# ErikNatanael/knaster

Hardware: AMD Instinct MI355X
Metric: UGen-samples/sec (voices x block_size x UGens / s) (higher is better)
Workload: dtype f32

## Files before the change

bindings/rust/knaster_hip/src/ffi.rs:

```rust
#![allow(non_camel_case_types)]
use core::ffi::{c_char, c_void};

#[repr(C)]
pub struct knh_bank {
    _private: [u8; 0],
}
#[repr(C)]
pub struct knh_comm {
    _private: [u8; 0],
}
pub const KNH_COMM_ID_BYTES: usize = 128;
pub type knh_reduce_fn = Option<unsafe extern "C" fn(user: *mut c_void, device_buf: *mut c_void, count: usize, sample_type: u32, root: u32, hip_stream: *mut c_void) -> i32>;

#[repr(C)]
#[derive(Clone, Copy, Debug, Default, PartialEq, Eq)]
pub struct knh_stage_desc {
    pub kind: u16,
    pub flags: u16,
    pub delayed_changes_per_block: u16,
    pub ar_param: u16,
    pub input: u16,
    pub input2: u16,
}

#[repr(C)]
pub struct knh_bank_desc {
    pub abi_version: u32,
    pub n_voices: u32,
    pub sample_type: u32,
    pub n_stages: u32,
    pub stages: *const knh_stage_desc,
    pub out_channels: u32,
    pub mix_mode: u32,
    pub device: i32,
    pub allow_fma: u32,
    pub in_channels: u32,
}

pub const KNH_ABI_VERSION: u32 = 4;

pub const KNH_OK: i32 = 0;
pub const KNH_ERR_INVALID_ARGUMENT: i32 = 1;
pub const KNH_ERR_OUT_OF_RANGE: i32 = 2;
pub const KNH_ERR_UNSUPPORTED_CHAIN: i32 = 3;
pub const KNH_ERR_DEVICE: i32 = 4;
pub const KNH_ERR_NOT_INITIALISED: i32 = 5;
pub const KNH_ERR_NO_DEVICE: i32 = 6;
pub const KNH_ERR_WRONG_VALUE_KIND: i32 = 7;
pub const KNH_ERR_OUT_OF_MEMORY: i32 = 8;
pub const KNH_ERR_INTERNAL: i32 = 9;

pub const KNH_F32: u32 = 0;
pub const KNH_F64: u32 = 1;

pub const KNH_VALUE_FLOAT: u32 = 0;
pub const KNH_VALUE_TRIGGER: u32 = 1;
pub const KNH_VALUE_INTEGER: u32 = 2;
pub const KNH_VALUE_BOOL: u32 = 3;
pub const KNH_VALUE_SMOOTHING: u32 = 4;

pub const KNH_STAGE_SIN_WT: u16 = 0;
pub const KNH_STAGE_SIN_NUMERIC: u16 = 1;
pub const KNH_STAGE_SVF: u16 = 2;
pub const KNH_STAGE_ONEPOLE_LPF: u16 = 3;
pub const KNH_STAGE_ONEPOLE_HPF: u16 = 4;
pub const KNH_STAGE_MUL_ENV_ASR: u16 = 5;
pub const KNH_STAGE_MUL_ENV_AR: u16 = 6;
pub const KNH_STAGE_MUL_CONST: u16 = 7;
pub const KNH_STAGE_ADD_CONST: u16 = 8;
pub const KNH_STAGE_SUB_CONST: u16 = 9;
pub const KNH_STAGE_DIV_CONST: u16 = 10;
pub const KNH_STAGE_WR_MUL: u16 = 11;
pub const KNH_STAGE_WR_ADD: u16 = 12;
pub const KNH_STAGE_WR_SUB: u16 = 13;
pub const KNH_STAGE_MUL_ENVELOPE: u16 = 14;
pub const KNH_STAGE_WR_VSUB: u16 = 15;
pub const KNH_STAGE_WR_DIV: u16 = 16;
pub const KNH_STAGE_WR_VDIV: u16 = 17;
pub const KNH_STAGE_WR_POWF: u16 = 18;
pub const KNH_STAGE_WR_POWI: u16 = 19;
pub const KNH_STAGE_POW_CONST: u16 = 20;
pub const KNH_STAGE_SAMPLE_DELAY: u16 = 21;
pub const KNH_STAGE_PHASOR: u16 = 22;
pub const KNH_STAGE_SAFETY_LIMITER: u16 = 23;
pub const KNH_STAGE_POLYBLEP: u16 = 24;
pub const KNH_STAGE_ALLPASS_DELAY: u16 = 25;
pub const KNH_STAGE_ALLPASS_FB_DELAY: u16 = 26;
pub const KNH_STAGE_BUFFER_READER: u16 = 27;
pub const KNH_STAGE_WHITE_NOISE: u16 = 28;
pub const KNH_STAGE_PINK_NOISE: u16 = 29;
pub const KNH_STAGE_BROWN_NOISE: u16 = 30;
pub const KNH_STAGE_RANDOM_LIN: u16 = 31;
pub const KNH_STAGE_PAN2: u16 = 32;
pub const KNH_STAGE_MATH_ADD: u16 = 33;
pub const KNH_STAGE_MATH_SUB: u16 = 34;
pub const KNH_STAGE_MATH_MUL: u16 = 35;
pub const KNH_STAGE_MATH_DIV: u16 = 36;
pub const KNH_STAGE_MATH_POW: u16 = 37;
pub const KNH_STAGE_INPUT: u16 = 38;
pub const KNH_STAGE_GALACTIC: u16 = 39;
pub const KNH_STAGE_KIND_COUNT: u16 = 40;

pub const KNH_SVF_LOW: u32 = 0;
pub const KNH_SVF_HIGH: u32 = 1;
pub const KNH_SVF_BAND: u32 = 2;
pub const KNH_SVF_NOTCH: u32 = 3;
pub const KNH_SVF_PEAK: u32 = 4;
pub const KNH_SVF_ALL: u32 = 5;
pub const KNH_SVF_BELL: u32 = 6;
pub const KNH_SVF_LOW_SHELF: u32 = 7;
pub const KNH_SVF_HIGH_SHELF: u32 = 8;

pub const KNH_STAGE_FLAG_AR_FREQ: u16 = 1 << 0;
pub const KNH_STAGE_FLAG_SMOOTH_PARAMS: u16 = 1 << 1;

pub const KNH_MIX_TREE: u32 = 0;
pub const KNH_MIX_LEFT_FOLD: u32 = 1;

pub const KNH_FLAG_ANY_DONE: u32 = 1 << 0;
pub const KNH_FLAG_ALL_DONE: u32 = 1 << 1;

#[link(name = "knaster_hip")]
unsafe extern "C" {
    pub fn knh_abi_version() -> u32;
    pub fn knh_device_count() -> i32;
    pub fn knh_status_string(status: i32) -> *const c_char;
    pub fn knh_last_error(bank: *const knh_bank) -> *const c_char;
    pub fn knh_chain_ugen_count(stages: *const knh_stage_desc, n_stages: u32) -> i32;
    pub fn knh_bank_create(desc: *const knh_bank_desc, out_bank: *mut *mut knh_bank) -> i32;
    pub fn knh_bank_create_sharded(desc: *const knh_bank_desc, host_threads: u32, out_bank: *mut *mut knh_bank) -> i32;
    pub fn knh_bank_set_ctor_args(bank: *mut knh_bank, stage: u32, first_voice: u32, count: u32, args: *const f64, n_args: u32) -> i32;
    pub fn knh_bank_set_buffer(bank: *mut knh_bank, stage: u32, samples: *const c_void, n_frames: usize, buffer_sample_rate: f64) -> i32;
    pub fn knh_bank_init(bank: *mut knh_bank, sample_rate: u32, block_size: usize) -> i32;
    pub fn knh_bank_destroy(bank: *mut knh_bank);
    pub fn knh_bank_inputs(bank: *const knh_bank) -> u16;
    pub fn knh_bank_outputs(bank: *const knh_bank) -> u16;
    pub fn knh_bank_stage_parameters(bank: *const knh_bank, stage: u32) -> u16;
    pub fn knh_bank_stage_param_description(bank: *const knh_bank, stage: u32, param: u32) -> *const c_char;
    pub fn knh_bank_param_apply(bank: *mut knh_bank, voice: u32, stage: u32, param: u32, kind: u32, fvalue: f64, ivalue: i64) -> i32;
    pub fn knh_bank_set_delay_within_block_for_param(bank: *mut knh_bank, voice: u32, stage: u32, param: u32, delay: u16) -> i32;
    pub fn knh_bank_param_apply_range(bank: *mut knh_bank, voice_begin: u32, voice_end: u32, stage: u32, param: u32, kind: u32, fvalue: f64, ivalue: i64) -> i32;
    pub fn knh_bank_param_apply_many(bank: *mut knh_bank, count: usize, voices: *const u32, stages: *const u32, params: *const u32, kinds: *const u32, fvalues: *const f64, ivalues: *const i64, delays: *const u16) -> i32;
    pub fn knh_bank_process_block(bank: *mut knh_bank, frames_to_process: usize, block_start_offset: usize, frame_clock: u64, out: *mut c_void, out_flags: *mut u32) -> i32;
    pub fn knh_jit_stats(memory_hits: *mut u64, disk_hits: *mut u64, helper_compiles: *mut u64, in_process_compiles: *mut u64);
    pub fn knh_bank_resident_stats(bank: *mut knh_bank, calls: *mut u64, launches: *mut u64) -> i32;
    pub fn knh_bank_resident_trace(bank: *mut knh_bank, ticks5: *mut u64) -> i32;
    pub fn knh_bank_process_block_channels(bank: *mut knh_bank, frames_to_process: usize, block_start_offset: usize, frame_clock: u64, out_channels: *const *mut c_void, out_flags: *mut u32) -> i32;
    pub fn knh_bank_process_block_device(bank: *mut knh_bank, frames_to_process: usize, block_start_offset: usize, frame_clock: u64, out_device: *mut c_void, hip_stream: *mut c_void) -> i32;
    pub fn knh_bank_process_block_voices(bank: *mut knh_bank, frames_to_process: usize, block_start_offset: usize, frame_clock: u64, out: *mut c_void, voices_out: *mut c_void, out_flags: *mut u32) -> i32;
    pub fn knh_bank_process_blocks(bank: *mut knh_bank, n_blocks: u32, frame_clock: u64, out: *mut c_void, out_flags: *mut u32) -> i32;
    pub fn knh_bank_process_blocks_device(bank: *mut knh_bank, n_blocks: u32, frame_clock: u64, out_device: *mut c_void, hip_stream: *mut c_void) -> i32;
    pub fn knh_bank_process_blocks_device_add(bank: *mut knh_bank, n_blocks: u32, frame_clock: u64, out_device: *mut c_void, hip_stream: *mut c_void) -> i32;
    pub fn knh_device_malloc(bytes: usize, device: i32) -> *mut c_void;
    pub fn knh_device_free(device_ptr: *mut c_void);
    pub fn knh_device_read(dst_host: *mut c_void, src_device: *const c_void, bytes: usize, hip_stream: *mut c_void) -> i32;
    pub fn knh_bank_param_apply_many_at(bank: *mut knh_bank, block_offset: u32, count: usize, voices: *const u32, stages: *const u32, params: *const u32, kinds: *const u32, fvalues: *const f64, ivalues: *const i64, delays: *const u16) -> i32;
    pub fn knh_bank_read_done_frames(bank: *mut knh_bank, done_frames: *mut u32) -> i32;
    pub fn knh_bank_debug_words(bank: *mut knh_bank, out16: *mut u32) -> i32;
    pub fn knh_bank_debug_signature(bank: *const knh_bank) -> *const core::ffi::c_char;
    pub fn knh_bank_synchronize(bank: *mut knh_bank) -> i32;
    pub fn knh_bank_timing_reset(bank: *mut knh_bank, enable: i32) -> i32;
    pub fn knh_bank_timing_read(bank: *mut knh_bank, kernel_ms: *mut f64, launches: *mut u64) -> i32;
    pub fn knh_bank_collective_timing_read(bank: *mut knh_bank, reduce_ms: *mut f64, reduces: *mut u64) -> i32;
    pub fn knh_bank_algorithmic_bytes_per_voice_block(bank: *const knh_bank, read_bytes: *mut u32, write_bytes: *mut u32) -> i32;
    pub fn knh_bank_process_blocks_begin(bank: *mut knh_bank, n_blocks: u32, frame_clock: u64) -> i32;
    pub fn knh_bank_process_blocks_end(bank: *mut knh_bank, out: *mut c_void) -> i32;
    pub fn knh_bank_set_input(bank: *mut knh_bank, n_blocks: u32, input: *const c_void) -> i32;
    pub fn knh_bank_set_input_device(bank: *mut knh_bank, n_blocks: u32, in_device: *const c_void) -> i32;
    pub fn knh_bank_create_multi_device(desc: *const knh_bank_desc, devices: *const i32, n_devices: u32, out_bank: *mut *mut knh_bank) -> i32;
    pub fn knh_comm_unique_id(id: *mut u8) -> i32;
    pub fn knh_bank_create_rank(desc: *const knh_bank_desc, rank: u32, world: u32, comm_id: *const u8, out_bank: *mut *mut knh_bank) -> i32;
    pub fn knh_bank_create_rank_custom(desc: *const knh_bank_desc, rank: u32, world: u32, reduce: knh_reduce_fn, user: *mut c_void, out_bank: *mut *mut knh_bank) -> i32;
    pub fn knh_shard_voice_range(n_voices: u32, rank: u32, world: u32, first: *mut u32, count: *mut u32) -> i32;
    pub fn knh_bank_ranks(bank: *const knh_bank) -> u32;
    pub fn knh_comm_create(rank: u32, world: u32, id: *const u8, device: i32, out_comm: *mut *mut knh_comm) -> i32;
    pub fn knh_comm_destroy(comm: *mut knh_comm);
    pub fn knh_comm_last_error(comm: *const knh_comm) -> *const c_char;
    pub fn knh_comm_world(comm: *const knh_comm) -> u32;
    pub fn knh_comm_rccl_version() -> i32;
    pub fn knh_comm_reduce_sum(comm: *mut knh_comm, buf: *mut c_void, count: usize, sample_type: u32, root: u32, after_stream: *mut c_void) -> i32;
    pub fn knh_comm_wait_buffer(comm: *mut knh_comm, buf: *const c_void, stream: *mut c_void) -> i32;
    pub fn knh_comm_wait(comm: *mut knh_comm, stream: *mut c_void) -> i32;
    pub fn knh_comm_synchronize(comm: *mut knh_comm) -> i32;
    pub fn knh_comm_timing_reset(comm: *mut knh_comm, enable: i32) -> i32;
    pub fn knh_comm_timing_read(comm: *mut knh_comm, reduce_ms: *mut f64, reduces: *mut u64) -> i32;
}
```

include/knaster_hip.h:

```cpp
#ifndef KNASTER_HIP_H
#define KNASTER_HIP_H

#include <stddef.h>
#include <stdint.h>

#ifdef __cplusplus
extern "C" {
#endif

#define KNH_ABI_VERSION 4

typedef enum knh_status {
  KNH_OK = 0,
  KNH_ERR_INVALID_ARGUMENT = 1,
  KNH_ERR_OUT_OF_RANGE = 2,
  KNH_ERR_UNSUPPORTED_CHAIN = 3,
  KNH_ERR_DEVICE = 4,
  KNH_ERR_NOT_INITIALISED = 5,
  KNH_ERR_NO_DEVICE = 6,
  KNH_ERR_WRONG_VALUE_KIND = 7,
  KNH_ERR_OUT_OF_MEMORY = 8,
  KNH_ERR_INTERNAL = 9
} knh_status;

typedef enum knh_sample_type { KNH_F32 = 0, KNH_F64 = 1 } knh_sample_type;

typedef enum knh_value_kind {
  KNH_VALUE_FLOAT = 0,
  KNH_VALUE_TRIGGER = 1,
  KNH_VALUE_INTEGER = 2,
  KNH_VALUE_BOOL = 3,
  KNH_VALUE_SMOOTHING = 4
} knh_value_kind;

typedef enum knh_stage_kind {
  KNH_STAGE_SIN_WT = 0,
  KNH_STAGE_SIN_NUMERIC = 1,
  KNH_STAGE_SVF = 2,
  KNH_STAGE_ONEPOLE_LPF = 3,
  KNH_STAGE_ONEPOLE_HPF = 4,
  KNH_STAGE_MUL_ENV_ASR = 5,
  KNH_STAGE_MUL_ENV_AR = 6,
  KNH_STAGE_MUL_CONST = 7,
  KNH_STAGE_ADD_CONST = 8,
  KNH_STAGE_SUB_CONST = 9,
  KNH_STAGE_DIV_CONST = 10,
  KNH_STAGE_WR_MUL = 11,
  KNH_STAGE_WR_ADD = 12,
  KNH_STAGE_WR_SUB = 13,
  KNH_STAGE_MUL_ENVELOPE = 14,
  KNH_STAGE_WR_VSUB = 15,
  KNH_STAGE_WR_DIV = 16,
  KNH_STAGE_WR_VDIV = 17,
  KNH_STAGE_WR_POWF = 18,
  KNH_STAGE_WR_POWI = 19,
  KNH_STAGE_POW_CONST = 20,
  KNH_STAGE_SAMPLE_DELAY = 21,
  KNH_STAGE_PHASOR = 22,
  KNH_STAGE_SAFETY_LIMITER = 23,
  KNH_STAGE_POLYBLEP = 24,
  KNH_STAGE_ALLPASS_DELAY = 25,
  KNH_STAGE_ALLPASS_FB_DELAY = 26,
  KNH_STAGE_BUFFER_READER = 27,
  KNH_STAGE_WHITE_NOISE = 28,
  KNH_STAGE_PINK_NOISE = 29,
  KNH_STAGE_BROWN_NOISE = 30,
  KNH_STAGE_RANDOM_LIN = 31,
  KNH_STAGE_PAN2 = 32,
  KNH_STAGE_MATH_ADD = 33,
  KNH_STAGE_MATH_SUB = 34,
  KNH_STAGE_MATH_MUL = 35,
  KNH_STAGE_MATH_DIV = 36,
  KNH_STAGE_MATH_POW = 37,
  KNH_STAGE_INPUT = 38,
  KNH_STAGE_GALACTIC = 39,
  KNH_STAGE_KIND_COUNT = 40
} knh_stage_kind;

typedef enum knh_svf_type {
  KNH_SVF_LOW = 0, KNH_SVF_HIGH = 1, KNH_SVF_BAND = 2, KNH_SVF_NOTCH = 3, KNH_SVF_PEAK = 4,
  KNH_SVF_ALL = 5, KNH_SVF_BELL = 6, KNH_SVF_LOW_SHELF = 7, KNH_SVF_HIGH_SHELF = 8
} knh_svf_type;

enum {
  KNH_STAGE_FLAG_AR_FREQ = 1u << 0,
  KNH_STAGE_FLAG_SMOOTH_PARAMS = 1u << 1
};

typedef struct knh_stage_desc {
  uint16_t kind;
  uint16_t flags;
  uint16_t delayed_changes_per_block;
  uint16_t ar_param;
  uint16_t input;
  uint16_t input2;
} knh_stage_desc;

typedef enum knh_mix_mode {
  KNH_MIX_TREE = 0,
  KNH_MIX_LEFT_FOLD = 1
} knh_mix_mode;

typedef struct knh_bank_desc {
  uint32_t abi_version;
  uint32_t n_voices;
  uint32_t sample_type;
  uint32_t n_stages;
  const knh_stage_desc* stages;
  uint32_t out_channels;
  uint32_t mix_mode;
  int32_t device;
  uint32_t allow_fma;
  uint32_t in_channels;
} knh_bank_desc;

typedef struct knh_bank knh_bank;

enum {
  KNH_FLAG_ANY_DONE = 1u << 0,
  KNH_FLAG_ALL_DONE = 1u << 1
};

uint32_t knh_abi_version(void);
int32_t knh_device_count(void);
const char* knh_status_string(int32_t status);
const char* knh_last_error(const knh_bank* bank);

int32_t knh_chain_ugen_count(const knh_stage_desc* stages, uint32_t n_stages);

int32_t knh_bank_create(const knh_bank_desc* desc, knh_bank** out_bank);
int32_t knh_bank_create_sharded(const knh_bank_desc* desc, uint32_t host_threads, knh_bank** out_bank);
int32_t knh_bank_set_ctor_args(knh_bank* bank, uint32_t stage, uint32_t first_voice, uint32_t count,
                               const double* args, uint32_t n_args);
int32_t knh_bank_set_buffer(knh_bank* bank, uint32_t stage, const void* samples, size_t n_frames, double buffer_sample_rate);
int32_t knh_bank_init(knh_bank* bank, uint32_t sample_rate, size_t block_size);
void knh_bank_destroy(knh_bank* bank);

uint16_t knh_bank_inputs(const knh_bank* bank);
uint16_t knh_bank_outputs(const knh_bank* bank);
uint16_t knh_bank_stage_parameters(const knh_bank* bank, uint32_t stage);
const char* knh_bank_stage_param_description(const knh_bank* bank, uint32_t stage, uint32_t param);

int32_t knh_bank_param_apply(knh_bank* bank, uint32_t voice, uint32_t stage, uint32_t param,
                             uint32_t kind, double fvalue, int64_t ivalue);
int32_t knh_bank_set_delay_within_block_for_param(knh_bank* bank, uint32_t voice, uint32_t stage,
                                                  uint32_t param, uint16_t delay);
int32_t knh_bank_param_apply_many(knh_bank* bank, size_t count, const uint32_t* voices,
                                  const uint32_t* stages, const uint32_t* params,
                                  const uint32_t* kinds, const double* fvalues,
                                  const int64_t* ivalues, const uint16_t* delays);
int32_t knh_bank_param_apply_range(knh_bank* bank, uint32_t voice_begin, uint32_t voice_end, uint32_t stage,
                                   uint32_t param, uint32_t kind, double fvalue, int64_t ivalue);

int32_t knh_bank_process_block(knh_bank* bank, size_t frames_to_process, size_t block_start_offset,
                               uint64_t frame_clock, void* out, uint32_t* out_flags);
int32_t knh_bank_process_block_channels(knh_bank* bank, size_t frames_to_process, size_t block_start_offset,
                                        uint64_t frame_clock, void* const* out_channels, uint32_t* out_flags);
int32_t knh_bank_resident_stats(knh_bank* bank, uint64_t* calls, uint64_t* launches);
int32_t knh_bank_resident_trace(knh_bank* bank, uint64_t* ticks5);
int32_t knh_bank_process_block_device(knh_bank* bank, size_t frames_to_process,
                                      size_t block_start_offset, uint64_t frame_clock,
                                      void* out_device, void* hip_stream);
int32_t knh_bank_set_input(knh_bank* bank, uint32_t n_blocks, const void* in);
int32_t knh_bank_set_input_device(knh_bank* bank, uint32_t n_blocks, const void* in_device);
int32_t knh_bank_process_block_voices(knh_bank* bank, size_t frames_to_process,
                                      size_t block_start_offset, uint64_t frame_clock, void* out,
                                      void* voices_out, uint32_t* out_flags);
int32_t knh_bank_process_blocks(knh_bank* bank, uint32_t n_blocks, uint64_t frame_clock, void* out,
                                uint32_t* out_flags);
int32_t knh_bank_process_blocks_device(knh_bank* bank, uint32_t n_blocks, uint64_t frame_clock,
                                       void* out_device, void* hip_stream);
int32_t knh_bank_process_blocks_device_add(knh_bank* bank, uint32_t n_blocks, uint64_t frame_clock,
                                           void* out_device, void* hip_stream);
int32_t knh_bank_process_blocks_begin(knh_bank* bank, uint32_t n_blocks, uint64_t frame_clock);
int32_t knh_bank_process_blocks_end(knh_bank* bank, void* out);
void* knh_device_malloc(size_t bytes, int32_t device);
void knh_device_free(void* device_ptr);
int32_t knh_device_read(void* dst_host, const void* src_device, size_t bytes, void* hip_stream);
int32_t knh_bank_param_apply_many_at(knh_bank* bank, uint32_t block_offset, size_t count,
                                     const uint32_t* voices, const uint32_t* stages,
                                     const uint32_t* params, const uint32_t* kinds,
                                     const double* fvalues, const int64_t* ivalues,
                                     const uint16_t* delays);
int32_t knh_bank_read_done_frames(knh_bank* bank, uint32_t* done_frames);
int32_t knh_bank_debug_words(knh_bank* bank, uint32_t* out16);
const char* knh_bank_debug_signature(const knh_bank* bank);
void knh_jit_stats(uint64_t* memory_hits, uint64_t* disk_hits, uint64_t* helper_compiles, uint64_t* in_process_compiles);
int32_t knh_bank_synchronize(knh_bank* bank);

int32_t knh_bank_timing_reset(knh_bank* bank, int32_t enable);
int32_t knh_bank_timing_read(knh_bank* bank, double* kernel_ms, uint64_t* launches);
int32_t knh_bank_collective_timing_read(knh_bank* bank, double* reduce_ms, uint64_t* reduces);
int32_t knh_bank_algorithmic_bytes_per_voice_block(const knh_bank* bank, uint32_t* read_bytes,
                                                   uint32_t* write_bytes);


int32_t knh_bank_create_multi_device(const knh_bank_desc* desc, const int32_t* devices, uint32_t n_devices, knh_bank** out_bank);

#define KNH_COMM_ID_BYTES 128
int32_t knh_comm_unique_id(uint8_t* id);
int32_t knh_bank_create_rank(const knh_bank_desc* desc, uint32_t rank, uint32_t world, const uint8_t* comm_id, knh_bank** out_bank);
typedef int32_t (*knh_reduce_fn)(void* user, void* device_buf, size_t count, uint32_t sample_type, uint32_t root, void* hip_stream);
int32_t knh_bank_create_rank_custom(const knh_bank_desc* desc, uint32_t rank, uint32_t world, knh_reduce_fn reduce, void* user,
                                    knh_bank** out_bank);
int32_t knh_shard_voice_range(uint32_t n_voices, uint32_t rank, uint32_t world, uint32_t* first, uint32_t* count);
uint32_t knh_bank_ranks(const knh_bank* bank);

typedef struct knh_comm knh_comm;
int32_t knh_comm_create(uint32_t rank, uint32_t world, const uint8_t* id, int32_t device, knh_comm** out_comm);
void knh_comm_destroy(knh_comm* comm);
const char* knh_comm_last_error(const knh_comm* comm);
uint32_t knh_comm_world(const knh_comm* comm);
int32_t knh_comm_rccl_version(void);
int32_t knh_comm_reduce_sum(knh_comm* comm, void* buf, size_t count, uint32_t sample_type, uint32_t root, void* after_stream);
int32_t knh_comm_wait_buffer(knh_comm* comm, const void* buf, void* stream);
int32_t knh_comm_wait(knh_comm* comm, void* stream);
int32_t knh_comm_synchronize(knh_comm* comm);
int32_t knh_comm_timing_reset(knh_comm* comm, int32_t enable);
int32_t knh_comm_timing_read(knh_comm* comm, double* reduce_ms, uint64_t* reduces);

#ifdef __cplusplus
}
#endif
#endif
```

knaster_amd/_lib.py:

```python
from __future__ import annotations

import ctypes as C
import os

_HERE = os.path.dirname(os.path.abspath(__file__))
LIB_PATH = os.environ.get("KNH_LIB") or os.path.join(_HERE, "csrc", "libknaster_hip.so")

KNH_ABI_VERSION = 4

OK, ERR_INVALID_ARGUMENT, ERR_OUT_OF_RANGE, ERR_UNSUPPORTED_CHAIN, ERR_DEVICE = 0, 1, 2, 3, 4
ERR_NOT_INITIALISED, ERR_NO_DEVICE, ERR_WRONG_VALUE_KIND, ERR_OUT_OF_MEMORY, ERR_INTERNAL = 5, 6, 7, 8, 9
F32, F64 = 0, 1
VALUE_FLOAT, VALUE_TRIGGER, VALUE_INTEGER, VALUE_BOOL, VALUE_SMOOTHING = 0, 1, 2, 3, 4
(STAGE_SIN_WT, STAGE_SIN_NUMERIC, STAGE_SVF, STAGE_ONEPOLE_LPF, STAGE_ONEPOLE_HPF, STAGE_MUL_ENV_ASR,
 STAGE_MUL_ENV_AR, STAGE_MUL_CONST, STAGE_ADD_CONST, STAGE_SUB_CONST, STAGE_DIV_CONST, STAGE_WR_MUL,
 STAGE_WR_ADD, STAGE_WR_SUB, STAGE_MUL_ENVELOPE, STAGE_WR_VSUB, STAGE_WR_DIV, STAGE_WR_VDIV, STAGE_WR_POWF,
 STAGE_WR_POWI, STAGE_POW_CONST, STAGE_SAMPLE_DELAY, STAGE_PHASOR, STAGE_SAFETY_LIMITER, STAGE_POLYBLEP, STAGE_ALLPASS_DELAY, STAGE_ALLPASS_FB_DELAY, STAGE_BUFFER_READER,
 STAGE_WHITE_NOISE, STAGE_PINK_NOISE, STAGE_BROWN_NOISE, STAGE_RANDOM_LIN, STAGE_PAN2,
 STAGE_MATH_ADD, STAGE_MATH_SUB, STAGE_MATH_MUL, STAGE_MATH_DIV, STAGE_MATH_POW, STAGE_INPUT, STAGE_GALACTIC) = range(40)
STAGE_FLAG_AR_FREQ = 1
STAGE_FLAG_SMOOTH_PARAMS = 2
SVF_LOW, SVF_HIGH, SVF_BAND, SVF_NOTCH, SVF_PEAK, SVF_ALL, SVF_BELL, SVF_LOW_SHELF, SVF_HIGH_SHELF = range(9)
MIX_TREE, MIX_LEFT_FOLD = 0, 1
FLAG_ANY_DONE, FLAG_ALL_DONE = 1, 2

STAGE_CTOR_ARGS = {
    STAGE_SIN_WT: 1, STAGE_SIN_NUMERIC: 1, STAGE_SVF: 4, STAGE_ONEPOLE_LPF: 1, STAGE_ONEPOLE_HPF: 0,
    STAGE_MUL_ENV_ASR: 2, STAGE_MUL_ENV_AR: 2, STAGE_MUL_CONST: 1, STAGE_ADD_CONST: 1, STAGE_SUB_CONST: 1,
    STAGE_DIV_CONST: 1, STAGE_WR_MUL: 1, STAGE_WR_ADD: 1, STAGE_WR_SUB: 1,
    STAGE_WR_VSUB: 1, STAGE_WR_DIV: 1, STAGE_WR_VDIV: 1, STAGE_WR_POWF: 1, STAGE_WR_POWI: 1, STAGE_POW_CONST: 1, STAGE_SAMPLE_DELAY: 1, STAGE_PHASOR: 1, STAGE_SAFETY_LIMITER: 0, STAGE_POLYBLEP: 2, STAGE_ALLPASS_DELAY: 1, STAGE_ALLPASS_FB_DELAY: 1, STAGE_BUFFER_READER: 3,
    STAGE_WHITE_NOISE: 1, STAGE_PINK_NOISE: 1, STAGE_BROWN_NOISE: 1, STAGE_RANDOM_LIN: 2, STAGE_PAN2: 1,
    STAGE_MATH_ADD: 0, STAGE_MATH_SUB: 0, STAGE_MATH_MUL: 0, STAGE_MATH_DIV: 0, STAGE_MATH_POW: 0, STAGE_INPUT: 1,
    STAGE_GALACTIC: 7,
}


class StageDesc(C.Structure):
    _fields_ = [("kind", C.c_uint16), ("flags", C.c_uint16), ("delayed_changes_per_block", C.c_uint16),
                ("ar_param", C.c_uint16), ("input", C.c_uint16), ("input2", C.c_uint16)]


class BankDesc(C.Structure):
    _fields_ = [("abi_version", C.c_uint32), ("n_voices", C.c_uint32), ("sample_type", C.c_uint32),
                ("n_stages", C.c_uint32), ("stages", C.POINTER(StageDesc)), ("out_channels", C.c_uint32),
                ("mix_mode", C.c_uint32), ("device", C.c_int32), ("allow_fma", C.c_uint32), ("in_channels", C.c_uint32)]


PROTOTYPES = {
    "knh_abi_version": (C.c_uint32, []),
    "knh_device_count": (C.c_int32, []),
    "knh_status_string": (C.c_char_p, [C.c_int32]),
    "knh_last_error": (C.c_char_p, [C.c_void_p]),
    "knh_chain_ugen_count": (C.c_int32, [C.POINTER(StageDesc), C.c_uint32]),
    "knh_bank_create": (C.c_int32, [C.POINTER(BankDesc), C.POINTER(C.c_void_p)]),
    "knh_bank_create_sharded": (C.c_int32, [C.POINTER(BankDesc), C.c_uint32, C.POINTER(C.c_void_p)]),
    "knh_bank_set_ctor_args": (C.c_int32, [C.c_void_p, C.c_uint32, C.c_uint32, C.c_uint32, C.c_void_p, C.c_uint32]),
    "knh_bank_set_buffer": (C.c_int32, [C.c_void_p, C.c_uint32, C.c_void_p, C.c_size_t, C.c_double]),
    "knh_bank_init": (C.c_int32, [C.c_void_p, C.c_uint32, C.c_size_t]),
    "knh_bank_destroy": (None, [C.c_void_p]),
    "knh_bank_inputs": (C.c_uint16, [C.c_void_p]),
    "knh_bank_outputs": (C.c_uint16, [C.c_void_p]),
    "knh_bank_stage_parameters": (C.c_uint16, [C.c_void_p, C.c_uint32]),
    "knh_bank_stage_param_description": (C.c_char_p, [C.c_void_p, C.c_uint32, C.c_uint32]),
    "knh_bank_param_apply": (C.c_int32, [C.c_void_p, C.c_uint32, C.c_uint32, C.c_uint32, C.c_uint32, C.c_double, C.c_int64]),
    "knh_bank_set_delay_within_block_for_param": (C.c_int32, [C.c_void_p, C.c_uint32, C.c_uint32, C.c_uint32, C.c_uint16]),
    "knh_bank_param_apply_many": (C.c_int32, [C.c_void_p, C.c_size_t, C.c_void_p, C.c_void_p, C.c_void_p, C.c_void_p,
                                             C.c_void_p, C.c_void_p, C.c_void_p]),
    "knh_bank_param_apply_range": (C.c_int32, [C.c_void_p, C.c_uint32, C.c_uint32, C.c_uint32, C.c_uint32, C.c_uint32, C.c_double, C.c_int64]),
    "knh_bank_process_block": (C.c_int32, [C.c_void_p, C.c_size_t, C.c_size_t, C.c_uint64, C.c_void_p, C.POINTER(C.c_uint32)]),
    "knh_jit_stats": (None, [C.POINTER(C.c_uint64), C.POINTER(C.c_uint64), C.POINTER(C.c_uint64), C.POINTER(C.c_uint64)]),
    "knh_bank_resident_stats": (C.c_int32, [C.c_void_p, C.POINTER(C.c_uint64), C.POINTER(C.c_uint64)]),
    "knh_bank_resident_trace": (C.c_int32, [C.c_void_p, C.POINTER(C.c_uint64)]),
    "knh_bank_process_block_channels": (C.c_int32, [C.c_void_p, C.c_size_t, C.c_size_t, C.c_uint64, C.POINTER(C.c_void_p), C.POINTER(C.c_uint32)]),
    "knh_bank_process_block_device": (C.c_int32, [C.c_void_p, C.c_size_t, C.c_size_t, C.c_uint64, C.c_void_p, C.c_void_p]),
    "knh_bank_process_block_voices": (C.c_int32, [C.c_void_p, C.c_size_t, C.c_size_t, C.c_uint64, C.c_void_p, C.c_void_p,
                                                 C.POINTER(C.c_uint32)]),
    "knh_bank_process_blocks": (C.c_int32, [C.c_void_p, C.c_uint32, C.c_uint64, C.c_void_p, C.POINTER(C.c_uint32)]),
    "knh_bank_process_blocks_device": (C.c_int32, [C.c_void_p, C.c_uint32, C.c_uint64, C.c_void_p, C.c_void_p]),
    "knh_bank_process_blocks_device_add": (C.c_int32, [C.c_void_p, C.c_uint32, C.c_uint64, C.c_void_p, C.c_void_p]),
    "knh_device_malloc": (C.c_void_p, [C.c_size_t, C.c_int32]),
    "knh_device_free": (None, [C.c_void_p]),
    "knh_device_read": (C.c_int32, [C.c_void_p, C.c_void_p, C.c_size_t, C.c_void_p]),
    "knh_bank_param_apply_many_at": (C.c_int32, [C.c_void_p, C.c_uint32, C.c_size_t, C.c_void_p, C.c_void_p, C.c_void_p,
                                                C.c_void_p, C.c_void_p, C.c_void_p, C.c_void_p]),
    "knh_bank_read_done_frames": (C.c_int32, [C.c_void_p, C.c_void_p]),
    "knh_bank_debug_words": (C.c_int32, [C.c_void_p, C.c_void_p]),
    "knh_bank_debug_signature": (C.c_char_p, [C.c_void_p]),
    "knh_bank_synchronize": (C.c_int32, [C.c_void_p]),
    "knh_bank_timing_reset": (C.c_int32, [C.c_void_p, C.c_int32]),
    "knh_bank_timing_read": (C.c_int32, [C.c_void_p, C.POINTER(C.c_double), C.POINTER(C.c_uint64)]),
    "knh_bank_collective_timing_read": (C.c_int32, [C.c_void_p, C.POINTER(C.c_double), C.POINTER(C.c_uint64)]),
    "knh_bank_algorithmic_bytes_per_voice_block": (C.c_int32, [C.c_void_p, C.POINTER(C.c_uint32), C.POINTER(C.c_uint32)]),
}

COMM_ID_BYTES = 128
REDUCE_FN = C.CFUNCTYPE(C.c_int32, C.c_void_p, C.c_void_p, C.c_size_t, C.c_uint32, C.c_uint32, C.c_void_p)
PROTOTYPES.update({
    "knh_bank_process_blocks_begin": (C.c_int32, [C.c_void_p, C.c_uint32, C.c_uint64]),
    "knh_bank_process_blocks_end": (C.c_int32, [C.c_void_p, C.c_void_p]),
    "knh_bank_set_input": (C.c_int32, [C.c_void_p, C.c_uint32, C.c_void_p]),
    "knh_bank_set_input_device": (C.c_int32, [C.c_void_p, C.c_uint32, C.c_void_p]),
    "knh_bank_create_multi_device": (C.c_int32, [C.POINTER(BankDesc), C.POINTER(C.c_int32), C.c_uint32, C.POINTER(C.c_void_p)]),
    "knh_comm_unique_id": (C.c_int32, [C.c_void_p]),
    "knh_bank_create_rank": (C.c_int32, [C.POINTER(BankDesc), C.c_uint32, C.c_uint32, C.c_void_p, C.POINTER(C.c_void_p)]),
    "knh_bank_create_rank_custom": (C.c_int32, [C.POINTER(BankDesc), C.c_uint32, C.c_uint32, REDUCE_FN, C.c_void_p, C.POINTER(C.c_void_p)]),
    "knh_shard_voice_range": (C.c_int32, [C.c_uint32, C.c_uint32, C.c_uint32, C.POINTER(C.c_uint32), C.POINTER(C.c_uint32)]),
    "knh_bank_ranks": (C.c_uint32, [C.c_void_p]),
    "knh_comm_create": (C.c_int32, [C.c_uint32, C.c_uint32, C.c_void_p, C.c_int32, C.POINTER(C.c_void_p)]),
    "knh_comm_destroy": (None, [C.c_void_p]),
    "knh_comm_last_error": (C.c_char_p, [C.c_void_p]),
    "knh_comm_world": (C.c_uint32, [C.c_void_p]),
    "knh_comm_rccl_version": (C.c_int32, []),
    "knh_comm_reduce_sum": (C.c_int32, [C.c_void_p, C.c_void_p, C.c_size_t, C.c_uint32, C.c_uint32, C.c_void_p]),
    "knh_comm_wait_buffer": (C.c_int32, [C.c_void_p, C.c_void_p, C.c_void_p]),
    "knh_comm_wait": (C.c_int32, [C.c_void_p, C.c_void_p]),
    "knh_comm_synchronize": (C.c_int32, [C.c_void_p]),
    "knh_comm_timing_reset": (C.c_int32, [C.c_void_p, C.c_int32]),
    "knh_comm_timing_read": (C.c_int32, [C.c_void_p, C.POINTER(C.c_double), C.POINTER(C.c_uint64)]),
})

_lib = None


class KnasterHipError(RuntimeError):
    def __init__(self, status: int, message: str):
        super().__init__(f"knaster_hip status {status}: {message}")
        self.status = status


def load() -> C.CDLL:
    global _lib
    if _lib is not None:
        return _lib
    if not os.path.exists(LIB_PATH):
        raise ImportError(
            f"{LIB_PATH} is missing: build it with `python -m knaster_amd.build` "
            "(hipcc --offload-arch=gfx950).  knaster_amd has no CPU fallback.")
    lib = C.CDLL(LIB_PATH)
    for name, (res, args) in PROTOTYPES.items():
        fn = getattr(lib, name)
        fn.restype = res
        fn.argtypes = args
    if lib.knh_abi_version() != KNH_ABI_VERSION:
        raise ImportError("libknaster_hip.so ABI version mismatch; rebuild it")
    _lib = lib
    return lib
```

knaster_amd/bank.py:

```python
from __future__ import annotations

import ctypes as C
from dataclasses import dataclass
from typing import Optional, Sequence

import numpy as np

from . import _lib as L

TRIGGER = object()


@dataclass(frozen=True)
class Stage:
    kind: int
    flags: int = 0
    delayed_changes_per_block: int = 0
    input: int = 0
    input2: int = 0
    ar_param: int = 0


def _stage_array(stages: Sequence[Stage]):
    arr = (L.StageDesc * len(stages))()
# ... 84 lines not shown
    def _check(self, rc: int):
        if rc != L.OK:
            raise L.KnasterHipError(rc, (self._lib.knh_last_error(self._h) or b"").decode())

    def set_ctor_args(self, stage: int, args, first_voice: int = 0):
        a = np.ascontiguousarray(np.asarray(args, dtype=np.float64))
        if a.ndim == 1:
            a = a.reshape(-1, 1)
        self._check(self._lib.knh_bank_set_ctor_args(self._h, stage, first_voice, a.shape[0],
                                                     a.ctypes.data_as(C.c_void_p), a.shape[1]))

    def set_buffer(self, stage: int, samples, buffer_sample_rate: float):
        a = np.ascontiguousarray(np.asarray(samples, dtype=self.dtype))
        self._check(self._lib.knh_bank_set_buffer(self._h, stage, a.ctypes.data_as(C.c_void_p), a.shape[0], float(buffer_sample_rate)))

    def init(self, sample_rate: int, block_size: int):
        self._check(self._lib.knh_bank_init(self._h, sample_rate, block_size))
        self.sample_rate, self.block_size = sample_rate, block_size

    def inputs(self) -> int:
        return int(self._lib.knh_bank_inputs(self._h))

    def outputs(self) -> int:
        return int(self._lib.knh_bank_outputs(self._h))

    def stage_parameters(self, stage: int) -> int:
        return int(self._lib.knh_bank_stage_parameters(self._h, stage))

    def stage_param_descriptions(self, stage: int):
        out = []
        for p in range(self.stage_parameters(stage)):
            d = self._lib.knh_bank_stage_param_description(self._h, stage, p)
            out.append(d.decode() if d else None)
        return out

    @staticmethod
    def _value(value):
        if value is TRIGGER:
            return L.VALUE_TRIGGER, 0.0, 0
        if isinstance(value, (bool, np.bool_)):
            return L.VALUE_BOOL, 0.0, int(value)
        if isinstance(value, (int, np.integer)):
            return L.VALUE_INTEGER, 0.0, int(value)
        return L.VALUE_FLOAT, float(value), 0

    def param_apply(self, voice: int, stage: int, param: int, value):
        kind, f, i = self._value(value)
        self._check(self._lib.knh_bank_param_apply(self._h, voice, stage, param, kind, f, i))

    def param(self, voice: int, stage: int, param, value):
        if isinstance(param, str):
            descs = self.stage_param_descriptions(stage)
            if param not in descs:
                raise KeyError(f"DescriptionNotFound({param!r})")
            param = descs.index(param)
        self.param_apply(voice, stage, param, value)

    def set_delay_within_block_for_param(self, voice: int, stage: int, param: int, delay: int):
        self._check(self._lib.knh_bank_set_delay_within_block_for_param(self._h, voice, stage, param, delay))

    def param_apply_many(self, voices, stages, params, kinds, fvalues=None, ivalues=None, delays=None, block_offset=0):
        self.param_apply_prepared(self.prepare_many(voices, stages, params, kinds, fvalues, ivalues, delays), block_offset)

    def param_apply_range(self, voice_begin, voice_end, stage, param, kind, fvalue=0.0, ivalue=0):
        self._check(self._lib.knh_bank_param_apply_range(self._h, voice_begin, voice_end, stage, param, kind, float(fvalue), int(ivalue)))

    @staticmethod
    def prepare_many(voices, stages, params, kinds, fvalues=None, ivalues=None, delays=None):
        v = np.ascontiguousarray(voices, dtype=np.uint32)
        n = v.shape[0]
        s = np.ascontiguousarray(np.broadcast_to(np.asarray(stages, dtype=np.uint32), (n,)))
        p = np.ascontiguousarray(np.broadcast_to(np.asarray(params, dtype=np.uint32), (n,)))
        k = np.ascontiguousarray(np.broadcast_to(np.asarray(kinds, dtype=np.uint32), (n,)))
        f = None if fvalues is None else np.ascontiguousarray(np.broadcast_to(np.asarray(fvalues, dtype=np.float64), (n,)))
        i = None if ivalues is None else np.ascontiguousarray(np.broadcast_to(np.asarray(ivalues, dtype=np.int64), (n,)))
        d = None if delays is None else np.ascontiguousarray(np.broadcast_to(np.asarray(delays, dtype=np.uint16), (n,)))
        arrays = (v, s, p, k, f, i, d)
        return n, arrays, tuple(None if a is None else a.ctypes.data_as(C.c_void_p) for a in arrays)

    def param_apply_prepared(self, batch, block_offset=0):
        n, _arrays, ptrs = batch
        if block_offset:
            self._check(self._lib.knh_bank_param_apply_many_at(self._h, block_offset, n, *ptrs))
        else:
            self._check(self._lib.knh_bank_param_apply_many(self._h, n, *ptrs))

    def set_input(self, blocks):
        a = np.ascontiguousarray(np.asarray(blocks, dtype=self.dtype))
        if a.ndim == 2:
            a = a.reshape(1, *a.shape)
        assert a.shape[1:] == (self.in_channels, self.block_size), a.shape
        self._check(self._lib.knh_bank_set_input(self._h, a.shape[0], a.ctypes.data_as(C.c_void_p)))

    def process_block(self, frames_to_process: Optional[int] = None, block_start_offset: int = 0, frame_clock: int = 0,
                      out: Optional[np.ndarray] = None):
        ftp = self.block_size if frames_to_process is None else frames_to_process
        if out is None:
            out = np.zeros((self.out_channels, self.block_size), dtype=self.dtype)
        flags = C.c_uint32(0)
        self._check(self._lib.knh_bank_process_block(self._h, ftp, block_start_offset, frame_clock,
                                                     out.ctypes.data_as(C.c_void_p), C.byref(flags)))
        return out, int(flags.value)

    def process_block_voices(self, frames_to_process: Optional[int] = None, block_start_offset: int = 0, frame_clock: int = 0):
        ftp = self.block_size if frames_to_process is None else frames_to_process
        out = np.zeros((self.out_channels, self.block_size), dtype=self.dtype)
        pan = bool(self.stages) and self.stages[-1].kind in (L.STAGE_PAN2, L.STAGE_GALACTIC)
        voices = np.zeros((2, self.n_voices, self.block_size) if pan else (self.n_voices, self.block_size), dtype=self.dtype)
        flags = C.c_uint32(0)
        self._check(self._lib.knh_bank_process_block_voices(self._h, ftp, block_start_offset, frame_clock,
                                                            out.ctypes.data_as(C.c_void_p),
                                                            voices.ctypes.data_as(C.c_void_p), C.byref(flags)))
        return out, voices, int(flags.value)

    def process_block_device(self, out_device_ptr: int = 0, hip_stream: int = 0, frames_to_process: Optional[int] = None,
                             block_start_offset: int = 0, frame_clock: int = 0):
        ftp = self.block_size if frames_to_process is None else frames_to_process
        self._check(self._lib.knh_bank_process_block_device(self._h, ftp, block_start_offset, frame_clock,
                                                            C.c_void_p(out_device_ptr or None), C.c_void_p(hip_stream or None)))

    def process_blocks(self, n_blocks: int, frame_clock: int = 0):
        out = np.zeros((n_blocks, self.out_channels, self.block_size), dtype=self.dtype)
        flags = C.c_uint32(0)
        self._check(self._lib.knh_bank_process_blocks(self._h, n_blocks, frame_clock, out.ctypes.data_as(C.c_void_p), C.byref(flags)))
        return out, int(flags.value)

    def process_blocks_begin(self, n_blocks: int, frame_clock: int = 0):
        self._check(self._lib.knh_bank_process_blocks_begin(self._h, n_blocks, frame_clock))
        self._begun = getattr(self, "_begun", []) + [n_blocks]

    def process_blocks_end(self):
        n_blocks = self._begun.pop(0)
        out = np.zeros((n_blocks, self.out_channels, self.block_size), dtype=self.dtype)
        self._check(self._lib.knh_bank_process_blocks_end(self._h, out.ctypes.data_as(C.c_void_p)))
        return out

    def process_blocks_device(self, n_blocks: int, out_device_ptr: int = 0, hip_stream: int = 0, frame_clock: int = 0):
        self._check(self._lib.knh_bank_process_blocks_device(self._h, n_blocks, frame_clock, C.c_void_p(out_device_ptr or None),
                                                             C.c_void_p(hip_stream or None)))

    def read_done_frames(self) -> np.ndarray:
        d = np.zeros(self.n_voices, dtype=np.uint32)
        self._check(self._lib.knh_bank_read_done_frames(self._h, d.ctypes.data_as(C.c_void_p)))
        return d

    def debug_signature(self) -> str:
        return self._lib.knh_bank_debug_signature(self._h).decode()

    def resident_stats(self):
        c, n = C.c_uint64(0), C.c_uint64(0)
        self._check(self._lib.knh_bank_resident_stats(self._h, C.byref(c), C.byref(n)))
        return int(c.value), int(n.value)

    def debug_words(self) -> np.ndarray:
        d = np.zeros(16, dtype=np.uint32)
        self._check(self._lib.knh_bank_debug_words(self._h, d.ctypes.data_as(C.c_void_p)))
        return d

    def synchronize(self):
        self._check(self._lib.knh_bank_synchronize(self._h))

    def ranks(self) -> int:
        return int(self._lib.knh_bank_ranks(self._h))

    def timing_reset(self, enable: bool = True):
        self._check(self._lib.knh_bank_timing_reset(self._h, 1 if enable else 0))

    def timing_read(self):
        ms, n = C.c_double(0), C.c_uint64(0)
        self._check(self._lib.knh_bank_timing_read(self._h, C.byref(ms), C.byref(n)))
        return float(ms.value), int(n.value)

    def collective_timing_read(self):
        ms, n = C.c_double(0), C.c_uint64(0)
        self._check(self._lib.knh_bank_collective_timing_read(self._h, C.byref(ms), C.byref(n)))
        return float(ms.value), int(n.value)

    def algorithmic_bytes_per_voice_block(self):
        r, w = C.c_uint32(0), C.c_uint32(0)
        self._check(self._lib.knh_bank_algorithmic_bytes_per_voice_block(self._h, C.byref(r), C.byref(w)))
        return int(r.value), int(w.value)
```

knaster_amd/build.py:

```python
from __future__ import annotations

import os
import shutil
import subprocess
import sys

HERE = os.path.dirname(os.path.abspath(__file__))
CSRC = os.path.join(HERE, "csrc")
LIB = os.path.join(CSRC, "libknaster_hip.so")
SOURCES = ["kernels_pipe.hip", "kernels_single.hip", "kernels_wide.hip", "kernels_fold.hip", "kernels_interp.hip", "kernels_events.hip", "kernels_galactic.hip", "bank.hip", "jit.hip", "comm.hip"]
UNITS = [("kernels_pipe.hip", "kernels_pipe_mixer.o", ["-DKNH_PIPE_PART=0"]), ("kernels_pipe.hip", "kernels_pipe_fold.o", ["-DKNH_PIPE_PART=1"]),
         ("kernels_pipe.hip", "kernels_pipe_inplace.o", ["-DKNH_PIPE_PART=2"])] + [(s, s.replace(".hip", ".o"), []) for s in SOURCES[1:]]
HELPER = os.path.join(CSRC, "knh_jit_helper")
HEADERS = ["jit_cache.hpp", "stage_table.hpp", "bank_base.hpp", "voice_bank.hpp", "resident_call.hpp", "event_resolver.hpp", "chain_signature.hpp", "voice_stages.hpp", "voice_chain.hpp", "voice_pipe.hpp", "voice_frame.hpp", "kernel_registry.hpp", "jit.hpp", "host_shards.hpp", "shard_workers.hpp", "rank_bank.hpp", "galactic_bank.hpp", "voice_galactic.hpp", os.path.join("..", "..", "include", "knaster_hip.h"),
           os.path.join("..", "build.py")]
FLAGS = [
    "--offload-arch=gfx950",
    "-O3",
    "-std=c++17",
    "-ffp-contract=off",
    "-fPIC",
    "-Wall",
    "-Wno-unused-value",
]
LINK_FLAGS = ["--offload-arch=gfx950", "-shared", "-fPIC", "-lhiprtc", "-lpthread", "-ldl"]


def _hipcc() -> str:
    for cand in (os.environ.get("HIPCC"), shutil.which("hipcc"), "/opt/rocm/bin/hipcc"):
        if cand and os.path.exists(cand):
            return cand
    raise RuntimeError("hipcc not found (looked at $HIPCC, PATH, /opt/rocm/bin/hipcc)")


def needs_build() -> bool:
    if not os.path.exists(LIB) or not os.path.exists(HELPER):
        return True
    t = min(os.path.getmtime(LIB), os.path.getmtime(HELPER))
    deps = [os.path.join(CSRC, f) for f in SOURCES + HEADERS + ["jit_helper.cpp"]]
    return any(os.path.getmtime(d) > t for d in deps)


def build_helper(verbose: bool = True) -> str:
    src = os.path.join(CSRC, "jit_helper.cpp")
    if os.path.exists(HELPER) and os.path.getmtime(HELPER) >= max(os.path.getmtime(src), os.path.getmtime(os.path.join(CSRC, "jit_cache.hpp"))):
        return HELPER
    rocm = os.environ.get("ROCM_PATH", "/opt/rocm")
    cmd = [os.environ.get("CXX", "g++"), "-std=c++17", "-O2", "-Wall", "-D__HIP_PLATFORM_AMD__", "-I" + os.path.join(rocm, "include"), src, "-o", HELPER + ".tmp",
           "-L" + os.path.join(rocm, "lib"), "-Wl,-rpath," + os.path.join(rocm, "lib"), "-lhiprtc", "-lpthread"]
    if verbose:
        print("[knaster_amd.build]", " ".join(cmd), flush=True)
    res = subprocess.run(cmd, cwd=CSRC, capture_output=True, text=True)
    if res.returncode != 0:
        sys.stderr.write(res.stdout + res.stderr)
        raise RuntimeError("building knh_jit_helper failed")
    os.replace(HELPER + ".tmp", HELPER)
    return HELPER


def write_jit_source() -> None:
    text = open(os.path.join(CSRC, "voice_stages.hpp")).read()
    chain = open(os.path.join(CSRC, "voice_chain.hpp")).read()
    text += "\n" + chain.replace("#pragma once", "").replace('#include "voice_stages.hpp"', "")
    pipe = open(os.path.join(CSRC, "voice_pipe.hpp")).read()
    text += "\n" + pipe.replace("#pragma once", "").replace('#include "voice_chain.hpp"', "")
    frame = open(os.path.join(CSRC, "voice_frame.hpp")).read()
    text += "\n" + frame.replace("#pragma once", "").replace('#include "voice_chain.hpp"', "")
    chunks = [text[i:i + 8000] for i in range(0, len(text), 8000)]
    body = "\n".join('R"KNHJIT(' + c + ')KNHJIT"' for c in chunks) + "\n"
    path = os.path.join(CSRC, "jit_source.inc")
    if not os.path.exists(path) or open(path).read() != body:
        with open(path, "w") as f:
            f.write(body)


def build(force: bool = False, verbose: bool = True, variant: str = "") -> str:
    variant = variant or os.environ.get("KNH_BUILD_VARIANT", "")
    lib = LIB if not variant else LIB.replace(".so", "_" + variant + ".so")
    if not force and not variant and not needs_build():
        return LIB
    build_helper(verbose)
    write_jit_source()
    extra = ["-DKNH_DAG_STAMPS"] if os.environ.get("KNH_BUILD_STAMPS") == "1" or variant == "stamps" else []
    extra += os.environ.get("KNH_EXTRA_FLAGS", "").split()
    objdir = os.path.join(CSRC, "build" + ("_" + variant if variant else ""))
    os.makedirs(objdir, exist_ok=True)
    hipcc = _hipcc()
    procs = []
    objs = []
    header_time = max(os.path.getmtime(os.path.join(CSRC, h)) for h in HEADERS if os.path.exists(os.path.join(CSRC, h)))
    header_time = max(header_time, os.path.getmtime(os.path.join(CSRC, "jit_source.inc")))
    for src, objname, unit_flags in UNITS:
        obj = os.path.join(objdir, objname)
        objs.append(obj)
        cmd = [hipcc, *FLAGS, *extra, *unit_flags, "-c", src, "-o", obj]
        stamp = obj + ".flags"
        fresh = (not force and os.path.exists(obj) and os.path.exists(stamp) and open(stamp).read() == " ".join(cmd)
                 and os.path.getmtime(obj) >= max(os.path.getmtime(os.path.join(CSRC, src)), header_time))
        if fresh:
            continue
        if os.path.exists(stamp):
            os.remove(stamp)
        if verbose:
            print("[knaster_amd.build]", " ".join(cmd), flush=True)
        procs.append((src, obj, subprocess.Popen(cmd, cwd=CSRC, stdout=subprocess.PIPE, stderr=subprocess.STDOUT, text=True), " ".join(cmd)))
    failed = False
    for src, obj, p, cmdline in procs:
        out, _ = p.communicate()
        if p.returncode == 0:
            with open(obj + ".flags", "w") as f:
                f.write(cmdline)
        if p.returncode != 0:
            sys.stderr.write(out)
            failed = True
        elif out.strip() and verbose:
            sys.stderr.write(out)
    if failed:
        raise RuntimeError("hipcc failed building libknaster_hip.so")
    cmd = [hipcc, *LINK_FLAGS, "-o", lib + ".tmp", *objs]
    if verbose:
        print("[knaster_amd.build]", " ".join(cmd), flush=True)
    res = subprocess.run(cmd, cwd=CSRC, capture_output=True, text=True)
    if res.returncode != 0:
        sys.stderr.write(res.stdout + res.stderr)
        raise RuntimeError("hipcc failed linking libknaster_hip.so")
    os.replace(lib + ".tmp", lib)
    return lib


if __name__ == "__main__":
    print(build(force="--force" in sys.argv, variant=next((a.split("=", 1)[1] for a in sys.argv if a.startswith("--variant=")), "")))
```

knaster_amd/csrc/bank.hip:

```cpp
#include <hip/hip_runtime.h>

#include <algorithm>
#include <atomic>
#include <chrono>
#include <cmath>
#include <cstddef>
#include <cstdio>
#include <cstdlib>
#include <cstring>
#include <functional>
#include <memory>
#include <mutex>
#include <new>
#include <stdexcept>
#include <string>
#include <thread>
#include <vector>

#include "../../include/knaster_hip.h"
#include "jit.hpp"
#include "kernel_registry.hpp"

using knh_dev::Event;
using knh_dev::VoiceKernelArgs;

#include "stage_table.hpp"
#include "bank_base.hpp"
#include "chain_signature.hpp"
#include "event_resolver.hpp"
#include "resident_call.hpp"
#include "voice_bank.hpp"

namespace {

template <typename F>
knh_bank* make_bank(const knh_bank_desc& d, const knh::KernelEntry* entry, const std::string& sig) {
  std::unique_ptr<Bank<F>> b(new Bank<F>());
  b->desc = d;
  b->entry = entry;
  b->signature = sig;
  {
    const char* jit_env = std::getenv("KNH_JIT");
    if (jit_env && jit_env[0] == '1') b->entry = nullptr;
    const char* env = std::getenv("KNH_PIPELINE");
    const int level = env && env[0] >= '0' && env[0] <= '2' ? env[0] - '0' : 1;
    b->pipeline_level = level;
    const char* big_env = std::getenv("KNH_PIPE_BIG");
    const unsigned forms = big_env && big_env[0] == '0' ? 1u : (big_env && big_env[0] == '1' ? 3u : 7u);
    if (b->entry && level >= 1) b->pipe = knh::find_pipe(sig.c_str(), forms);
    {
      const unsigned groups = (d.n_voices + 63u) / 64u;
      const char* penv = std::getenv("KNH_PAIR");
      const knh::PipeEntry* pair = b->entry && level >= 1 ? knh::find_pipe(sig.c_str(), 1u << 2 , 2) : nullptr;
      const bool want = penv ? penv[0] == '1' : (groups > 256u && groups <= 512u && d.sample_type != KNH_F64);
      if (pair && want && !(penv && penv[0] == '0')) { b->pipe = pair; b->pipe_pair = true; }
    }
    b->wide = b->entry && !b->pipe_pair ? knh::find_wide(sig.c_str()) : nullptr;
    if (b->wide) {
      const unsigned groups = (d.n_voices + 63u) / 64u;
      const unsigned pipe_max = d.sample_type == KNH_F64 ? 256u : 512u;
      int ww = groups <= pipe_max && b->pipe ? 0 : (groups <= 1024 ? 4 : 8);
      if (!b->pipe && groups <= 256) ww = 0;
      if (b->pipe && sig.find_first_of("DYZ") != std::string::npos) ww = groups <= 256 ? 0 : (groups <= 1024 ? 4 : 8);
      const char* wenv = std::getenv("KNH_WIDE");
      if (wenv) ww = std::atoi(wenv);
      if (ww == 4 || ww == 8 || ww == 16) b->wide_waves = ww;
    }
  }
  b->nv = d.n_voices;
  int slot = 0, pbase = 0;
  for (uint32_t i = 0; i < d.n_stages; ++i) {
    const KindInfo& k = kKinds[d.stages[i].kind];
    StageInfo s{d.stages[i].kind, d.stages[i].flags, d.stages[i].delayed_changes_per_block, slot, k.n_slots, k.n_params, k.n_ctor, pbase,
                d.stages[i].input, d.stages[i].input2, d.stages[i].ar_param};
    if (s.kind == KNH_STAGE_SVF && s.ar_param != 0) s.n_slots = 12;
    b->stages.push_back(s);
    b->ctor.emplace_back(static_cast<size_t>(d.n_voices) * (k.n_ctor > 0 ? k.n_ctor : 0), 0.0);
    slot += s.n_slots;
    pbase += k.n_params;
  }
  b->n_slots = slot;
  b->n_params_total = pbase;
  b->desc.stages = nullptr;
  return b.release();
}

}

#include "host_shards.hpp"
#include "rank_bank.hpp"
#include "galactic_bank.hpp"

namespace {
template <typename F>
knh_bank* make_sharded(const knh_bank_desc& d, const knh::KernelEntry* entry, const std::string& sig, uint32_t host_threads,
                       const int32_t* devices = nullptr) {
  const uint32_t groups = (d.n_voices + 63u) / 64u;
  const uint32_t k = std::min(host_threads, groups);
  const uint32_t per = ((groups + k - 1) / k) * 64u;
  std::unique_ptr<ShardedBank<F>> b(new ShardedBank<F>());
  b->desc = d;
  b->nv = d.n_voices;
  b->per_shard = per;
  for (uint32_t v = 0; v < d.n_voices; v += per) {
    knh_bank_desc dk = d;
    dk.n_voices = std::min(per, d.n_voices - v);
    if (devices) {
      dk.device = devices[b->shard.size()];
      b->shard_device.push_back(dk.device);
    }
    b->base.push_back(v);
    b->shard.emplace_back(make_bank<F>(dk, entry, sig));
  }
  b->base.push_back(d.n_voices);
  b->stages = b->shard[0]->stages;
  b->n_slots = b->shard[0]->n_slots;
  b->n_params_total = b->shard[0]->n_params_total;
  b->desc.stages = nullptr;
  return b.release();
}
}

namespace {
template <typename F>
knh_bank* make_rank_bank(const knh_bank_desc& d, const knh::KernelEntry* entry, const std::string& sig, uint32_t rank, uint32_t world,
                                const uint8_t* comm_id, knh_reduce_fn reduce, void* user) {
  std::unique_ptr<RankBank<F>> b(new RankBank<F>());
  b->desc = d;
  b->total = d.n_voices;
  b->rank = rank;
  b->world = world;
  uint32_t first = 0, count = 0;
  shard_voice_range(d.n_voices, rank, world, &first, &count);
  b->lo = first;
  b->hi = first + count;
  if (comm_id) std::memcpy(b->comm_id, comm_id, KNH_COMM_ID_BYTES);
  b->custom = reduce;
  b->custom_user = user;
  knh_bank_desc dl = d;
  dl.n_voices = count ? count : 1;
  const char* env = std::getenv("KNH_HOST_THREADS");
  const long k = env ? std::strtol(env, nullptr, 10) : 0;
  std::unique_ptr<knh_bank> proto(k >= 2 && k <= 64 && dl.n_voices > 64 ? make_sharded<F>(dl, entry, sig, static_cast<uint32_t>(k)) : make_bank<F>(dl, entry, sig));
  b->stages = proto->stages;
  b->n_slots = proto->n_slots;
  b->n_params_total = proto->n_params_total;
  if (count) b->local = std::move(proto);
  b->desc.stages = nullptr;
  return b.release();
}
}

namespace {
inline bool ends_in_galactic(const knh_bank_desc& d) { return d.n_stages > 0 && d.stages[d.n_stages - 1].kind == KNH_STAGE_GALACTIC; }
template <typename F>
knh_bank* make_galactic(const knh_bank_desc& d, const std::string& inner_sig) {
  std::unique_ptr<GalacticBank<F>> b(new GalacticBank<F>());
  knh_bank_desc di = d;
  di.n_stages = d.n_stages - 1;
  di.out_channels = 1;
  di.mix_mode = KNH_MIX_TREE;
  b->inner.reset(static_cast<Bank<F>*>(make_bank<F>(di, knh::find_kernel(inner_sig.c_str()), inner_sig)));
  b->desc = d;
  b->nv = d.n_voices;
  b->gstage = d.n_stages - 1;
  b->stages = b->inner->stages;
  const KindInfo& k = kKinds[KNH_STAGE_GALACTIC];
  b->stages.push_back(StageInfo{KNH_STAGE_GALACTIC, 0, 0, b->inner->n_slots, k.n_slots, k.n_params, k.n_ctor, b->inner->n_params_total, 0, 0, 0});
  b->n_slots = b->inner->n_slots;
  b->n_params_total = b->inner->n_params_total + k.n_params;
  b->gctor.assign(static_cast<size_t>(d.n_voices) * 7, 0.0);
  b->par.assign(static_cast<size_t>(d.n_voices) * 5, F(0));
  b->drifted.assign(d.n_voices, 0);
  b->h_params.resize(d.n_voices);
  b->desc.stages = nullptr;
  return b.release();
}
}

namespace {
template <typename Fn>
int32_t guarded(knh_bank* bank, Fn&& fn) noexcept {
  const char* what = nullptr;
// ... 141 lines not shown
  return guarded(nullptr, [&]() -> int32_t {
    if (world > 1 && !reduce) { g_create_error = "null reduce function"; if (out_bank) *out_bank = nullptr; return KNH_ERR_INVALID_ARGUMENT; }
    return create_rank_bank(desc, rank, world, nullptr, reduce, user, out_bank);
  });
}
uint32_t knh_bank_ranks(const knh_bank* bank) { return bank ? bank->ranks() : 0; }

static int32_t create_bank(const knh_bank_desc* desc, uint32_t host_threads, knh_bank** out_bank) {
  return guarded(nullptr, [&]() -> int32_t {
    std::string sig;
    int rc = check_desc(desc, out_bank, &sig);
    if (rc != KNH_OK) return rc;
    if (host_threads > 64) { g_create_error = "host_threads must be at most 64"; return KNH_ERR_INVALID_ARGUMENT; }
    if (ends_in_galactic(*desc)) {
      *out_bank = desc->sample_type == KNH_F64 ? make_galactic<double>(*desc, sig) : make_galactic<float>(*desc, sig);
      return KNH_OK;
    }
    const knh::KernelEntry* entry = knh::find_kernel(sig.c_str());
    if (host_threads >= 2 && desc->mix_mode == KNH_MIX_TREE && desc->n_voices > 64)
      *out_bank = desc->sample_type == KNH_F64 ? make_sharded<double>(*desc, entry, sig, host_threads) : make_sharded<float>(*desc, entry, sig, host_threads);
    else
      *out_bank = desc->sample_type == KNH_F64 ? make_bank<double>(*desc, entry, sig) : make_bank<float>(*desc, entry, sig);
    return KNH_OK;
  });
}

int32_t knh_bank_create(const knh_bank_desc* desc, knh_bank** out_bank) {
  return guarded(nullptr, [&]() -> int32_t {
    const char* env = std::getenv("KNH_HOST_THREADS");
    const long k = env ? std::strtol(env, nullptr, 10) : 0;
    return create_bank(desc, k >= 2 && k <= 64 ? static_cast<uint32_t>(k) : 0u, out_bank);
  });
}

int32_t knh_bank_create_sharded(const knh_bank_desc* desc, uint32_t host_threads, knh_bank** out_bank) {
  return guarded(nullptr, [&]() -> int32_t {
    return create_bank(desc, host_threads, out_bank);
  });
}

void knh_bank_destroy(knh_bank* bank) {
  try {
    if (bank && bank->pipe_stream) {
      (void)hipSetDevice(bank->device);
      (void)hipStreamSynchronize(bank->pipe_stream);
    }
    delete bank;
  } catch (...) {
  }
}

int32_t knh_bank_set_ctor_args(knh_bank* bank, uint32_t stage, uint32_t first_voice, uint32_t count, const double* args, uint32_t n_args) {
  return guarded(bank, [&]() -> int32_t {
    if (!bank) return KNH_ERR_INVALID_ARGUMENT;
    return bank->set_ctor(stage, first_voice, count, args, n_args);
  });
}
int32_t knh_bank_set_buffer(knh_bank* bank, uint32_t stage, const void* samples, size_t n_frames, double buffer_sample_rate) {
  return guarded(bank, [&]() -> int32_t {
    if (!bank) return KNH_ERR_INVALID_ARGUMENT;
    return bank->set_buffer(stage, samples, n_frames, buffer_sample_rate);
  });
}
int32_t knh_bank_init(knh_bank* bank, uint32_t sample_rate, size_t block_size) {
  return guarded(bank, [&]() -> int32_t {
    if (!bank) return KNH_ERR_INVALID_ARGUMENT;
    const int rc = bank->init(sample_rate, block_size);
    if (rc == KNH_OK) bank->channel_block.assign(static_cast<size_t>(bank->desc.out_channels) * block_size * (bank->desc.sample_type == KNH_F64 ? 8 : 4), 0);
    return rc;
  });
}
uint16_t knh_bank_inputs(const knh_bank* bank) { return bank ? static_cast<uint16_t>(bank->desc.in_channels) : 0; }
int32_t knh_bank_set_input(knh_bank* bank, uint32_t n_blocks, const void* in) {
  return guarded(bank, [&]() -> int32_t {
    if (!bank) return KNH_ERR_INVALID_ARGUMENT;
    if (!in) return bank->fail(KNH_ERR_INVALID_ARGUMENT, "null input");
    return bank->set_input(n_blocks, in, nullptr);
  });
}
int32_t knh_bank_set_input_device(knh_bank* bank, uint32_t n_blocks, const void* in_device) {
  return guarded(bank, [&]() -> int32_t {
    if (!bank) return KNH_ERR_INVALID_ARGUMENT;
    if (!in_device) return bank->fail(KNH_ERR_INVALID_ARGUMENT, "null input");
    return bank->set_input(n_blocks, nullptr, in_device);
  });
}
uint16_t knh_bank_outputs(const knh_bank* bank) { return bank ? static_cast<uint16_t>(bank->desc.out_channels) : 0; }
uint16_t knh_bank_stage_parameters(const knh_bank* bank, uint32_t stage) {
  if (!bank || stage >= bank->stages.size()) return 0;
  return static_cast<uint16_t>(bank->stages[stage].n_params);
}
const char* knh_bank_stage_param_description(const knh_bank* bank, uint32_t stage, uint32_t param) {
  if (!bank || stage >= bank->stages.size() || param >= static_cast<uint32_t>(bank->stages[stage].n_params)) return nullptr;
  return kKinds[bank->stages[stage].kind].params[param];
}
int32_t knh_bank_param_apply(knh_bank* bank, uint32_t voice, uint32_t stage, uint32_t param, uint32_t kind, double fvalue, int64_t ivalue) {
  return guarded(bank, [&]() -> int32_t {
    if (!bank) return KNH_ERR_INVALID_ARGUMENT;
    return bank->param_apply(voice, stage, param, kind, fvalue, ivalue);
  });
}
int32_t knh_bank_set_delay_within_block_for_param(knh_bank* bank, uint32_t voice, uint32_t stage, uint32_t param, uint16_t delay) {
  return guarded(bank, [&]() -> int32_t {
    if (!bank) return KNH_ERR_INVALID_ARGUMENT;
    return bank->set_delay(voice, stage, param, delay);
  });
}
int32_t knh_bank_param_apply_many(knh_bank* bank, size_t count, const uint32_t* voices, const uint32_t* stages, const uint32_t* params,
                                  const uint32_t* kinds, const double* fvalues, const int64_t* ivalues, const uint16_t* delays) {
  return guarded(bank, [&]() -> int32_t {
    if (!bank) return KNH_ERR_INVALID_ARGUMENT;
    if (count && (!voices || !stages || !params || !kinds)) return bank->fail(KNH_ERR_INVALID_ARGUMENT, "null array");
    return bank->apply_many(0, count, voices, stages, params, kinds, fvalues, ivalues, delays);
  });
}
int32_t knh_bank_param_apply_range(knh_bank* bank, uint32_t voice_begin, uint32_t voice_end, uint32_t stage, uint32_t param, uint32_t kind,
                                   double fvalue, int64_t ivalue) {
  return guarded(bank, [&]() -> int32_t {
    if (!bank) return KNH_ERR_INVALID_ARGUMENT;
    if (voice_end < voice_begin) return bank->fail(KNH_ERR_INVALID_ARGUMENT, "voice_end < voice_begin");
    return bank->apply_range(voice_begin, voice_end, stage, param, kind, fvalue, ivalue);
  });
}
int32_t knh_bank_process_block(knh_bank* bank, size_t frames_to_process, size_t block_start_offset, uint64_t frame_clock, void* out, uint32_t* out_flags) {
  return guarded(bank, [&]() -> int32_t {
    if (!bank) return KNH_ERR_INVALID_ARGUMENT;
    if (!out) return bank->fail(KNH_ERR_INVALID_ARGUMENT, "null output block");
    return bank->process(1, frames_to_process, block_start_offset, frame_clock, out, nullptr, nullptr, out_flags, nullptr, true);
  });
}
int32_t knh_bank_process_block_channels(knh_bank* bank, size_t frames_to_process, size_t block_start_offset, uint64_t frame_clock, void* const* out_channels, uint32_t* out_flags) {
  return guarded(bank, [&]() -> int32_t {
    if (!bank) return KNH_ERR_INVALID_ARGUMENT;
    if (!out_channels) return bank->fail(KNH_ERR_INVALID_ARGUMENT, "null output channels");
    for (uint32_t c = 0; c < bank->desc.out_channels; ++c)
      if (!out_channels[c]) return bank->fail(KNH_ERR_INVALID_ARGUMENT, "null output channel");
    if (!bank->initialised) return bank->fail(KNH_ERR_NOT_INITIALISED, "bank not initialised");
    unsigned char* blk = bank->channel_block.data();
    const int rc = bank->process(1, frames_to_process, block_start_offset, frame_clock, blk, nullptr, nullptr, out_flags, nullptr, true);
    if (rc != KNH_OK) return rc;
    const size_t word = bank->desc.sample_type == KNH_F64 ? 8 : 4;
    for (uint32_t c = 0; c < bank->desc.out_channels; ++c)
      std::memcpy(out_channels[c], blk + (static_cast<size_t>(c) * bank->block_size + block_start_offset) * word, frames_to_process * word);
    return KNH_OK;
  });
}
int32_t knh_bank_resident_stats(knh_bank* bank, uint64_t* calls, uint64_t* launches) {
  return guarded(bank, [&]() -> int32_t {
    if (!bank) return KNH_ERR_INVALID_ARGUMENT;
    bank->resident_stats(calls, launches);
    return KNH_OK;
  });
}
int32_t knh_bank_resident_trace(knh_bank* bank, uint64_t* ticks5) {
  return guarded(bank, [&]() -> int32_t {
    if (!bank || !ticks5) return KNH_ERR_INVALID_ARGUMENT;
    bank->resident_trace(ticks5);
    return KNH_OK;
  });
}
int32_t knh_bank_process_block_device(knh_bank* bank, size_t frames_to_process, size_t block_start_offset, uint64_t frame_clock, void* out_device, void* hip_stream) {
  return guarded(bank, [&]() -> int32_t {
    if (!bank) return KNH_ERR_INVALID_ARGUMENT;
    return bank->process(1, frames_to_process, block_start_offset, frame_clock, nullptr, out_device, nullptr, nullptr, hip_stream, false);
  });
}
int32_t knh_bank_process_block_voices(knh_bank* bank, size_t frames_to_process, size_t block_start_offset, uint64_t frame_clock, void* out, void* voices_out, uint32_t* out_flags) {
  return guarded(bank, [&]() -> int32_t {
    if (!bank) return KNH_ERR_INVALID_ARGUMENT;
    if (!voices_out) return bank->fail(KNH_ERR_INVALID_ARGUMENT, "null voices_out");
    return bank->process(1, frames_to_process, block_start_offset, frame_clock, out, nullptr, voices_out, out_flags, nullptr, true);
  });
}
int32_t knh_bank_process_blocks(knh_bank* bank, uint32_t n_blocks, uint64_t frame_clock, void* out, uint32_t* out_flags) {
  return guarded(bank, [&]() -> int32_t {
    if (!bank) return KNH_ERR_INVALID_ARGUMENT;
    if (!out) return bank->fail(KNH_ERR_INVALID_ARGUMENT, "null output");
    return bank->process(n_blocks, bank->block_size, 0, frame_clock, out, nullptr, nullptr, out_flags, nullptr, true);
  });
}
int32_t knh_bank_process_blocks_device(knh_bank* bank, uint32_t n_blocks, uint64_t frame_clock, void* out_device, void* hip_stream) {
  return guarded(bank, [&]() -> int32_t {
    if (!bank) return KNH_ERR_INVALID_ARGUMENT;
    return bank->process(n_blocks, bank->block_size, 0, frame_clock, nullptr, out_device, nullptr, nullptr, hip_stream, false);
  });
}
int32_t knh_bank_process_blocks_device_add(knh_bank* bank, uint32_t n_blocks, uint64_t frame_clock, void* out_device, void* hip_stream) {
  return guarded(bank, [&]() -> int32_t {
    if (!bank) return KNH_ERR_INVALID_ARGUMENT;
    return bank->process(n_blocks, bank->block_size, 0, frame_clock, nullptr, out_device, nullptr, nullptr, hip_stream, false, true);
  });
}
int32_t knh_bank_process_blocks_begin(knh_bank* bank, uint32_t n_blocks, uint64_t frame_clock) {
  return guarded(bank, [&]() -> int32_t {
    if (!bank) return KNH_ERR_INVALID_ARGUMENT;
    if (!bank->initialised) return bank->fail(KNH_ERR_NOT_INITIALISED, "bank not initialised");
    if (bank->pipe_count == 2) return bank->fail(KNH_ERR_INVALID_ARGUMENT, "two launches are outstanding: fetch one with knh_bank_process_blocks_end first");
    if (n_blocks == 0 || n_blocks > 4096) return bank->fail(KNH_ERR_INVALID_ARGUMENT, "n_blocks must be in 1..4096");
    auto hip = [&](hipError_t e, const char* what) { return e == hipSuccess ? KNH_OK : bank->fail(KNH_ERR_DEVICE, std::string(what) + ": " + hipGetErrorString(e)); };
    int rc = hip(hipSetDevice(bank->device), "hipSetDevice");
    if (rc != KNH_OK) return rc;
    if (!bank->pipe_stream && (rc = hip(hipStreamCreateWithFlags(&bank->pipe_stream, hipStreamNonBlocking), "hipStreamCreate")) != KNH_OK) return rc;
    knh_bank::PipeSlot& p = bank->pipe[(bank->pipe_head + bank->pipe_count) % 2];
    const size_t bytes = static_cast<size_t>(n_blocks) * bank->desc.out_channels * bank->block_size * (bank->desc.sample_type == KNH_F64 ? 8 : 4);
    if (bytes > p.cap) {
      if (p.dev) (void)hipFree(p.dev);
      if (p.host) (void)hipHostFree(p.host);
      p.dev = p.host = nullptr;
      p.cap = 0;
      if ((rc = hip(hipMalloc(&p.dev, bytes), "hipMalloc")) != KNH_OK) return rc;
      if ((rc = hip(hipMemset(p.dev, 0, bytes), "hipMemset")) != KNH_OK) return rc;
      if ((rc = hip(hipHostMalloc(&p.host, bytes), "hipHostMalloc")) != KNH_OK) return rc;
      p.cap = bytes;
    }
    if (!p.done && (rc = hip(hipEventCreateWithFlags(&p.done, hipEventDisableTiming), "hipEventCreate")) != KNH_OK) return rc;
    p.bytes = bytes;
    rc = bank->process(n_blocks, bank->block_size, 0, frame_clock, nullptr, p.dev, nullptr, nullptr, bank->pipe_stream, false);
    if (rc != KNH_OK) return rc;
    if ((rc = bank->order_after_collective(bank->pipe_stream)) != KNH_OK) return rc;
    if ((rc = hip(hipSetDevice(bank->device), "hipSetDevice")) != KNH_OK) return rc;
    if ((rc = hip(hipMemcpyAsync(p.host, p.dev, bytes, hipMemcpyDeviceToHost, bank->pipe_stream), "hipMemcpyAsync")) != KNH_OK) return rc;
    if ((rc = hip(hipEventRecord(p.done, bank->pipe_stream), "hipEventRecord")) != KNH_OK) return rc;
    bank->pipe_count += 1;
    return KNH_OK;
  });
}
int32_t knh_bank_process_blocks_end(knh_bank* bank, void* out) {
  return guarded(bank, [&]() -> int32_t {
    if (!bank) return KNH_ERR_INVALID_ARGUMENT;
    if (!out) return bank->fail(KNH_ERR_INVALID_ARGUMENT, "null output");
    if (bank->pipe_count == 0) return bank->fail(KNH_ERR_INVALID_ARGUMENT, "no launch is outstanding (knh_bank_process_blocks_begin)");
    knh_bank::PipeSlot& p = bank->pipe[bank->pipe_head];
    if (hipSetDevice(bank->device) != hipSuccess || hipEventSynchronize(p.done) != hipSuccess) return bank->fail(KNH_ERR_DEVICE, "waiting for the launch failed");
    std::memcpy(out, p.host, p.bytes);
    bank->pipe_head = (bank->pipe_head + 1) % 2;
    bank->pipe_count -= 1;
    return KNH_OK;
  });
}
void* knh_device_malloc(size_t bytes, int32_t device) {
  if (device >= 0 && hipSetDevice(device) != hipSuccess) return nullptr;
  void* p = nullptr;
  if (hipMalloc(&p, bytes) != hipSuccess) return nullptr;
  if (hipMemset(p, 0, bytes) != hipSuccess) { (void)hipFree(p); return nullptr; }
  return p;
}
void knh_device_free(void* p) {
  if (p) (void)hipFree(p);
}
int32_t knh_device_read(void* dst_host, const void* src_device, size_t bytes, void* hip_stream) {
  return guarded(nullptr, [&]() -> int32_t {
    if (hipDeviceSynchronize() != hipSuccess) return KNH_ERR_DEVICE;
    (void)hip_stream;
    return hipMemcpy(dst_host, src_device, bytes, hipMemcpyDeviceToHost) == hipSuccess ? KNH_OK : KNH_ERR_DEVICE;
  });
}
int32_t knh_bank_param_apply_many_at(knh_bank* bank, uint32_t block_offset, size_t count, const uint32_t* voices, const uint32_t* stages,
                                     const uint32_t* params, const uint32_t* kinds, const double* fvalues, const int64_t* ivalues,
                                     const uint16_t* delays) {
  return guarded(bank, [&]() -> int32_t {
    if (!bank) return KNH_ERR_INVALID_ARGUMENT;
    if (count && (!voices || !stages || !params || !kinds)) return bank->fail(KNH_ERR_INVALID_ARGUMENT, "null array");
    return bank->apply_many(block_offset, count, voices, stages, params, kinds, fvalues, ivalues, delays);
  });
}
int32_t knh_bank_read_done_frames(knh_bank* bank, uint32_t* done_frames) {
  return guarded(bank, [&]() -> int32_t {
    if (!bank) return KNH_ERR_INVALID_ARGUMENT;
    return bank->read_done_frames(done_frames);
  });
}
void knh_jit_stats(uint64_t* memory_hits, uint64_t* disk_hits, uint64_t* helper_compiles, uint64_t* in_process_compiles) {
  const knh::JitStats st = knh::jit_stats();
  if (memory_hits) *memory_hits = st.memory_hits;
  if (disk_hits) *disk_hits = st.disk_hits;
  if (helper_compiles) *helper_compiles = st.helper_runs;
  if (in_process_compiles) *in_process_compiles = st.in_process;
}
const char* knh_bank_debug_signature(const knh_bank* bank) { return bank ? bank->debug_signature() : ""; }
int32_t knh_bank_debug_words(knh_bank* bank, uint32_t* out16) {
  return guarded(bank, [&]() -> int32_t {
    if (!bank || !out16) return KNH_ERR_INVALID_ARGUMENT;
    return bank->debug_read(out16);
  });
}
int32_t knh_bank_synchronize(knh_bank* bank) {
  return guarded(bank, [&]() -> int32_t {
    if (!bank) return KNH_ERR_INVALID_ARGUMENT;
    return bank->synchronize();
  });
}
int32_t knh_bank_timing_reset(knh_bank* bank, int32_t enable) {
  return guarded(bank, [&]() -> int32_t {
    if (!bank) return KNH_ERR_INVALID_ARGUMENT;
    return bank->timing_reset(enable);
  });
}
int32_t knh_bank_timing_read(knh_bank* bank, double* kernel_ms, uint64_t* launches) {
  return guarded(bank, [&]() -> int32_t {
    if (!bank) return KNH_ERR_INVALID_ARGUMENT;
    return bank->timing_read(kernel_ms, launches);
  });
}
int32_t knh_bank_collective_timing_read(knh_bank* bank, double* reduce_ms, uint64_t* reduces) {
  return guarded(bank, [&]() -> int32_t {
    if (!bank) return KNH_ERR_INVALID_ARGUMENT;
// ... 37 lines not shown
```

knaster_amd/csrc/bank_base.hpp:

```cpp
#pragma once

struct knh_bank {
  virtual ~knh_bank() {
    if (pipe_stream || pipe[0].dev || pipe[1].dev) (void)hipSetDevice(device);
    for (PipeSlot& p : pipe) {
      if (p.done) (void)hipEventDestroy(p.done);
      if (p.dev) (void)hipFree(p.dev);
      if (p.host) (void)hipHostFree(p.host);
    }
    if (pipe_stream) (void)hipStreamDestroy(pipe_stream);
  }
  struct PipeSlot { void* dev = nullptr; void* host = nullptr; hipEvent_t done = nullptr; size_t cap = 0, bytes = 0; };
  PipeSlot pipe[2];
  hipStream_t pipe_stream = nullptr;
  unsigned pipe_head = 0, pipe_count = 0;
  virtual int order_after_collective(void* ) { return KNH_OK; }
  std::vector<unsigned char> channel_block;
  std::string err;
  std::vector<std::string> warnings;
  knh_bank_desc desc{};
  std::vector<StageInfo> stages;
  int n_slots = 0, n_params_total = 0;
  bool initialised = false;
  uint32_t sample_rate = 0;
  size_t block_size = 0;
  int device = 0;

  virtual int set_ctor(uint32_t stage, uint32_t first, uint32_t count, const double* args, uint32_t n_args) = 0;
  virtual int set_buffer(uint32_t stage, const void* samples, size_t n_frames, double buffer_sample_rate) = 0;
  virtual int init(uint32_t sr, size_t bs) = 0;
  virtual int param_apply(uint32_t voice, uint32_t stage, uint32_t param, uint32_t kind, double f, int64_t i) = 0;
  virtual int set_delay(uint32_t voice, uint32_t stage, uint32_t param, uint16_t delay) = 0;
  virtual int call_at(uint32_t block_offset, bool is_delay, uint32_t voice, uint32_t stage, uint32_t param, uint32_t kind, double f,
                      int64_t i, uint16_t delay) = 0;
  virtual int check_call(uint32_t , uint32_t , uint32_t , uint32_t ) { return KNH_OK; }
  virtual int process(uint32_t n_blocks, size_t ftp, size_t offset, uint64_t clock, void* out_host, void* out_device,
                      void* voices_host, uint32_t* out_flags, void* stream, bool sync, bool accumulate = false) = 0;
  std::vector<uint32_t> range_scratch[4];
  std::vector<double> range_f;
  std::vector<int64_t> range_i;
  virtual int apply_range(uint32_t v0, uint32_t v1, uint32_t stage, uint32_t param, uint32_t kind, double f, int64_t iv) {
    const size_t n = v1 - v0;
    if (n == 0) return KNH_OK;
    range_scratch[0].resize(n);
    for (size_t k = 0; k < n; ++k) range_scratch[0][k] = v0 + static_cast<uint32_t>(k);
    range_scratch[1].assign(n, stage);
    range_scratch[2].assign(n, param);
    range_scratch[3].assign(n, kind);
    range_f.assign(n, f);
    range_i.assign(n, iv);
    return apply_many(0, n, range_scratch[0].data(), range_scratch[1].data(), range_scratch[2].data(), range_scratch[3].data(), range_f.data(), range_i.data(), nullptr);
  }
  virtual int apply_many(uint32_t block_offset, size_t count, const uint32_t* voices, const uint32_t* stgs, const uint32_t* params,
                         const uint32_t* kinds, const double* fvalues, const int64_t* ivalues, const uint16_t* delays) {
    int rc = KNH_OK;
    for (size_t k = 0; k < count; ++k) {
      if (delays && delays[k] > 0) {
        int r = check_call(voices[k], stgs[k], params[k], kinds[k]);
        if (r == KNH_OK) r = call_at(block_offset, true, voices[k], stgs[k], params[k], 0, 0.0, 0, delays[k]);
        if (r != KNH_OK) { rc = r; continue; }
      }
      int r = call_at(block_offset, false, voices[k], stgs[k], params[k], kinds[k], fvalues ? fvalues[k] : 0.0, ivalues ? ivalues[k] : 0, 0);
      if (r != KNH_OK) rc = r;
    }
    return rc;
  }
  virtual int set_input(uint32_t n_blocks, const void* host, const void* dev) = 0;
  virtual int read_done_frames(uint32_t* out) = 0;
  virtual int synchronize() = 0;
  virtual int debug_read(uint32_t* out16) = 0;
  virtual const char* debug_signature() const { return ""; }
  virtual int timing_reset(int enable) = 0;
  virtual int timing_read(double* ms, uint64_t* launches) = 0;
  virtual int collective_timing_read(double* ms, uint64_t* reduces) {
    if (ms) *ms = 0.0;
    if (reduces) *reduces = 0;
    return KNH_OK;
  }
  virtual uint32_t ranks() const { return 1; }
  virtual void resident_stats(uint64_t* calls, uint64_t* launches) { if (calls) *calls = 0; if (launches) *launches = 0; }
  virtual void resident_trace(uint64_t* five) { for (int k = 0; k < 5; ++k) five[k] = 0; }

  int fail(int code, const std::string& msg) {
    err = msg;
    return code;
  }
  void warn(const std::string& msg) {
    if (warnings.size() < 32) warnings.push_back(msg);
  }
};

#define KNH_HIP(expr)                                                                                      \
  do {                                                                                                     \
    hipError_t e_ = (expr);                                                                                \
    if (e_ != hipSuccess)                                                                                  \
      return fail(KNH_ERR_DEVICE, std::string(#expr) + ": " + hipGetErrorString(e_));                      \
  } while (0)
```

knaster_amd/csrc/voice_bank.hpp:

```cpp
#pragma once

namespace {

template <typename F>
struct Bank final : knh_bank {
  typedef typename knh_dev::WordOf<F>::type W;
  const knh::KernelEntry* entry = nullptr;
  const knh::PipeEntry* pipe = nullptr;
  bool pipe_pair = false;
  const knh::WideEntry* wide = nullptr;
  int wide_waves = 0;
  bool interp = false;
  std::vector<knh_dev::InterpOp> h_prog;
  knh_dev::InterpOp* d_prog = nullptr;
  unsigned interp_sigs = 0, interp_out = 0;
  const knh::JitKernel* frame_jit = nullptr;
  uint32_t* d_sin_slots = nullptr;
  unsigned frame_vpw = 1, n_sin = 0;
  uint64_t env_ranks = 0;
  const knh::JitKernel* jit = nullptr;
  int pipeline_level = 1;
  std::string signature;
  const char* debug_signature() const override { return signature.c_str(); }
  uint32_t nv = 0;
// ... 7 lines not shown
  std::vector<Shadow> shadow;
  double f2pi = 0.0;
  std::vector<uint16_t> next_delay;
  std::vector<std::pair<uint64_t, QueuedChange>> queued;
  struct SmoothState {
    bool linear = false;
    double current_value = 0, start_value = 0, end_value = 0;
    size_t duration_frames = 0, frames_elapsed = 0;
    uint8_t audio_rate = 0;
    bool done = true;
    double interpolated() const {
      double mix = static_cast<double>(frames_elapsed) / static_cast<double>(duration_frames);
      return (end_value - start_value) * mix + start_value;
    }
  };
  std::vector<std::vector<SmoothState>> smooth;
  std::vector<uint64_t> smooth_active;
  std::vector<std::vector<uint32_t>> smooth_mark;
  uint32_t smooth_epoch = 0;
  std::vector<HostEvent> pending;
  bool pending_needs_sort = false;
  struct RangeEvent { uint32_t v0, v1, frame, op, slot; uint64_t bits; size_t at; };
  std::vector<RangeEvent> pending_ranges, sent_ranges;
  uint32_t res_n_ranges = 0;
  void expand_ranges() {
    if (pending_ranges.empty()) return;
    size_t extra = 0;
    for (const RangeEvent& r : pending_ranges) extra += r.v1 - r.v0;
    std::vector<HostEvent> out;
    out.reserve(pending.size() + extra);
    size_t k = 0;
    auto emit = [&](const RangeEvent& r) { for (uint32_t v = r.v0; v < r.v1; ++v) out.push_back(HostEvent{v, r.frame, r.op, r.slot, r.bits}); };
    for (size_t i = 0; i < pending.size(); ++i) {
      while (k < pending_ranges.size() && pending_ranges[k].at <= i) emit(pending_ranges[k++]);
      out.push_back(pending[i]);
    }
    while (k < pending_ranges.size()) emit(pending_ranges[k++]);
    pending.swap(out);
    pending_ranges.clear();
  }
  bool res_ranges_ok() const { return jit ? jit_pipe : pipe != nullptr; }
  uint32_t frame_base = 0;
  struct Call { uint8_t is_delay; uint16_t delay; uint32_t voice, stage, param, kind; double f; int64_t i; };
  std::vector<std::vector<Call>> future;
  std::vector<std::vector<QRec>> qfuture;
  struct NodeQ { uint32_t epoch; uint16_t at; uint16_t taken : 15, blocked : 1; };
  std::vector<NodeQ> node_q;
  std::vector<int> wrapped_index;
  uint32_t n_wrapped = 0, q_epoch = 0;
  bool fastq(const StageInfo& S) const { return S.dcpb > 0 && !(S.flags & KNH_STAGE_FLAG_SMOOTH_PARAMS); }
  std::vector<QRec>& qblock(uint32_t block_offset) {
    if (qfuture.size() <= block_offset) qfuture.resize(block_offset + 1);
    return qfuture[block_offset];
  }
  std::vector<uint8_t> stage_dev;
  std::vector<uint8_t> dev_class;
  DevEventResolver resolver;
  static bool dev_resolvable_kind(uint16_t kind) {
    switch (kind) {
      case KNH_STAGE_SIN_WT: case KNH_STAGE_SIN_NUMERIC: case KNH_STAGE_MUL_ENV_ASR: case KNH_STAGE_MUL_ENV_AR:
      case KNH_STAGE_MUL_CONST: case KNH_STAGE_ADD_CONST: case KNH_STAGE_SUB_CONST: case KNH_STAGE_DIV_CONST: case KNH_STAGE_POW_CONST:
      case KNH_STAGE_WR_MUL: return true;
      default: return false;
    }
  }
  int push_rec(uint32_t block_offset, const QRec& r) {
    if (stage_dev[r.stage]) return resolver.push(block_offset, r);
    qblock(block_offset).push_back(r);
    return KNH_OK;
  }

  hipStream_t own_stream = nullptr;
  W* d_state = nullptr;
  float* d_sine = nullptr;
  double* d_seg_table = nullptr;
  uint32_t seg_max = 0;
  F* d_buffer = nullptr;
  std::vector<F> h_buffer;
  double buffer_sr = 0.0;
  std::vector<double> buf_start, buf_dur, buf_rate;
  double buf_base_rate = 0.0;
  void* d_delay = nullptr;
  uint32_t delay_stride = 0;
  std::vector<uint32_t> delay_len;
  std::vector<double> env_start;
  std::vector<uint32_t> env_nseg;
  F* d_partials = nullptr;
  F* d_out = nullptr;
  F* d_voices = nullptr;
  uint32_t* d_done = nullptr;
  uint32_t* d_flags = nullptr;
  uint32_t flags_parity = 0;
  uint32_t* flags_last = nullptr;
  hipStream_t flags_stream = nullptr;
  bool flags_stream_set = false;
  uint32_t* h_ev_start2[2] = {nullptr, nullptr};
  Event* h_events2[2] = {nullptr, nullptr};
  size_t h_events_cap2[2] = {0, 0};
  hipEvent_t list_done[2] = {nullptr, nullptr};
  bool list_busy[2] = {false, false};
  unsigned list_parity = 0;
  int list_in_use = -1;
  uint32_t* h_ev_start = nullptr;
  Event* h_events = nullptr;
  F* h_out = nullptr;
  uint32_t* h_done = nullptr;
  uint32_t* d_fold_count = nullptr;
  uint32_t done_epoch = 0;
  ResidentCall<F> resident;
  void resident_stats(uint64_t* calls, uint64_t* launches) override { resident.stats(calls, launches); }
  void resident_trace(uint64_t* five) override { resident.trace(five); }
  bool jit_pipe = false;
  bool res_possible() const {
    if (interp || uses_input || desc.mix_mode != KNH_MIX_TREE) return false;
    if ((nv + 63u) / 64u > 256u || block_size > 4096) return false;
    if (wide_waves != 0) return false;
    if (jit) return true;
    if (pipe) return !pipe_pair && pipe->form != 1  && pipe->gpw == 1;
    return entry != nullptr;
  }
  uint32_t res_tile_frames() const {
    if (jit && jit_pipe) return sizeof(F) == 8 ? 16u : 32u;
    if (jit || !pipe) return 64u;
    const bool big = pipe->long_tiles != 0;
    return sizeof(F) == 8 ? (big ? 32u : 16u) : (big ? 64u : 32u);
  }
  void fill_launch_args(VoiceKernelArgs<F>& a, uint32_t n_blocks, uint32_t fb, uint32_t fe) {
    a.state = d_state;
    a.stride = stride;
    a.n_voices = nv;
    a.env_ranks = env_ranks;
    a.block_size = static_cast<uint32_t>(block_size);
    a.n_blocks = n_blocks;
    a.frame_begin = fb;
    a.frame_end = fe;
    a.sine_table = d_sine;
    a.f2pi = f2pi;
    a.sample_rate = sample_rate;
    a.seg_table = d_seg_table;
    a.seg_max = seg_max;
    a.delay_ring = d_delay;
    a.delay_stride = delay_stride;
    a.buffer = d_buffer;
    a.buffer_frames = static_cast<uint32_t>(h_buffer.size());
    a.input = nullptr;
    a.in_channels = desc.in_channels;
    a.ev_start = nullptr;
    a.events = nullptr;
    a.partials = d_partials;
    a.voices_out = nullptr;
    a.done_frames = d_done;
    a.flags = d_flags;
    a.res = knh_dev::Resident{};
  }
  bool timing = false;
  std::vector<std::pair<hipEvent_t, hipEvent_t>> timing_pool;
  size_t timing_used = 0;
  double timing_ms = 0.0;
  uint64_t timing_launches = 0;

  ~Bank() override {
    if (device >= 0) (void)hipSetDevice(device);
    (void)resident.leave();
    if (own_stream) (void)hipStreamSynchronize(own_stream);
    resolver.quiesce();
    if (flags_stream_set && flags_stream != own_stream) (void)hipStreamSynchronize(flags_stream);
    void* dev_ptrs[] = {d_state, d_sine, d_seg_table, d_delay, d_buffer, d_partials, d_out, d_voices, d_done, d_flags, d_input, d_prog, d_sin_slots, d_fold_count};
    for (void* p : dev_ptrs)
      if (p) (void)hipFree(p);
    void* host_ptrs[] = {h_ev_start2[0], h_ev_start2[1], h_events2[0], h_events2[1], h_out, h_input, h_done};
    for (void* p : host_ptrs)
      if (p) (void)hipHostFree(p);
    for (hipEvent_t e : list_done)
      if (e) (void)hipEventDestroy(e);
    if (in_copied) (void)hipEventDestroy(in_copied);
    for (auto& p : timing_pool) {
      (void)hipEventDestroy(p.first);
      (void)hipEventDestroy(p.second);
    }
    if (own_stream) (void)hipStreamDestroy(own_stream);
  }

  int set_ctor(uint32_t stage, uint32_t first, uint32_t count, const double* args, uint32_t n_args) override {
    if (initialised) return fail(KNH_ERR_INVALID_ARGUMENT, "constructor arguments must be set before init");
    if (stage >= stages.size()) return fail(KNH_ERR_OUT_OF_RANGE, "stage out of range");
    if (static_cast<uint64_t>(first) + count > nv) return fail(KNH_ERR_OUT_OF_RANGE, "voice range out of range");
    if (stages[stage].kind == KNH_STAGE_MUL_ENVELOPE && stages[stage].n_ctor < 0) {
      if (n_args < 6 || (n_args - 4) % 2 != 0) return fail(KNH_ERR_INVALID_ARGUMENT, "Envelope takes 4 + 2 * n_max constructor arguments");
      stages[stage].n_ctor = static_cast<int>(n_args);
      ctor[stage].assign(static_cast<size_t>(nv) * n_args, 0.0);
    }
    if (static_cast<int>(n_args) != stages[stage].n_ctor) return fail(KNH_ERR_INVALID_ARGUMENT, "wrong number of constructor arguments");
    if (n_args && !args) return fail(KNH_ERR_INVALID_ARGUMENT, "null args");
    std::copy(args, args + static_cast<size_t>(count) * n_args, ctor[stage].begin() + static_cast<size_t>(first) * n_args);
    return KNH_OK;
  }

  int set_buffer(uint32_t stage, const void* samples, size_t n_frames, double sr) override {
    if (initialised) return fail(KNH_ERR_INVALID_ARGUMENT, "knh_bank_set_buffer comes before knh_bank_init");
    if (stage >= stages.size() || stages[stage].kind != KNH_STAGE_BUFFER_READER) return fail(KNH_ERR_INVALID_ARGUMENT, "not a BufferReader stage");
    if (!samples || n_frames == 0 || n_frames >= (1ull << 31) || !(sr > 0.0)) return fail(KNH_ERR_INVALID_ARGUMENT, "empty buffer or bad sample rate");
    h_buffer.assign(static_cast<const F*>(samples), static_cast<const F*>(samples) + n_frames);
    buffer_sr = sr;
    return KNH_OK;
  }

  F* d_input = nullptr;
  F* h_input = nullptr;
  uint32_t in_blocks_cap = 0, in_blocks_set = 0;
  const void* in_device = nullptr;
  bool in_host_pending = false;
  hipEvent_t in_copied = nullptr;
  bool in_copy_pending = false;
  bool uses_input = false;
  int set_input(uint32_t n_blocks, const void* host, const void* dev) override {
    if (!initialised) return fail(KNH_ERR_NOT_INITIALISED, "bank not initialised");
    if (desc.in_channels == 0) return fail(KNH_ERR_INVALID_ARGUMENT, "the bank has no input channels (knh_bank_desc.in_channels)");
    if (n_blocks == 0 || n_blocks > 4096 || (!host && !dev)) return fail(KNH_ERR_INVALID_ARGUMENT, "knh_bank_set_input: n_blocks in 1..4096 and a buffer");
    KNH_HIP(hipSetDevice(device));
    in_blocks_set = n_blocks;
    in_device = dev;
    in_host_pending = false;
    if (dev) return KNH_OK;
    const size_t elems = static_cast<size_t>(n_blocks) * desc.in_channels * block_size;
    if (n_blocks > in_blocks_cap) {
      KNH_HIP(hipDeviceSynchronize());
      if (d_input) KNH_HIP(hipFree(d_input));
      if (h_input) KNH_HIP(hipHostFree(h_input));
      d_input = nullptr; h_input = nullptr;
      KNH_HIP(hipMalloc(&d_input, elems * sizeof(F)));
      KNH_HIP(hipHostMalloc(&h_input, elems * sizeof(F)));
      in_blocks_cap = n_blocks;
    } else if (in_copy_pending) {
      KNH_HIP(hipEventSynchronize(in_copied));
      in_copy_pending = false;
    }
    std::memcpy(h_input, host, elems * sizeof(F));
    in_host_pending = true;
    return KNH_OK;
  }

  int init(uint32_t sr, size_t bs) override {
    if (initialised) return fail(KNH_ERR_INVALID_ARGUMENT, "already initialised");
    if (sr == 0 || bs == 0 || bs > 65535) return fail(KNH_ERR_INVALID_ARGUMENT, "sample_rate/block_size out of range (block_size <= 65535)");
    int ndev = knh_device_count();
    if (ndev <= 0) return fail(KNH_ERR_NO_DEVICE, "no gfx950 device visible; this engine has no CPU path");
    if (desc.device >= 0) device = desc.device;
    else KNH_HIP(hipGetDevice(&device));
    KNH_HIP(hipSetDevice(device));
    if (pipe && !pipe_pair && pipe->form != 0 && bs % (sizeof(F) == 4 ? 64u : 32u) != 0) pipe = knh::find_pipe(signature.c_str(), 1u);
    const unsigned n_groups = (nv + 63u) / 64u;
    {
      const char* ie = std::getenv("KNH_INTERP");
      bool can = !entry && bs <= 1024 && stages.size() <= 4096;
      for (const StageInfo& S : stages) can = can && S.flags == 0 && S.dcpb == 0 && S.ar_param == 0 && std::strchr("Wmasdvq*+-/", kKinds[S.kind].sig) != nullptr;
      if (can && !(ie && ie[0] == '0')) {
        if (!parse_frame_program(signature, stages, &h_prog, &interp_sigs, &interp_out)) return fail(KNH_ERR_UNSUPPORTED_CHAIN, "interpreter: malformed graph signature");
        if (knh::interp_lds_bytes(static_cast<unsigned>(h_prog.size()), static_cast<unsigned>(n_slots), interp_sigs, static_cast<unsigned>(bs), sizeof(F) == 8) <= 158u * 1024u)
          interp = true;
        const char* fj = std::getenv("KNH_FRAME_JIT");
        if (interp && !(fj && fj[0] == '0')) {
          const unsigned tpv = ((static_cast<unsigned>(bs) + 63u) / 64u) * 64u;
          const size_t nwp = (static_cast<size_t>(n_slots) + 3u) & ~size_t(3);
          unsigned vpw = std::max(1u, nv / 256u);
          vpw = std::min(vpw, 1024u / tpv);
          while (vpw > 1u && 65536u + vpw * nwp * sizeof(W) > 156u * 1024u) --vpw;
          if (65536u + vpw * nwp * sizeof(W) <= 156u * 1024u) {
            std::vector<knh::FrameOp> fops(h_prog.size());
            for (size_t k = 0; k < h_prog.size(); ++k) fops[k] = knh::FrameOp{h_prog[k].kind, h_prog[k].a, h_prog[k].b, h_prog[k].o, h_prog[k].slot};
            std::string why;
            frame_jit = knh::jit_frame_kernel(fops.data(), static_cast<unsigned>(fops.size()), interp_sigs, interp_out, static_cast<unsigned>(n_slots), vpw, tpv,
                                              sizeof(F) == 8, &why);
            if (frame_jit) frame_vpw = vpw;
            else warnings.push_back("frame-parallel kernel not built (" + why.substr(0, 300) + "): the interpreter runs the voice");
          }
        }
      }
    }
    env_ranks = envelope_task_ranks(signature, stages);
    const char* jp = std::getenv("KNH_JIT_PIPE");
    const unsigned jit_pipe_max = !entry && (sizeof(F) == 8 || signature.find_first_of("DYZ") != std::string::npos) ? 256u : 512u;
    const bool pipe_jit = !interp && !pipe && wide_waves == 0 && pipeline_level >= 1 && n_groups <= jit_pipe_max && !(jp && jp[0] == '0') &&
                          !(entry && n_groups == 1) && !signature_is_dag(signature);
    if (pipe_jit) {
      std::string why;
      unsigned cuts[2];
      const unsigned n_cuts = partition_chain(signature, cuts);
      jit = knh::jit_pipe_kernel(signature.c_str(), cuts, n_cuts, sizeof(F) == 8, desc.allow_fma != 0, &why);
      jit_pipe = jit != nullptr;
      if (!jit) return fail(why.rfind("JIT_CRASH: ", 0) == 0 ? KNH_ERR_INTERNAL : KNH_ERR_UNSUPPORTED_CHAIN, "run-time fusion of chain '" + signature + "' (pipelined) failed: " + why);
    } else if (!entry && !interp) {
      std::string why;
      unsigned jw = !signature_is_dag(signature) && n_groups > jit_pipe_max ? (n_groups <= 1024 ? 4u : 8u) : 1u;
      if (const char* e = std::getenv("KNH_JIT_WAVES")) { const int v = std::atoi(e); if ((v == 1 || v == 4 || v == 8 || v == 16) && !signature_is_dag(signature)) jw = static_cast<unsigned>(v); }
      if (sizeof(F) == 8 && jw == 16) jw = 8;
      jit = knh::jit_voice_kernel(signature.c_str(), sizeof(F) == 8, desc.allow_fma != 0, &why, jw);
      if (!jit) return fail(why.rfind("JIT_CRASH: ", 0) == 0 ? KNH_ERR_INTERNAL : KNH_ERR_UNSUPPORTED_CHAIN, "run-time fusion of chain '" + signature + "' failed: " + why);
    }
    sample_rate = sr;
    block_size = bs;
    stride = (static_cast<long>(nv) + 63) / 64 * 64;
    f2pi = 16384.0 * 65536.0 * (1.0 / static_cast<double>(sr));
    const F sr_as_f32 = static_cast<F>(static_cast<float>(sr));

    std::vector<W> st(static_cast<size_t>(n_slots) * stride, W(0));
    std::vector<double> seg_rows;
    auto slot = [&](int s, uint32_t v) -> W& { return st[static_cast<size_t>(s) * stride + v]; };
    auto fw = [](F x) { return static_cast<W>(to_bits(x)); };
    shadow.assign(stages.size(), Shadow{});
    for (size_t si = 0; si < stages.size(); ++si) {
      const StageInfo& S = stages[si];
      const double* ca = ctor[si].data();
      Shadow& sh = shadow[si];
      for (uint32_t v = 0; v < nv; ++v) {
        const double* a = ca + static_cast<size_t>(v) * S.n_ctor;
        switch (S.kind) {
          case KNH_STAGE_SIN_WT: {
            if (v == 0) sh.a.resize(nv);
            F freq = static_cast<F>(a[0]);
            sh.a[v] = freq;
// ... 103 lines not shown
            const double step = a[0] * (1.0 / static_cast<double>(sr));
            const uint64_t sb = to_bits(step);
            slot(S.slot_base + 0, v) = 0;
            slot(S.slot_base + 1, v) = 0;
            slot(S.slot_base + 2, v) = static_cast<W>(static_cast<uint32_t>(sb));
            slot(S.slot_base + 3, v) = static_cast<W>(static_cast<uint32_t>(sb >> 32));
          } break;
          case KNH_STAGE_SAFETY_LIMITER: break;
          case KNH_STAGE_INPUT: {
            uses_input = true;
            if (!(a[0] >= 0.0) || a[0] >= static_cast<double>(desc.in_channels)) return fail(KNH_ERR_INVALID_ARGUMENT, "KNH_STAGE_INPUT: channel is not below knh_bank_desc.in_channels");
            slot(S.slot_base, v) = static_cast<W>(static_cast<uint32_t>(a[0]));
          } break;
          case KNH_STAGE_MATH_ADD: case KNH_STAGE_MATH_SUB: case KNH_STAGE_MATH_MUL: case KNH_STAGE_MATH_DIV: case KNH_STAGE_MATH_POW: break;
          case KNH_STAGE_WHITE_NOISE: case KNH_STAGE_PINK_NOISE: case KNH_STAGE_BROWN_NOISE: {
            const uint64_t seed = a[0] >= 0.0 ? static_cast<uint64_t>(a[0]) : 0u;
            slot(S.slot_base + 0, v) = static_cast<W>(static_cast<uint32_t>(seed));
            slot(S.slot_base + 1, v) = static_cast<W>(static_cast<uint32_t>(seed >> 32));
            if (S.kind == KNH_STAGE_BROWN_NOISE) slot(S.slot_base + 2, v) = to_bits(F(0));
            if (S.kind == KNH_STAGE_PINK_NOISE) {
              slot(S.slot_base + 2, v) = 1u;
              for (int k = 3; k < 14; ++k) slot(S.slot_base + k, v) = to_bits(F(0));
            }
          } break;
          case KNH_STAGE_RANDOM_LIN: {
            uint64_t rng = (a[0] >= 0.0 ? static_cast<uint64_t>(a[0]) : 0u) * 94u + 53u;
            auto draw = [&rng]() {
              rng += 0x2d358dccaa6c78a5ull;
              const unsigned __int128 t = static_cast<unsigned __int128>(rng) * static_cast<unsigned __int128>(rng ^ 0x8bb84b93962eacc9ull);
              const uint32_t r = static_cast<uint32_t>(static_cast<uint64_t>(t) ^ static_cast<uint64_t>(t >> 64));
              const uint32_t bits = 0x3F800000u + (r >> 9);
              float f;
              std::memcpy(&f, &bits, 4);
              return f - 1.0f;
            };
            const F first = static_cast<F>(draw());
            const F inc = F(1) / static_cast<F>(sr);
            const F step = static_cast<F>(a[1]) * inc;
            const F old_target = first + F(0);
            const F second = static_cast<F>(draw());
            slot(S.slot_base + 0, v) = static_cast<W>(static_cast<uint32_t>(rng));
            slot(S.slot_base + 1, v) = static_cast<W>(static_cast<uint32_t>(rng >> 32));
            slot(S.slot_base + 2, v) = to_bits(old_target);
            slot(S.slot_base + 3, v) = to_bits(static_cast<F>(second - old_target));
            slot(S.slot_base + 4, v) = to_bits(F(0));
            slot(S.slot_base + 5, v) = to_bits(step);
          } break;
          case KNH_STAGE_POLYBLEP: {
            const F srf = static_cast<F>(sr);
            const F freq = static_cast<F>(a[1]);
            const F dt = freq != F(0) ? freq / srf : F(0);
            const uint64_t wf = a[0] >= 0.0 && a[0] < 14.0 ? static_cast<uint64_t>(a[0]) : 0u;
            slot(S.slot_base + 0, v) = fw(F(0));
            slot(S.slot_base + 1, v) = fw(dt);
            slot(S.slot_base + 2, v) = fw(F(0.5));
            slot(S.slot_base + 3, v) = static_cast<W>(wf);
            slot(S.slot_base + 4, v) = (dt * srf >= srf / F(4)) ? 1u : 0u;
          } break;
          case KNH_STAGE_ALLPASS_FB_DELAY:
          case KNH_STAGE_ALLPASS_DELAY: {
            if (v == 0) delay_len.assign(nv, 0u);
            const double secs_in = a[0];
            if (!(secs_in >= 0.0) || secs_in >= 4294967296.0) return fail(KNH_ERR_INVALID_ARGUMENT, "AllpassDelay: max delay out of range");
            const uint64_t whole = static_cast<uint64_t>(std::floor(secs_in));
            const uint64_t tes = sat_u32((secs_in - std::floor(secs_in)) * 282240000.0);
            const uint64_t nsamp = whole * sr + tes * static_cast<uint64_t>(sr) / 282240000ull;
            if (nsamp == 0) return fail(KNH_ERR_INVALID_ARGUMENT, "AllpassDelay: the ring would be empty (the reference takes a remainder by zero)");
            if (nsamp >= (1ull << 30)) return fail(KNH_ERR_INVALID_ARGUMENT, "AllpassDelay: max delay too long");
            delay_len[v] = static_cast<uint32_t>(nsamp);
            slot(S.slot_base + 0, v) = 0;
            slot(S.slot_base + 1, v) = 0;
            slot(S.slot_base + 2, v) = static_cast<W>(nsamp);
            slot(S.slot_base + 3, v) = v;
            slot(S.slot_base + 4, v) = fw(F(1));
            slot(S.slot_base + 5, v) = fw(F(1));
            slot(S.slot_base + 6, v) = fw(F(1));
            if (S.kind == KNH_STAGE_ALLPASS_FB_DELAY) slot(S.slot_base + 7, v) = fw(F(0));
          } break;
          case KNH_STAGE_SAMPLE_DELAY: {
            if (v == 0) delay_len.assign(nv, 0u);
            const double secs_in = a[0];
            if (!(secs_in >= 0.0) || secs_in >= 4294967296.0) return fail(KNH_ERR_INVALID_ARGUMENT, "SampleDelay: max delay out of range");
            const uint32_t whole = static_cast<uint32_t>(std::floor(secs_in));
            const uint32_t tes = sat_u32((secs_in - std::floor(secs_in)) * 282240000.0);
            const double secs = static_cast<double>(whole) + static_cast<double>(tes) / 282240000.0;
            const double nf = secs * static_cast<double>(sr);
            if (!(nf >= 1.0)) return fail(KNH_ERR_INVALID_ARGUMENT, "SampleDelay: the ring would be empty (the reference divides by zero)");
            if (nf >= 1073741824.0) return fail(KNH_ERR_INVALID_ARGUMENT, "SampleDelay: max delay too long");
            const uint32_t len = static_cast<uint32_t>(nf);
            delay_len[v] = len;
            slot(S.slot_base + 0, v) = 0;
            slot(S.slot_base + 1, v) = len;
            slot(S.slot_base + 2, v) = len;
            slot(S.slot_base + 3, v) = v;
          } break;
          case KNH_STAGE_WR_POWI:
            slot(S.slot_base, v) = static_cast<W>(static_cast<uint32_t>(static_cast<int32_t>(a[0])));
            break;
          case KNH_STAGE_PAN2: {
            float gl, gr;
            pan2_gains(static_cast<float>(a[0]), &gl, &gr);
            slot(S.slot_base + 0, v) = fw(static_cast<F>(gl));
            slot(S.slot_base + 1, v) = fw(static_cast<F>(gr));
          } break;
          default:
            slot(S.slot_base, v) = fw(static_cast<F>(a[0]));
            break;
        }
      }
    }
    KNH_HIP(hipStreamCreateWithFlags(&own_stream, hipStreamNonBlocking));
    KNH_HIP(hipMalloc(&d_state, st.size() * sizeof(W)));
    KNH_HIP(hipMemcpy(d_state, st.data(), st.size() * sizeof(W), hipMemcpyHostToDevice));
    {
      std::vector<float> table(16384);
      const double PI = 3.14159265358979323846;
      for (int i = 0; i < 16384; ++i) table[i] = static_cast<float>(std::sin((static_cast<double>(i) / 16384.0) * PI * 2.0));
      KNH_HIP(hipMalloc(&d_sine, 16384 * sizeof(float)));
      KNH_HIP(hipMemcpy(d_sine, table.data(), 16384 * sizeof(float), hipMemcpyHostToDevice));
    }
    if (!h_buffer.empty()) {
      KNH_HIP(hipMalloc(&d_buffer, h_buffer.size() * sizeof(F)));
      KNH_HIP(hipMemcpy(d_buffer, h_buffer.data(), h_buffer.size() * sizeof(F), hipMemcpyHostToDevice));
    }
    if (!delay_len.empty()) {
      uint32_t mx = 0;
      for (uint32_t l : delay_len) mx = std::max(mx, l);
      delay_stride = (mx + 3u) & ~3u;
      const size_t bytes = (static_cast<size_t>(nv) + 1) * delay_stride * sizeof(F) + 4096;
      size_t free_b = 0, total_b = 0;
      KNH_HIP(hipMemGetInfo(&free_b, &total_b));
      if (bytes > free_b) return fail(KNH_ERR_DEVICE, "SampleDelay: the delay rings do not fit in device memory");
      KNH_HIP(hipMalloc(&d_delay, bytes));
      KNH_HIP(hipMemset(d_delay, 0, bytes));
    }
    if (!seg_rows.empty()) {
      KNH_HIP(hipMalloc(&d_seg_table, seg_rows.size() * sizeof(double)));
      KNH_HIP(hipMemcpy(d_seg_table, seg_rows.data(), seg_rows.size() * sizeof(double), hipMemcpyHostToDevice));
    }
    const size_t n_waves = interp ? nv : (nv + 63) / 64;
    if (interp) {
      KNH_HIP(hipMalloc(&d_prog, h_prog.size() * sizeof(knh_dev::InterpOp)));
      KNH_HIP(hipMemcpy(d_prog, h_prog.data(), h_prog.size() * sizeof(knh_dev::InterpOp), hipMemcpyHostToDevice));
      std::vector<uint32_t> sins;
      for (const knh_dev::InterpOp& op : h_prog)
        if (op.kind == knh_dev::INTERP_SIN_WT) sins.push_back(op.slot);
      n_sin = static_cast<unsigned>(sins.size());
      KNH_HIP(hipMalloc(&d_sin_slots, std::max<size_t>(1, sins.size()) * sizeof(uint32_t)));
      if (!sins.empty()) KNH_HIP(hipMemcpy(d_sin_slots, sins.data(), sins.size() * sizeof(uint32_t), hipMemcpyHostToDevice));
    }
    pan = !signature.empty() && stages.back().kind == KNH_STAGE_PAN2;
    fold_planes = pan ? 2u : 1u;
    KNH_HIP(hipMalloc(&d_partials, fold_planes * n_waves * bs * sizeof(F)));
    KNH_HIP(hipMalloc(&d_out, desc.out_channels * bs * sizeof(F)));
    KNH_HIP(hipMemset(d_out, 0, desc.out_channels * bs * sizeof(F)));
    KNH_HIP(hipMalloc(&d_done, static_cast<size_t>(nv) * sizeof(uint32_t)));
    KNH_HIP(hipMemset(d_done, 0xFF, static_cast<size_t>(nv) * sizeof(uint32_t)));
    KNH_HIP(hipMalloc(&d_flags, 48 * sizeof(uint32_t)));
    KNH_HIP(hipMemset(d_flags, 0, 48 * sizeof(uint32_t)));
    for (int b = 0; b < 2; ++b) {
      KNH_HIP(hipHostMalloc(&h_ev_start2[b], (static_cast<size_t>(nv) + 2) * sizeof(uint32_t)));
      h_events_cap2[b] = std::max<size_t>(2048, 2 * static_cast<size_t>(nv));
      KNH_HIP(hipHostMalloc(&h_events2[b], h_events_cap2[b] * sizeof(Event)));
      KNH_HIP(hipEventCreateWithFlags(&list_done[b], hipEventDisableTiming));
    }
    KNH_HIP(hipHostMalloc(&h_out, desc.out_channels * bs * sizeof(F) + 2 * sizeof(uint32_t), hipHostMallocMapped | hipHostMallocCoherent));
    KNH_HIP(hipHostMalloc(&h_done, 64, hipHostMallocMapped | hipHostMallocCoherent));
    std::memset(h_done, 0, 64);
    KNH_HIP(hipMalloc(&d_fold_count, sizeof(uint32_t)));
    KNH_HIP(hipMemset(d_fold_count, 0, sizeof(uint32_t)));
    if (desc.mix_mode == KNH_MIX_LEFT_FOLD) KNH_HIP(ensure_voices());
    bool any_wrapped = false;
    for (auto& S : stages) any_wrapped = any_wrapped || S.dcpb > 0;
    if (any_wrapped) next_delay.assign(static_cast<size_t>(n_params_total) * nv, 0);
    wrapped_index.assign(stages.size(), -1);
    n_wrapped = 0;
    for (size_t si = 0; si < stages.size(); ++si)
      if (fastq(stages[si])) wrapped_index[si] = static_cast<int>(n_wrapped++);
    node_q.assign(static_cast<size_t>(nv) * n_wrapped, NodeQ{0u, 0, 0, 0});
    {
      const char* de = std::getenv("KNH_DEV_EVENTS");
      stage_dev.assign(stages.size(), 0);
      std::vector<knh_dev::DevStage> ds(stages.size());
      int n_dev = 0;
      for (size_t si = 0; si < stages.size(); ++si) {
        const StageInfo& S = stages[si];
        const bool on = fastq(S) && dev_resolvable_kind(S.kind) && n_dev < 8 && !(de && de[0] == '0') && S.slot_base < 65536 && n_params_total < 65536;
        ds[si] = knh_dev::DevStage{S.kind, S.dcpb, static_cast<unsigned short>(S.slot_base), static_cast<unsigned short>(S.param_base), S.flags, S.ar_param,
                                   static_cast<short>(on ? n_dev : -1), 0};
        if (on) { stage_dev[si] = 1; ++n_dev; }
      }
      dev_class.assign(stages.size() * 8u, 0);
      for (size_t si = 0; si < stages.size(); ++si)
        if (stage_dev[si])
          for (int pp = 0; pp < stages[si].n_params && pp < 8; ++pp) dev_class[si * 8u + pp] = static_cast<uint8_t>(1 + expected_value_kind(stages[si].kind, pp));
      if (n_dev > 0) {
        const int rc = resolver.init(DevEventResolver::Setup{this, nv, static_cast<uint32_t>(n_params_total), static_cast<uint32_t>(bs), sr, sizeof(F) == 8, f2pi}, ds);
        if (rc != KNH_OK) return rc;
      }
    }
    smooth.assign(stages.size(), {});
    smooth_mark.assign(stages.size(), {});
    for (size_t si = 0; si < stages.size(); ++si)
      if (stages[si].flags & KNH_STAGE_FLAG_SMOOTH_PARAMS) {
        smooth[si].assign(static_cast<size_t>(nv) * stages[si].n_params, SmoothState{});
        smooth_mark[si].assign(nv, 0u);
      }
    can_finish = chain_can_finish(stages);
    {
      typename ResidentCall<F>::Setup rs{};
      rs.bank = this;
      rs.own_stream = own_stream;
      rs.n_rows = (nv + 63u) / 64u;
      rs.fold_planes = fold_planes;
      rs.out_channels = desc.out_channels;
      rs.block_size = static_cast<uint32_t>(bs);
      rs.tile_frames = res_tile_frames();
      rs.can_finish = can_finish;
      rs.ev_start = h_ev_start2;
      rs.events = h_events2;
      rs.launch_voice = [this](const knh_dev::Resident& r) {
        VoiceKernelArgs<F> a;
        fill_launch_args(a, 1, 0, static_cast<uint32_t>(block_size));
        a.flags = d_flags + 32;
        a.res = r;
        return launch_voice(a, (nv + 63) / 64, own_stream);
      };
      resident.setup(rs);
    }
    initialised = true;
    return KNH_OK;
  }
  bool can_finish = false;
  bool pan = false;
  F* stage_out = nullptr;
  unsigned fold_planes = 1;
  hipError_t ensure_voices() {
    if (d_voices) return hipSuccess;
    return hipMalloc(&d_voices, static_cast<size_t>(fold_planes) * nv * block_size * sizeof(F));
  }

  int check_target(uint32_t voice, uint32_t stage, uint32_t param) {
    if (!initialised) return fail(KNH_ERR_NOT_INITIALISED, "bank not initialised");
    if (voice >= nv) return fail(KNH_ERR_OUT_OF_RANGE, "voice out of range");
    if (stage >= stages.size()) return fail(KNH_ERR_OUT_OF_RANGE, "stage out of range");
    if (param >= static_cast<uint32_t>(stages[stage].n_params)) return fail(KNH_ERR_OUT_OF_RANGE, "parameter index out of range");
    return KNH_OK;
  }
  int set_delay(uint32_t voice, uint32_t stage, uint32_t param, uint16_t delay) override {
    int rc = check_target(voice, stage, param);
    if (rc != KNH_OK) return rc;
    const StageInfo& S = stages[stage];
    if (S.dcpb == 0) {
      warn("Parameter delay set, but the stage is not wrapped in WrPreciseTiming; no effect");
      return KNH_OK;
    }
    if (fastq(S)) {
      QRec r{};
      r.voice = voice; r.delay = delay; r.stage = static_cast<uint16_t>(stage); r.param = static_cast<uint8_t>(param); r.kb = 0x10u;
      return push_rec(0, r);
    }
    next_delay[static_cast<size_t>(S.param_base + param) * nv + voice] = delay;
    return KNH_OK;
  }
  int param_apply(uint32_t voice, uint32_t stage, uint32_t param, uint32_t kind, double f, int64_t i) override {
    int rc = check_target(voice, stage, param);
    if (rc != KNH_OK) return rc;
    const StageInfo& S = stages[stage];
    if (!kind_ok(S, param, kind)) return fail(KNH_ERR_WRONG_VALUE_KIND, "parameter value kind does not match the parameter type");
    if (fastq(S) && frame_base == 0) {
      return push_rec(0, make_qrec(voice, stage, param, kind, f, i, 0, false));
    }
    if (S.dcpb > 0) {
      uint16_t d = next_delay[static_cast<size_t>(S.param_base + param) * nv + voice];
      if (d != 0) {
        queued.emplace_back(static_cast<uint64_t>(voice) * stages.size() + stage, QueuedChange{d, param, kind, f, i});
        return KNH_OK;
      }
    }
    deliver(voice, stage, param, kind, f, i, frame_base);
    return KNH_OK;
  }
  static QRec make_qrec(uint32_t voice, uint32_t stage, uint32_t param, uint32_t kind, double f, int64_t i, uint16_t delay, bool arm) {
    QRec r{};
    r.voice = voice; r.delay = delay; r.stage = static_cast<uint16_t>(stage); r.param = static_cast<uint8_t>(param);
    r.kb = static_cast<uint8_t>((kind & 15u) | (arm ? 0x10u : 0u) | 0x20u);
    if (kind == KNH_VALUE_FLOAT) r.v.f = f; else r.v.i = i;
    return r;
  }
  static bool kind_ok(const StageInfo& S, uint32_t param, uint32_t kind) {
    const int want = expected_value_kind(S.kind, param);
    if (static_cast<int>(kind) == want) return true;
    return kind == KNH_VALUE_SMOOTHING && (S.flags & KNH_STAGE_FLAG_SMOOTH_PARAMS) && want == KNH_VALUE_FLOAT;
  }
  void deliver(uint32_t voice, uint32_t stage, uint32_t param, uint32_t kind, double f, int64_t iv, uint32_t frame) {
    const StageInfo& S = stages[stage];
    if (!(S.flags & KNH_STAGE_FLAG_SMOOTH_PARAMS) || (kind != KNH_VALUE_FLOAT && kind != KNH_VALUE_SMOOTHING)) {
      apply_now(voice, stage, param, f, iv, frame, pending);
      return;
    }
    SmoothState& st = smooth[stage][static_cast<size_t>(voice) * S.n_params + param];
    if (kind == KNH_VALUE_SMOOTHING) {
      if (iv == 0) {
        if (st.linear) {
          double cv = st.interpolated();
          st = SmoothState{};
// ... 572 lines not shown
      KNH_HIP(hipEventSynchronize(list_done[lb]));
      list_busy[lb] = false;
    }
    if (total > h_events_cap2[lb]) {
      { int rl = resident.leave(); if (rl != KNH_OK) return rl; }
      size_t cap = std::max<size_t>(total, 1024) * 2;
      if (h_events2[lb]) KNH_HIP(hipHostFree(h_events2[lb]));
      h_events2[lb] = nullptr;
      KNH_HIP(hipHostMalloc(&h_events2[lb], cap * sizeof(Event)));
      h_events_cap2[lb] = cap;
    }
    h_ev_start = h_ev_start2[lb];
    h_events = h_events2[lb];
    list_in_use = static_cast<int>(lb);
    if (!pending_ranges.empty()) {
      for (size_t j = 0; j < pending_ranges.size(); ++j) {
        const RangeEvent& r = pending_ranges[j];
        Event& d = h_events[2 * j];
        d.frame = r.frame;
        d.slot_op = (r.slot & 0xFFFFFFu) | (r.op << 24);
        d.bits = r.bits;
        Event& w = h_events[2 * j + 1];
        w.frame = r.v0;
        w.slot_op = r.v1;
        w.bits = 0;
      }
      res_n_ranges = static_cast<uint32_t>(pending_ranges.size());
      sent_ranges.swap(pending_ranges);
      pending_ranges.clear();
      finish();
      *have_events = true;
      return KNH_OK;
    }
    uint32_t* start = h_ev_start;
    bool in_voice_order = true;
    {
      uint32_t prev = 0;
      for (const HostEvent& e : pending) { if (e.voice < prev) { in_voice_order = false; break; } prev = e.voice; }
    }
    if (in_voice_order) {
      uint32_t v_next = 0, i = 0;
      for (const HostEvent& e : pending) {
        while (v_next <= e.voice) start[v_next++] = i;
        Event& d = h_events[i++];
        d.frame = e.frame;
        d.slot_op = (e.slot & 0xFFFFFFu) | (e.op << 24);
        d.bits = e.bits;
      }
      while (v_next <= nv) start[v_next++] = i;
    } else {
    std::fill(start, start + nv + 2, 0u);
    for (const HostEvent& e : pending) start[e.voice + 2]++;
    for (uint32_t v = 0; v < nv; ++v) start[v + 2] += start[v + 1];
    for (const HostEvent& e : pending) {
      Event& d = h_events[start[e.voice + 1]++];
      d.frame = e.frame;
      d.slot_op = (e.slot & 0xFFFFFFu) | (e.op << 24);
      d.bits = e.bits;
    }
    }
    if (pending_needs_sort) {
      for (uint32_t v = 0; v < nv; ++v) {
        Event* b = h_events + h_ev_start[v];
        Event* e = h_events + h_ev_start[v + 1];
        auto by_frame = [](const Event& x, const Event& y) { return x.frame < y.frame; };
        if (e - b > 1 && !std::is_sorted(b, e, by_frame)) std::stable_sort(b, e, by_frame);
      }
    }
    (void)s;
    finish();
    *have_events = true;
    return KNH_OK;
  }

  int process(uint32_t n_blocks, size_t ftp, size_t offset, uint64_t , void* out_host, void* out_device, void* voices_host,
              uint32_t* out_flags, void* stream, bool sync, bool accumulate) override {
    if (accumulate && !out_device) return fail(KNH_ERR_INVALID_ARGUMENT, "accumulation needs a device output buffer");
    if (!initialised) return fail(KNH_ERR_NOT_INITIALISED, "bank not initialised");
    if (offset + ftp > block_size) return fail(KNH_ERR_INVALID_ARGUMENT, "block_start_offset + frames_to_process exceeds block_size");
    if (n_blocks == 0 || n_blocks > 4096) return fail(KNH_ERR_INVALID_ARGUMENT, "n_blocks must be in 1..4096");
    if (n_blocks > 1 && (offset != 0 || ftp != block_size)) return fail(KNH_ERR_INVALID_ARGUMENT, "multi-block launches process whole blocks");
    if (n_blocks > 1 && voices_host) return fail(KNH_ERR_INVALID_ARGUMENT, "per-voice output is only available for single blocks");
    KNH_HIP(hipSetDevice(device));
    hipStream_t s = stream ? static_cast<hipStream_t>(stream) : own_stream;
    if (resolver.take_overflow()) warn("Not enough space for scheduled changes in WrPreciseTiming, change ignored");
    const uint32_t fb = static_cast<uint32_t>(offset), fe = static_cast<uint32_t>(offset + ftp);
    for (uint32_t b = 0; b < n_blocks; ++b) {
      frame_base = b * static_cast<uint32_t>(block_size);
      if (b > 0 && b < future.size()) {
        for (const Call& c : future[b]) {
          if (c.is_delay) set_delay(c.voice, c.stage, c.param, c.delay);
          else param_apply(c.voice, c.stage, c.param, c.kind, c.f, c.i);
        }
      }
      if (b < qfuture.size()) resolve_qrecs(qfuture[b], fb, fe);
      resolve_queues(fb, fe);
    }
    frame_base = 0;
    if (!qfuture.empty()) {
      if (qfuture.size() <= n_blocks) {
        for (auto& q : qfuture) q.clear();
      } else {
        std::rotate(qfuture.begin(), qfuture.begin() + n_blocks, qfuture.end());
        for (size_t k = qfuture.size() - n_blocks; k < qfuture.size(); ++k) qfuture[k].clear();
      }
    }
    const bool res_now = sync && out_host && !out_device && !voices_host && !stream && n_blocks == 1 && fe > fb && !accumulate && !timing &&
                         !resolver.pending() && res_possible() && resident.enabled() && resident.ready();
    bool have_events = false;
    int rc = upload_events(s, &have_events, n_blocks, res_now && res_ranges_ok());
    if (rc != KNH_OK) return rc;
    if (!future.empty()) {
      if (future.size() <= n_blocks) future.clear();
      else future.erase(future.begin(), future.begin() + n_blocks);
      if (!future.empty()) {
        std::vector<Call> due;
        due.swap(future[0]);
        for (const Call& c : due) {
          if (c.is_delay) set_delay(c.voice, c.stage, c.param, c.delay);
          else param_apply(c.voice, c.stage, c.param, c.kind, c.f, c.i);
        }
      }
    }
    {
      if (res_now) {
        const int held_list = list_in_use, call_list = have_events ? list_in_use : -1;
        if (call_list >= 0) { list_busy[call_list] = false; list_in_use = -1; }
        rc = resident.call(fb, fe, call_list, res_n_ranges, out_host, out_flags);
        if (rc != KNH_ERR_UNSUPPORTED_CHAIN) return rc;
        list_in_use = held_list;
        if (res_n_ranges) {
          pending_ranges.swap(sent_ranges);
          for (RangeEvent& r : pending_ranges) r.at = 0;
          rc = upload_events(s, &have_events, n_blocks, false);
          if (rc != KNH_OK) return rc;
        }
      }
      resident.sat_out();
      rc = resident.leave();
      if (rc != KNH_OK) return rc;
      ResidentCall<F>::make_room(device, this);
    }
    const bool want_voices = voices_host != nullptr || (desc.mix_mode == KNH_MIX_LEFT_FOLD) || stage_out != nullptr;
    if (desc.mix_mode == KNH_MIX_LEFT_FOLD && n_blocks > 1)
      return fail(KNH_ERR_INVALID_ARGUMENT, "KNH_MIX_LEFT_FOLD processes one block per call");
    if (stage_out && n_blocks > 1) return fail(KNH_ERR_INTERNAL, "a bank that feeds a following stage renders one block per launch");
    if (want_voices && !stage_out) KNH_HIP(ensure_voices());
    const unsigned n_waves = interp ? nv : (nv + 63) / 64;
    if (n_blocks > partials_blocks) {
      KNH_HIP(hipStreamSynchronize(s));
      KNH_HIP(hipFree(d_partials));
      d_partials = nullptr;
      KNH_HIP(hipMalloc(&d_partials, static_cast<size_t>(n_blocks) * fold_planes * n_waves * block_size * sizeof(F)));
      partials_blocks = n_blocks;
    }
    if (!out_device && n_blocks > out_blocks) {
      KNH_HIP(hipStreamSynchronize(s));
      KNH_HIP(hipFree(d_out));
      d_out = nullptr;
      KNH_HIP(hipMalloc(&d_out, static_cast<size_t>(n_blocks) * desc.out_channels * block_size * sizeof(F)));
      KNH_HIP(hipMemsetAsync(d_out, 0, static_cast<size_t>(n_blocks) * desc.out_channels * block_size * sizeof(F), s));
      if (h_out) KNH_HIP(hipHostFree(h_out));
      h_out = nullptr;
      KNH_HIP(hipHostMalloc(&h_out, static_cast<size_t>(n_blocks) * desc.out_channels * block_size * sizeof(F) + 2 * sizeof(uint32_t),
                            hipHostMallocMapped | hipHostMallocCoherent));
      out_blocks = n_blocks;
    }

    if (flags_stream_set && flags_stream != s) KNH_HIP(hipStreamSynchronize(flags_stream));
    flags_stream = s;
    flags_stream_set = true;
    uint32_t* const flags_now = d_flags + 16 * flags_parity;
    uint32_t* const flags_next = d_flags + 16 * (flags_parity ^ 1u);
    flags_parity ^= 1u;
    flags_last = flags_now;
    VoiceKernelArgs<F> a;
    fill_launch_args(a, n_blocks, fb, fe);
    if (uses_input) {
      if (in_blocks_set != n_blocks) return fail(KNH_ERR_INVALID_ARGUMENT, "a bank with KNH_STAGE_INPUT stages needs knh_bank_set_input for exactly the blocks of this call");
      if (in_device) {
        a.input = in_device;
      } else {
        if (in_host_pending) {
          KNH_HIP(hipMemcpyAsync(d_input, h_input, static_cast<size_t>(n_blocks) * desc.in_channels * block_size * sizeof(F), hipMemcpyHostToDevice, s));
          if (!in_copied) KNH_HIP(hipEventCreateWithFlags(&in_copied, hipEventDisableTiming));
          KNH_HIP(hipEventRecord(in_copied, s));
          in_copy_pending = true;
        }
        in_host_pending = false;
        a.input = d_input;
      }
      in_blocks_set = 0;
    }
    a.ev_start = have_events ? h_ev_start : nullptr;
    a.events = h_events;
    if (resolver.pending()) {
      DevEventResolver::Lists lists{};
      int r2 = resolver.resolve(s, n_blocks, fb, fe, have_events ? h_ev_start : nullptr, h_events, have_events ? h_ev_start[nv] : 0u, &lists);
      if (r2 != KNH_OK) return r2;
      a.ev_start = lists.ev_start;
      a.events = lists.events;
    }
    a.voices_out = want_voices ? (stage_out ? stage_out : d_voices) : nullptr;
    a.flags = flags_now;
    std::pair<hipEvent_t, hipEvent_t>* tp = nullptr;
    if (timing) {
      if (timing_used == timing_pool.size()) {
        if (timing_pool.size() >= 8192) {
          int r = timing_collect();
          if (r != KNH_OK) return r;
        } else {
          hipEvent_t e0, e1;
          KNH_HIP(hipEventCreate(&e0));
          KNH_HIP(hipEventCreate(&e1));
          timing_pool.emplace_back(e0, e1);
        }
      }
      tp = &timing_pool[timing_used++];
      KNH_HIP(hipEventRecord(tp->first, s));
    }
    if (interp) KNH_HIP(launch_interp(a, s));
    else KNH_HIP(launch_voice(a, n_waves, s));
    if (tp) KNH_HIP(hipEventRecord(tp->second, s));
    if (stage_out && interp)
      KNH_HIP(hipMemcpyAsync(stage_out, d_partials, static_cast<size_t>(nv) * block_size * sizeof(F), hipMemcpyDeviceToDevice, s));
    { int r2 = resolver.kernel_enqueued(s); if (r2 != KNH_OK) return r2; }
    if (have_events && list_in_use >= 0) {
      KNH_HIP(hipEventRecord(list_done[list_in_use], s));
      list_busy[list_in_use] = true;
      list_in_use = -1;
    }

    const bool hand_over = sync && out_host && !out_device && !voices_host && fe > fb;
    F* dst = out_device ? static_cast<F*>(out_device) : (hand_over ? h_out : d_out);
    knh_dev::HostDone hd{nullptr, nullptr, nullptr, 0u};
    if (hand_over) {
      done_epoch += 1;
      if (done_epoch == 0) done_epoch = 1;
      hd = knh_dev::HostDone{h_done, d_fold_count, flags_now, done_epoch};
    }
    const unsigned fold_channels = pan ? 1u : desc.out_channels;
    if (desc.mix_mode == KNH_MIX_LEFT_FOLD)
      KNH_HIP(launch_fold(false, interp ? d_partials : d_voices, nv, static_cast<unsigned>(block_size), fb, fe, dst, fold_channels, static_cast<unsigned>(block_size), fold_planes, accumulate, flags_next, s, hand_over ? &hd : nullptr));
    else
      KNH_HIP(launch_fold(true, d_partials, n_waves, static_cast<unsigned>(block_size), fb, fe, dst, fold_channels, static_cast<unsigned>(block_size), n_blocks * fold_planes, accumulate, flags_next, s, hand_over ? &hd : nullptr));

    if (!sync) return KNH_OK;
    const size_t blk_elems = desc.out_channels * block_size;
    const size_t out_bytes = static_cast<size_t>(n_blocks) * blk_elems * sizeof(F);
    uint32_t* h_flags = reinterpret_cast<uint32_t*>(reinterpret_cast<char*>(h_out) + static_cast<size_t>(out_blocks) * blk_elems * sizeof(F));
    if (hand_over) {
      volatile uint32_t* ep = h_done;
      for (uint64_t spin = 1;; ++spin) {
        if (__atomic_load_n(ep, __ATOMIC_ACQUIRE) == done_epoch) break;
        if ((spin & 0x3FFFu) == 0) {
          const hipError_t q = hipStreamQuery(s);
          if (q == hipSuccess) {
            if (__atomic_load_n(ep, __ATOMIC_ACQUIRE) == done_epoch) break;
            KNH_HIP(hipStreamSynchronize(s));
            if (__atomic_load_n(ep, __ATOMIC_ACQUIRE) != done_epoch) return fail(KNH_ERR_DEVICE, "the fold kernel finished without handing its block over");
            break;
          }
          if (q != hipErrorNotReady) return fail(KNH_ERR_DEVICE, std::string("hipStreamQuery: ") + hipGetErrorString(q));
        }
#if defined(__x86_64__)
        __builtin_ia32_pause();
#endif
      }
      h_flags[0] = h_done[1];
      h_flags[1] = h_done[2];
    } else {
      if (out_host) KNH_HIP(hipMemcpyAsync(h_out, dst, out_bytes, hipMemcpyDeviceToHost, s));
      KNH_HIP(hipMemcpyAsync(h_flags, flags_now, 2 * sizeof(uint32_t), hipMemcpyDeviceToHost, s));
      if (voices_host)
        KNH_HIP(hipMemcpyAsync(voices_host, interp ? d_partials : d_voices, static_cast<size_t>(fold_planes) * nv * block_size * sizeof(F), hipMemcpyDeviceToHost, s));
      KNH_HIP(hipStreamSynchronize(s));
    }
    if (out_host) {
      if (n_blocks > 1) {
        std::memcpy(out_host, h_out, out_bytes);
      } else {
        for (uint32_t c = 0; c < desc.out_channels; ++c)
          std::memcpy(static_cast<F*>(out_host) + c * block_size + offset, h_out + c * block_size + offset, ftp * sizeof(F));
      }
    }
    if (out_flags) *out_flags = done_flags(h_flags[0], h_flags[1], can_finish);
    return KNH_OK;
  }
  uint32_t partials_blocks = 1, out_blocks = 1;
  template <typename FF> hipError_t launch_frame(const VoiceKernelArgs<FF>& a, hipStream_t s) {
    struct { VoiceKernelArgs<FF> a; FF* rows; const uint32_t* sin_slots; uint32_t n_sin; } args{a, reinterpret_cast<FF*>(d_partials), d_sin_slots, n_sin};
    return knh::jit_frame_launch(frame_jit, &args, sizeof(args), (a.n_voices + frame_vpw - 1u) / frame_vpw, s);
  }
  hipError_t launch_interp(const VoiceKernelArgs<float>& a, hipStream_t s) {
    if (frame_jit) return launch_frame<float>(a, s);
    return knh::launch_interp_f32(a, d_prog, static_cast<unsigned>(h_prog.size()), static_cast<unsigned>(n_slots), interp_sigs, interp_out, reinterpret_cast<float*>(d_partials), s);
  }
  hipError_t launch_interp(const VoiceKernelArgs<double>& a, hipStream_t s) {
    if (frame_jit) return launch_frame<double>(a, s);
    return knh::launch_interp_f64(a, d_prog, static_cast<unsigned>(h_prog.size()), static_cast<unsigned>(n_slots), interp_sigs, interp_out, reinterpret_cast<double*>(d_partials), s);
  }
  hipError_t launch_voice(const VoiceKernelArgs<float>& a, unsigned n_waves, hipStream_t s) {
    if (jit) return knh::jit_launch(jit, &a, sizeof(a), n_waves, s);
    if (wide_waves == 4) return wide->f32_w4[desc.allow_fma ? 1 : 0](a, n_waves, s);
    if (wide_waves == 8) return wide->f32_w8[desc.allow_fma ? 1 : 0](a, n_waves, s);
    if (wide_waves == 16) return wide->f32_w16[desc.allow_fma ? 1 : 0](a, n_waves, s);
    if (pipe) return pipe->f32[desc.allow_fma ? 1 : 0](a, n_waves, s);
    return entry->f32[desc.allow_fma ? 1 : 0](a, n_waves, s);
  }
  hipError_t launch_voice(const VoiceKernelArgs<double>& a, unsigned n_waves, hipStream_t s) {
    if (jit) return knh::jit_launch(jit, &a, sizeof(a), n_waves, s);
    if (wide_waves == 4) return wide->f64_w4[desc.allow_fma ? 1 : 0](a, n_waves, s);
    if (wide_waves == 8) return wide->f64_w8[desc.allow_fma ? 1 : 0](a, n_waves, s);
    if (wide_waves == 16) return wide->f64_w16[desc.allow_fma ? 1 : 0](a, n_waves, s);
    if (pipe) return pipe->f64[desc.allow_fma ? 1 : 0](a, n_waves, s);
    return entry->f64[desc.allow_fma ? 1 : 0](a, n_waves, s);
  }
  static hipError_t launch_fold(bool tree, const float* rows, unsigned n, unsigned len, unsigned fb, unsigned fe, float* out, unsigned ch, unsigned os, unsigned nb, bool acc, uint32_t* zf, hipStream_t s, const knh_dev::HostDone* hd) {
    return knh::launch_fold_f32(tree, rows, n, len, fb, fe, out, ch, os, nb, acc, zf, s, hd);
  }
  static hipError_t launch_fold(bool tree, const double* rows, unsigned n, unsigned len, unsigned fb, unsigned fe, double* out, unsigned ch, unsigned os, unsigned nb, bool acc, uint32_t* zf, hipStream_t s, const knh_dev::HostDone* hd) {
    return knh::launch_fold_f64(tree, rows, n, len, fb, fe, out, ch, os, nb, acc, zf, s, hd);
  }

  int read_done_frames(uint32_t* out) override {
    if (!initialised) return fail(KNH_ERR_NOT_INITIALISED, "bank not initialised");
    if (!out) return fail(KNH_ERR_INVALID_ARGUMENT, "null output");
    { int rl = resident.leave(); if (rl != KNH_OK) return rl; }
    KNH_HIP(hipSetDevice(device));
    KNH_HIP(hipStreamSynchronize(own_stream));
    KNH_HIP(hipMemcpy(out, d_done, static_cast<size_t>(nv) * sizeof(uint32_t), hipMemcpyDeviceToHost));
    return KNH_OK;
  }
  int debug_read(uint32_t* out16) override {
    if (!initialised) return fail(KNH_ERR_NOT_INITIALISED, "bank not initialised");
    { int rl = resident.leave(); if (rl != KNH_OK) return rl; }
    KNH_HIP(hipSetDevice(device));
    KNH_HIP(hipDeviceSynchronize());
    KNH_HIP(hipMemcpy(out16, flags_last ? flags_last : d_flags, 16 * sizeof(uint32_t), hipMemcpyDeviceToHost));
    return KNH_OK;
  }
  int synchronize() override {
    if (!initialised) return fail(KNH_ERR_NOT_INITIALISED, "bank not initialised");
    { int rl = resident.leave(); if (rl != KNH_OK) return rl; }
    KNH_HIP(hipSetDevice(device));
    KNH_HIP(hipDeviceSynchronize());
    return KNH_OK;
  }
  int timing_collect() {
    KNH_HIP(hipDeviceSynchronize());
    for (size_t k = 0; k < timing_used; ++k) {
      float ms = 0.f;
      KNH_HIP(hipEventElapsedTime(&ms, timing_pool[k].first, timing_pool[k].second));
      timing_ms += ms;
      timing_launches += 1;
    }
    timing_used = 0;
    return KNH_OK;
  }
  int timing_reset(int enable) override {
    if (!initialised) return fail(KNH_ERR_NOT_INITIALISED, "bank not initialised");
    { int rl = resident.leave(); if (rl != KNH_OK) return rl; }
    KNH_HIP(hipSetDevice(device));
    int rc = timing_collect();
    if (rc != KNH_OK) return rc;
    timing_ms = 0.0;
    timing_launches = 0;
    timing = enable != 0;
    return KNH_OK;
  }
  int timing_read(double* ms, uint64_t* launches) override {
    if (!initialised) return fail(KNH_ERR_NOT_INITIALISED, "bank not initialised");
    KNH_HIP(hipSetDevice(device));
    int rc = timing_collect();
    if (rc != KNH_OK) return rc;
    if (ms) *ms = timing_ms;
    if (launches) *launches = timing_launches;
    return KNH_OK;
  }
};

}
```

knaster_amd/csrc/voice_chain.hpp:

```cpp
#pragma once
#include "voice_stages.hpp"

namespace knh_dev {

template <typename F, bool FMA, int BASE, typename... S> struct Chain;
template <typename F, bool FMA, int BASE>
struct Chain<F, FMA, BASE> {
  static constexpr int kSlots = BASE;
  static constexpr bool kUsesSine = false;
  static constexpr bool kPan = false;
  static constexpr u64 kParamBits = 0ull, kNopOkBits = 0ull;
  static constexpr bool kBinds = false;
  static constexpr bool kUsesRing = false;
  template <int T> __device__ __forceinline__ void tick_tile_sw(const Chain&, u32, u64, F (&)[T], const Ctx&, u32) {}
  __device__ __forceinline__ void pan_gains(F&, F&) const {}
  template <typename W> __device__ __forceinline__ void load(const W*, long) {}
  template <typename W> __device__ __forceinline__ void store(W*, long) const {}
  __device__ __forceinline__ F tick(F x, const Ctx&, u32) { return x; }
  template <int T> __device__ __forceinline__ void tick_tile(F (&)[T], const Ctx&, u32) {}
#ifdef KNH_DAG_STAMPS
  template <int T> __device__ __forceinline__ void tick_tile_stamped(F (&)[T], const Ctx&, u32, u64*, u64&) {}
#endif
  __device__ __forceinline__ void on_event(u32, u32, u64, u32) {}
  __device__ __forceinline__ bool last_env_stopped(bool dflt) const { return dflt; }
// ... 204 lines not shown
      rest.template collect_done_ranked<J + 1>(ranks, best_rank, best);
    } else {
      rest.template collect_done_ranked<J>(ranks, best_rank, best);
    }
  }
  __device__ __forceinline__ void pan_gains(F& l, F& rg) const {
    if constexpr (IsPan<S0>::value) { l = r.l; rg = r.r; }
    else rest.pan_gains(l, rg);
  }
  __device__ __forceinline__ void on_event(u32 op, u32 slot, u64 bits, u32 frame) {
    if (slot >= (u32)BASE && slot < (u32)(BASE + S0::kSlots)) S0::template on_event<F>(r, op, slot - BASE, bits, frame);
    else rest.on_event(op, slot, bits, frame);
  }
  __device__ __forceinline__ bool last_env_stopped(bool dflt) const {
    if constexpr (S0::kIsEnv) return rest.last_env_stopped(S0::template is_stopped<F>(r));
    else return rest.last_env_stopped(dflt);
  }
  __device__ __forceinline__ void begin_block(u32 frame_begin, const Ctx& c) {
    if constexpr (S0::kNeedsBind) S0::template bind<F>(r, c);
    if constexpr (S0::kIsEnv && S0::kHasSeg) r.seg = frame_begin;
    rest.begin_block(frame_begin, c);
  }
};
template <typename... S> struct SlotCount { static constexpr int value = 0; };
template <typename S0, typename... S> struct SlotCount<S0, S...> { static constexpr int value = SlotCount<S...>::value; };
template <int R> struct SlotCount<Slots<R>> { static constexpr int value = R; };
template <bool DAG, typename F, bool FMA, typename... S> struct ChainSelect { typedef Chain<F, FMA, 0, S...> type; };
template <typename F, bool FMA, typename... S> struct ChainSelect<true, F, FMA, S...> { typedef DagChain<F, FMA, 0, SlotCount<S...>::value, 0, S...> type; };

struct Resident {
  const u64* bell;
  u64* relay;
  u64* rows;
  u64* wg_flags;
  const u32* ev_start[2];
  const Event* events[2];
  u64 idle_ticks;
  u32* host_started;
  u32 first_epoch;
  u32 max_tiles;
  u32 bell_is_device;
};
__device__ __forceinline__ u32 res_tag(u32 epoch, u32 tile) { return (epoch << 8) | (tile & 0xFFu); }
__device__ __forceinline__ void res_put(u64* g, u32 data, u32 tag) { __hip_atomic_store(g, (u64)data | ((u64)tag << 32), __ATOMIC_RELAXED, __HIP_MEMORY_SCOPE_AGENT); }
__device__ __forceinline__ u64 res_get(const u64* g) { return __hip_atomic_load(g, __ATOMIC_RELAXED, __HIP_MEMORY_SCOPE_AGENT); }
__device__ __forceinline__ void res_put_host(u64* g, u32 data, u32 tag) { __hip_atomic_store(g, (u64)data | ((u64)tag << 32), __ATOMIC_RELAXED, __HIP_MEMORY_SCOPE_SYSTEM); }
__device__ __forceinline__ void res_put_host_sample(u64* g, float v, u32 tag) { res_put_host(g, __builtin_bit_cast(u32, v), tag); }
__device__ __forceinline__ void res_put_host_sample(u64* g, double v, u32 tag) {
  const u64 b = __builtin_bit_cast(u64, v);
  res_put_host(g, (u32)b, tag);
  res_put_host(g + 1, (u32)(b >> 32), tag);
}
template <typename F> struct ResWords { static constexpr int value = sizeof(F) == 8 ? 2 : 1; };
__device__ __forceinline__ void res_put_sample(u64* g, float v, u32 tag) { res_put(g, __builtin_bit_cast(u32, v), tag); }
__device__ __forceinline__ void res_put_sample(u64* g, double v, u32 tag) {
  const u64 b = __builtin_bit_cast(u64, v);
  res_put(g, (u32)b, tag);
  res_put(g + 1, (u32)(b >> 32), tag);
}
enum : u32 { RES_RELAY_RANGES = 16 };
enum : u64 { RES_EPOCH_MASK = 0xFFFFFFull, RES_HAS_EVENTS = 1ull << 56, RES_LIST = 1ull << 57, RES_LEAVE = 1ull << 58, RES_RANGES_SHIFT = 59, RES_RANGES_MASK = 0xFull };
struct ResCall {
  u32 epoch, frame_begin, frame_end;
  bool has_events, leave;
  u32 list;
  u32 n_ranges;
};
__device__ __forceinline__ ResCall res_unpack(u64 c) {
  ResCall r;
  r.epoch = (u32)(c & RES_EPOCH_MASK);
  r.frame_begin = (u32)((c >> 24) & 0xFFFFu);
  r.frame_end = (u32)((c >> 40) & 0xFFFFu);
  r.has_events = (c & RES_HAS_EVENTS) != 0ull;
  r.list = (c & RES_LIST) ? 1u : 0u;
  r.leave = (c & RES_LEAVE) != 0ull;
  r.n_ranges = (u32)((c >> RES_RANGES_SHIFT) & RES_RANGES_MASK);
  return r;
}
struct ResStaged { u32 first, count; };
__device__ __forceinline__ ResStaged res_stage_events(const Resident& r, const ResCall& call, Event* stage, u32 cap, u32 gv0, u32 gnv, u32 tid, u32 n_threads) {
  ResStaged st{0u, 0u};
  if (!call.has_events || cap == 0u) return st;
  if (call.n_ranges) {
    st.count = 2u * call.n_ranges;
    if (st.count > cap) { st.count = 0u; return st; }
    const u64* src = r.relay + RES_RELAY_RANGES;
    u64* dst = reinterpret_cast<u64*>(stage);
    for (u32 i = tid; i < 2u * st.count; i += n_threads) dst[i] = __hip_atomic_load(&src[i], __ATOMIC_RELAXED, __HIP_MEMORY_SCOPE_AGENT);
    __builtin_amdgcn_fence(__ATOMIC_RELEASE, "workgroup");
    __builtin_amdgcn_s_barrier();
    __builtin_amdgcn_fence(__ATOMIC_ACQUIRE, "workgroup");
    return st;
  } else {
    const u32* evs = r.ev_start[call.list];
    st.first = __hip_atomic_load(&evs[gv0], __ATOMIC_RELAXED, __HIP_MEMORY_SCOPE_SYSTEM);
    st.count = __hip_atomic_load(&evs[gv0 + gnv], __ATOMIC_RELAXED, __HIP_MEMORY_SCOPE_SYSTEM) - st.first;
  }
  if (st.count > cap) st.count = 0u;
  typedef u32 U4 __attribute__((ext_vector_type(4)));
  const volatile U4* src = reinterpret_cast<const volatile U4*>(r.events[call.list] + st.first);
  U4* dst = reinterpret_cast<U4*>(stage);
  for (u32 i = tid; i < st.count; i += n_threads) { const U4 e = src[i]; dst[i] = e; }
  __builtin_amdgcn_fence(__ATOMIC_RELEASE, "workgroup");
  __builtin_amdgcn_s_barrier();
  __builtin_amdgcn_fence(__ATOMIC_ACQUIRE, "workgroup");
  return st;
}
__device__ __forceinline__ ResCall res_wait(const Resident& r, u32 expect, u32* slot, int wave_all, int lane) {
  if (wave_all == 0) {
    const bool leader = blockIdx.x == 0u;
    u64 c = 0ull;
    if (lane == 0) {
      if (leader && expect == r.first_epoch) __hip_atomic_store(r.host_started, r.first_epoch, __ATOMIC_RELAXED, __HIP_MEMORY_SCOPE_SYSTEM);
      const u64 t0 = __builtin_amdgcn_s_memrealtime();
      const u64 patience = leader ? r.idle_ticks : 2ull * r.idle_ticks + 5000000ull;
      const bool from_bell = leader || r.bell_is_device != 0u;
      for (;;) {
        c = from_bell ? __hip_atomic_load(r.bell, __ATOMIC_RELAXED, __HIP_MEMORY_SCOPE_SYSTEM) : __hip_atomic_load(r.relay, __ATOMIC_RELAXED, __HIP_MEMORY_SCOPE_AGENT);
        if ((u32)(c & RES_EPOCH_MASK) == expect) break;
        if (!leader && from_bell) {
          const u64 l = __hip_atomic_load(r.relay, __ATOMIC_RELAXED, __HIP_MEMORY_SCOPE_AGENT);
          if ((l & RES_LEAVE) && (u32)(l & RES_EPOCH_MASK) == expect) { c = l; break; }
        }
        if (__builtin_amdgcn_s_memrealtime() - t0 > patience) { c = RES_LEAVE | (u64)expect; break; }
        __builtin_amdgcn_s_sleep(1);
      }
    }
    if (leader) {
      const u32 lo = __builtin_amdgcn_readfirstlane((u32)c), hi = __builtin_amdgcn_readfirstlane((u32)(c >> 32));
      const u64 cw = (u64)lo | ((u64)hi << 32);
      const ResCall call = res_unpack(cw);
      if (!call.leave && call.has_events && call.n_ranges) {
        const u64* src = reinterpret_cast<const u64*>(r.events[call.list]);
        if ((u32)lane < 4u * call.n_ranges)
          __hip_atomic_store(r.relay + RES_RELAY_RANGES + lane, __hip_atomic_load(&src[lane], __ATOMIC_RELAXED, __HIP_MEMORY_SCOPE_SYSTEM), __ATOMIC_RELAXED, __HIP_MEMORY_SCOPE_AGENT);
        __builtin_amdgcn_fence(__ATOMIC_RELEASE, "agent");
      }
      if (lane == 0) {
        __hip_atomic_store(r.relay, c, __ATOMIC_RELAXED, __HIP_MEMORY_SCOPE_AGENT);
        __hip_atomic_store(reinterpret_cast<u64*>(r.host_started + 4), __builtin_amdgcn_s_memrealtime(), __ATOMIC_RELAXED, __HIP_MEMORY_SCOPE_SYSTEM);
      }
    }
    if (lane == 0) {
      slot[0] = (u32)c;
      slot[1] = (u32)(c >> 32);
    }
  }
  __builtin_amdgcn_fence(__ATOMIC_RELEASE, "workgroup");
  __builtin_amdgcn_s_barrier();
  __builtin_amdgcn_fence(__ATOMIC_ACQUIRE, "workgroup");
  const u64 c = (u64)slot[0] | ((u64)slot[1] << 32);
  return res_unpack(c);
}
template <typename F>
struct VoiceKernelArgs {
  typename WordOf<F>::type* state;
  long stride;
  u32 n_voices;
  u32 block_size;
  u32 n_blocks;
  u32 frame_begin, frame_end;
  const float* sine_table;
  double f2pi;
  u32 sample_rate;
  const double* seg_table;
  u32 seg_max;
  void* delay_ring;
  u32 delay_stride;
  const void* buffer;
  u32 buffer_frames;
  const void* input;
  u32 in_channels;
  const u32* ev_start;
  const Event* events;
  F* partials;
  F* voices_out;
  u64 env_ranks;
  u32* done_frames;
  u32* flags;
  Resident res;
};

constexpr int kWave = 64;
constexpr int kTile = 8;

template <typename F, int N, bool FULL>
__device__ __forceinline__ F tree_reduce(F (&t)[N], u32 unit, u32 nv) {
  static_assert((N & (N - 1)) == 0, "a power of two");
#pragma unroll
  for (int w = N, step = 1; w > 1; w >>= 1, step <<= 1) {
#pragma unroll
    for (int i = 0; i < w / 2; ++i) {
      const F sum = t[2 * i] + t[2 * i + 1];
      t[i] = (FULL || (u32)((2 * i + 1) * step) * unit < nv) ? sum : t[2 * i];
    }
  }
  return t[0];
}
template <typename F, int N, bool FULL, int B>
__device__ __forceinline__ F tree_cols(const F* col, int st, u32 nv) {
  constexpr int BB = B < N ? B : N;
  F node[N / BB];
#pragma unroll
  for (int c = 0; c < N / BB; ++c) {
    F t[BB];
#pragma unroll
    for (int k = 0; k < BB; ++k) t[k] = col[(c * BB + k) * st];
    node[c] = tree_reduce<F, BB, FULL>(t, 1u, nv > (u32)(c * BB) ? nv - (u32)(c * BB) : 0u);
  }
  return tree_reduce<F, N / BB, FULL>(node, (u32)BB, nv);
}
template <typename F, int N, bool FULL, int B>
__device__ __forceinline__ void tree_cols_pan(const F* col, int st, const F* gl, const F* gr, int gst, u32 nv, F& left, F& right) {
  constexpr int BB = B < N ? B : N;
  F nl[N / BB], nr[N / BB];
#pragma unroll
  for (int c = 0; c < N / BB; ++c) {
    F t[BB], p[BB];
#pragma unroll
    for (int k = 0; k < BB; ++k) t[k] = col[(c * BB + k) * st];
    const u32 sub = nv > (u32)(c * BB) ? nv - (u32)(c * BB) : 0u;
#pragma unroll
    for (int k = 0; k < BB; ++k) p[k] = t[k] * gl[(c * BB + k) * gst];
    nl[c] = tree_reduce<F, BB, FULL>(p, 1u, sub);
#pragma unroll
    for (int k = 0; k < BB; ++k) p[k] = t[k] * gr[(c * BB + k) * gst];
    nr[c] = tree_reduce<F, BB, FULL>(p, 1u, sub);
  }
  left = tree_reduce<F, N / BB, FULL>(nl, (u32)BB, nv);
  right = tree_reduce<F, N / BB, FULL>(nr, (u32)BB, nv);
}
template <typename F, int B>
__device__ __forceinline__ F fold_group(const F* col, int st, u32 nv) {
  return nv == 64u ? tree_cols<F, 64, true, B>(col, st, nv) : tree_cols<F, 64, false, B>(col, st, nv);
}
template <typename F, int B>
__device__ __forceinline__ void fold_group_pan(const F* col, int st, const F* gl, const F* gr, int gst, u32 nv, F& l, F& r) {
  if (nv == 64u) tree_cols_pan<F, 64, true, B>(col, st, gl, gr, gst, nv, l, r);
  else tree_cols_pan<F, 64, false, B>(col, st, gl, gr, gst, nv, l, r);
}

template <typename F>
struct ResServerArgs {
  const u64* relay;
  const u64* rows;
  const u64* wg_flags;
  u64* group_rows;
  u64* group_flags;
  u64* host_out;
  const u64* bell;
  u32* host_done;
  u64 idle_ticks;
  u32 first_epoch, n_rows, planes, out_channels, block_size, tile_frames;
};
template <typename F> __device__ __forceinline__ bool res_read_sample(const u64* g, u32 tag, F& out);
template <> __device__ __forceinline__ bool res_read_sample<float>(const u64* g, u32 tag, float& out) {
  const u64 w = res_get(g);
  out = __builtin_bit_cast(float, (u32)w);
  return (u32)(w >> 32) == tag;
}
template <> __device__ __forceinline__ bool res_read_sample<double>(const u64* g, u32 tag, double& out) {
  const u64 lo = res_get(g), hi = res_get(g + 1);
  out = __builtin_bit_cast(double, (u64)(u32)lo | ((u64)(u32)hi << 32));
  return (u32)(lo >> 32) == tag && (u32)(hi >> 32) == tag;
}
template <typename F>
__global__ void __launch_bounds__(256, 3) res_fold_server(ResServerArgs<F> a) {
  constexpr int W = ResWords<F>::value;
  constexpr u32 NW = 4u;
  const u32 lane = threadIdx.x & 63u, wv = threadIdx.x >> 6;
  const u32 n_g = (a.n_rows + 31u) / 32u;
  const bool root = blockIdx.x == n_g;
  const bool alone = n_g == 1u;
  if (root && alone) return;
  const bool writes_host = root || alone;
  const u32 g = blockIdx.x;
  const u32 in_g = root ? n_g : (a.n_rows - g * 32u < 32u ? a.n_rows - g * 32u : 32u);
  u32 expect = a.first_epoch;
  const u64 patience = 2ull * a.idle_ticks + 5000000ull;
  if (blockIdx.x == 0u && threadIdx.x == 0u) __hip_atomic_store(&a.host_done[5], a.first_epoch, __ATOMIC_RELAXED, __HIP_MEMORY_SCOPE_SYSTEM);
  __builtin_amdgcn_s_setprio(0);
  for (;;) {
    u64 c;
    {
      const u64 t0 = __builtin_amdgcn_s_memrealtime();
      for (;;) {
        c = a.bell ? __hip_atomic_load(a.bell, __ATOMIC_RELAXED, __HIP_MEMORY_SCOPE_SYSTEM) : __hip_atomic_load(a.relay, __ATOMIC_RELAXED, __HIP_MEMORY_SCOPE_AGENT);
        if ((u32)(c & RES_EPOCH_MASK) == expect) break;
        if (a.bell) {
          const u64 l = __hip_atomic_load(a.relay, __ATOMIC_RELAXED, __HIP_MEMORY_SCOPE_AGENT);
          if ((l & RES_LEAVE) && (u32)(l & RES_EPOCH_MASK) == expect) { c = l; break; }
        }
        if (__builtin_amdgcn_s_memrealtime() - t0 > patience) { c = RES_LEAVE; break; }
        __builtin_amdgcn_s_sleep(1);
      }
    }
    const ResCall call = res_unpack(c);
    if (call.leave) return;
    expect = (expect + 1u) & (u32)RES_EPOCH_MASK;
    const u32 n_frames = call.frame_end - call.frame_begin;
    const u32 n_tiles = (n_frames + a.tile_frames - 1u) / a.tile_frames;
    const bool tracer = writes_host && lane == 0u;
    if (tracer && wv == 0u) __hip_atomic_store(reinterpret_cast<u64*>(a.host_done + 10), __builtin_amdgcn_s_memrealtime(), __ATOMIC_RELAXED, __HIP_MEMORY_SCOPE_SYSTEM);
    for (u32 t = wv; t <= n_tiles; t += NW) {
      const bool flags_pass = t == n_tiles;
      const u32 tag = res_tag(call.epoch, flags_pass ? 255u : t);
      const u32 rel = t * a.tile_frames;
      const u32 len = flags_pass ? 1u : (n_frames - rel < a.tile_frames ? n_frames - rel : a.tile_frames);
      const bool mine = lane < len;
      bool gave_up = false;
      for (u32 p = 0; p < (flags_pass ? 1u : a.planes); ++p) {
        const u64* base;
        long stride;
        if (flags_pass) { base = root ? a.group_flags : a.wg_flags + g * 32u; stride = 1; }
        else if (root) { base = a.group_rows + (((long)t * a.planes + p) * 8) * 64 * W; stride = 64 * W; }
        else { base = a.rows + (((long)t * a.planes + p) * a.n_rows + g * 32u) * 64 * W; stride = 64 * W; }
        const u64* const src = flags_pass ? base : base + (long)lane * W;
        if (writes_host && lane == 0u) __hip_atomic_store(&a.host_done[20 + wv], 0x100u | (t << 16) | (p << 12), __ATOMIC_RELAXED, __HIP_MEMORY_SCOPE_SYSTEM);
        if (p == 0u && !root) {
          const u64 tc = __builtin_amdgcn_s_memrealtime();
          for (;;) {
            bool there = false;
            if (lane < in_g) there = (u32)(res_get(base + (long)lane * stride) >> 32) == tag;
            if (__builtin_amdgcn_ballot_w64(there) != 0ull) break;
            if (__builtin_amdgcn_s_memrealtime() - tc > patience) { gave_up = true; break; }
            __builtin_amdgcn_s_sleep(4);
          }
          if (gave_up) break;
          if (tracer && t == 0u) __hip_atomic_store(reinterpret_cast<u64*>(a.host_done + 12), __builtin_amdgcn_s_memrealtime(), __ATOMIC_RELAXED, __HIP_MEMORY_SCOPE_SYSTEM);
          if (tracer && t + 1u == n_tiles) __hip_atomic_store(reinterpret_cast<u64*>(a.host_done + 14), __builtin_amdgcn_s_memrealtime(), __ATOMIC_RELAXED, __HIP_MEMORY_SCOPE_SYSTEM);
        }
        if (writes_host && lane == 0u) __hip_atomic_store(&a.host_done[20 + wv], 0x200u | (t << 16) | (p << 12), __ATOMIC_RELAXED, __HIP_MEMORY_SCOPE_SYSTEM);
        u64 w[32 * W];
        bool all = !mine;
        const u64 t0 = __builtin_amdgcn_s_memrealtime();
        while (__builtin_amdgcn_ballot_w64(!all) != 0ull) {
          if (!all) {
#pragma unroll
            for (int k = 0; k < 32; ++k) {
#pragma unroll
              for (int j = 0; j < W; ++j)
                w[k * W + j] = (u32)k < in_g && !(flags_pass && j > 0) ? res_get(src + (long)k * stride + j) : ((u64)tag << 32);
            }
            bool ok = true;
#pragma unroll
            for (int k = 0; k < 32 * W; ++k) ok = ok && (u32)(w[k] >> 32) == tag;
            all = ok;
          }
          if (__builtin_amdgcn_s_memrealtime() - t0 > patience) { gave_up = true; break; }
          if (__builtin_amdgcn_ballot_w64(!all) != 0ull) { if (root) __builtin_amdgcn_s_sleep(3); else __builtin_amdgcn_s_sleep(1); }
        }
        if (root && p == 0u && !gave_up) {
          if (tracer && t == 0u) __hip_atomic_store(reinterpret_cast<u64*>(a.host_done + 12), __builtin_amdgcn_s_memrealtime(), __ATOMIC_RELAXED, __HIP_MEMORY_SCOPE_SYSTEM);
          if (tracer && t + 1u == n_tiles) __hip_atomic_store(reinterpret_cast<u64*>(a.host_done + 14), __builtin_amdgcn_s_memrealtime(), __ATOMIC_RELAXED, __HIP_MEMORY_SCOPE_SYSTEM);
        }
        if (gave_up) break;
        if (!mine) continue;
        if (flags_pass) {
          u32 n_done = 0, n_run = 0;
#pragma unroll
          for (int k = 0; k < 32; ++k) {
            const u32 d = (u32)k < in_g ? (u32)w[k * W] : 0u;
            n_done += root ? (d & 0xFFFFu) : (d & 0xFFu);
            n_run += root ? (d >> 16) : ((d >> 8) & 0xFFu);
          }
          if (writes_host) {
            res_put_host(a.host_out + (long)a.planes * a.block_size * W, n_done | (n_run << 16), tag);
          } else {
            res_put(a.group_flags + g, n_done | (n_run << 16), tag);
          }
        } else {
          F v[32];
#pragma unroll
          for (int k = 0; k < 32; ++k) {
            if constexpr (W == 1) v[k] = (F)__builtin_bit_cast(float, (u32)w[k]);
            else v[k] = (F)__builtin_bit_cast(double, (u64)(u32)w[2 * k] | ((u64)(u32)w[2 * k + (W - 1)] << 32));
          }
          const F node = in_g == 32u ? tree_reduce<F, 32, true>(v, 1u, 32u) : tree_reduce<F, 32, false>(v, 1u, in_g);
          if (writes_host) {
            res_put_host_sample(a.host_out + ((long)p * a.block_size + call.frame_begin + rel + lane) * W, node, tag);
          } else {
            res_put_sample(a.group_rows + ((((long)t * a.planes + p) * 8 + g) * 64 + lane) * W, node, tag);
          }
        }
      }
      if (gave_up) return;
    }
    if (writes_host && lane == 0u) {
      __hip_atomic_store(&a.host_done[20 + wv], 0x300u, __ATOMIC_RELAXED, __HIP_MEMORY_SCOPE_SYSTEM);
      if ((n_tiles % NW) == wv) {
        __hip_atomic_store(reinterpret_cast<u64*>(a.host_done + 16), __builtin_amdgcn_s_memrealtime(), __ATOMIC_RELAXED, __HIP_MEMORY_SCOPE_SYSTEM);
        __hip_atomic_store(&a.host_done[0], call.epoch, __ATOMIC_RELAXED, __HIP_MEMORY_SCOPE_SYSTEM);
      }
// ... 492 lines not shown
```

knaster_amd/csrc/voice_pipe.hpp:

```cpp
#pragma once
#include "voice_chain.hpp"

namespace knh_dev {

template <typename... S> struct Group {};
template <int K, typename... S> struct Fan {};

template <typename G> struct GroupInfo;
template <typename... S> struct GroupInfo<Group<S...>> {
  static constexpr int slots = (0 + ... + S::kSlots);
  static constexpr bool uses_sine = (false || ... || S::kUsesSine);
  static constexpr bool uses_ring = (false || ... || S::kUsesRing);
  static constexpr bool has_env = (false || ... || S::kIsEnv);
  static constexpr bool pan = (false || ... || IsPan<S>::value);
  static constexpr int fan_for(int) { return 1; }
};
template <int K, typename... S> struct GroupInfo<Fan<K, S...>> {
  static constexpr int slots = (0 + ... + S::kSlots);
  static constexpr bool uses_sine = (false || ... || S::kUsesSine);
  static constexpr bool uses_ring = false;
  static constexpr bool has_env = false;
  static constexpr bool pan = false;
  static constexpr int fan_for(int T) { return K * 8 <= T ? K : (T >= 8 ? T / 8 : 1); }
  static_assert(((S::kMutableMask == 0u) && ...), "a Fan group's stages keep no state");
// ... 248 lines not shown
          while (next_frame < tile_end) {
            const u32 op = nxt.slot_op >> 24, slot = nxt.slot_op & 0xFFFFFFu, code = op & 0x7Fu;
            if (slot >= SLOT_LO && slot < SLOT_HI) {
              const u32 rel = nxt.frame - (base + n);
              if (sw == (u32)TW) sw = rel;
              bad = bad || sw != rel || slot >= 64u ||
                    !((code == EV_SET && ((ChainT::kParamBits >> (slot & 63u)) & 1ull)) || (code == EV_NOP && ((ChainT::kNopOkBits >> (slot & 63u)) & 1ull)));
              if (!bad) {
                cn.on_event(op, slot, nxt.bits, nxt.frame - base);
                touched |= 1ull << (slot & 63u);
                if (live && code == EV_SET) a.state[(long)slot * a.stride + voice] = (W)nxt.bits;
              }
            }
            ++ev_i;
            take_next();
          }
          if (__builtin_amdgcn_ballot_w64(bad) != 0) {
            ev_i = sv_i;
            nxt = sv_nxt;
            next_frame = sv_next_frame;
            return false;
          }
          const F* in_row = sh.edge + (long)Map::in_tile(I, g) * EdgeLayout<F, T>::tile + (long)lane * EdgeLayout<F, T>::stride + fo;
          for (u32 j0 = 0; j0 < (u32)TW; j0 += 8u) {
            F sub[8];
            if (I > 0) {
#pragma unroll
              for (int q = 0; q < 8 / VW; ++q) {
                const Vec v = reinterpret_cast<const Vec*>(in_row + j0)[q];
#pragma unroll
                for (int k = 0; k < VW; ++k) sub[q * VW + k] = v[k];
              }
            } else {
#pragma unroll
              for (int k = 0; k < 8; ++k) sub[k] = (F)0;
            }
            chain.template tick_tile_sw<8>(cn, sw - j0, touched, sub, ctx, n + j0);
#pragma unroll
            for (int q = 0; q < 8 / VW; ++q) {
              Vec v;
#pragma unroll
              for (int k = 0; k < VW; ++k) v[k] = sub[q * VW + k];
              reinterpret_cast<Vec*>(out_row + j0)[q] = v;
            }
          }
          return true;
        }()) {
        } else {
          const F* in_row = sh.edge + (long)Map::in_tile(I, g) * EdgeLayout<F, T>::tile + (long)lane * EdgeLayout<F, T>::stride + fo;
          for (u32 j0 = 0; j0 < m; j0 += 8u) {
            const u32 cnt = m - j0 < 8u ? m - j0 : 8u;
            F sub[8];
            if (I > 0) {
#pragma unroll
              for (int q = 0; q < 8 / VW; ++q) {
                const Vec v = reinterpret_cast<const Vec*>(in_row + j0)[q];
#pragma unroll
                for (int k = 0; k < VW; ++k) sub[q * VW + k] = v[k];
              }
            } else {
#pragma unroll
              for (int k = 0; k < 8; ++k) sub[k] = (F)0;
            }
#pragma unroll
            for (int k = 0; k < 8; ++k) {
              if ((u32)k < cnt) {
                apply_events_upto(base + n + j0 + (u32)k);
                sub[k] = chain.tick(sub[k], ctx, n + j0 + (u32)k);
              }
            }
#pragma unroll
            for (int q = 0; q < 8 / VW; ++q) {
              Vec v;
#pragma unroll
              for (int k = 0; k < VW; ++k) v[k] = sub[q * VW + k];
              reinterpret_cast<Vec*>(out_row + j0)[q] = v;
            }
          }
        }
        if constexpr (GroupInfo<G>::pan) {
          F gl = (F)0, gr = (F)0;
          chain.pan_gains(gl, gr);
          out_row[T] = gl;
          out_row[T + 1] = gr;
        }
#ifdef KNH_DAG_STAMPS
        asm volatile("s_waitcnt lgkmcnt(0)" ::: "memory");
        const u64 tf0 = __builtin_amdgcn_s_memtime();
#endif
        if constexpr (FOLDS) pipe_fold_tile<F, FMA, T, GroupInfo<G>::pan>(out_tile, a, lane, wave_global, n_waves_total, blk, n_tile, m_tile, v0, nv);
#ifdef KNH_DAG_STAMPS
        asm volatile("s_waitcnt lgkmcnt(0)" ::: "memory");
        busy_fold += __builtin_amdgcn_s_memtime() - tf0;
#endif
      }
#if defined(KNH_DAG_STAMPS) || defined(KNH_TILE_FENCES)
      asm volatile("" ::: "memory");
#endif
#ifdef KNH_DAG_STAMPS
      const u64 t2 = __builtin_amdgcn_s_memtime();
#endif
      if (++ti == tpb) {
        apply_events_upto(base + fend);
        ti = 0;
        ++blk;
        base += a.block_size;
        if (resident) {
          sh.res_marks[wave_all * 64 + lane] = chain.collect_done(0xFFFFFFFFu);
          if (GroupInfo<G>::has_env && I == LAST_ENV) sh.res_marks[15 * 64 + lane] = live && !chain.last_env_stopped(false) ? 1u : 0u;
        }
      }
#if defined(KNH_DAG_STAMPS) || defined(KNH_TILE_FENCES)
      asm volatile("s_waitcnt lgkmcnt(0)" ::: "memory");
#endif
#ifdef KNH_DAG_STAMPS
      const u64 t3 = __builtin_amdgcn_s_memtime();
      busy += t3 - t0;
      busy_out += t3 - t2;
#endif
    }
    pipe_barrier();
  }
#ifdef KNH_DAG_STAMPS
  if (wave_global == 0u && lane == 0) {
    const u64 d = (u64)(n_tiles > 0 ? n_tiles : 1);
    a.flags[4 + I] = (u32)(busy / d);
    if (8 + 2 * I + 1 < 16) { a.flags[8 + 2 * I] = (u32)(busy_in / d); a.flags[9 + 2 * I] = (u32)(busy_out / d); }
    if (FOLDS) { a.flags[14] = (u32)(busy_tick / d); a.flags[15] = (u32)(busy_fold / d); }
    else if (MODE != PIPE_FOLD && I == 1) { a.flags[14] = (u32)(busy_tick / d); a.flags[15] = (u32)((busy - busy_in - busy_out - busy_tick) / d); }
  }
#endif
  done_frame = chain.collect_done(0xFFFFFFFFu);
  if (!resident) break;
  }
  if (live) chain.store(a.state + voice, a.stride);
  if (!resident && GroupInfo<G>::has_env && I == LAST_ENV) {
    const bool running = live && !chain.last_env_stopped(false);
    const u64 br = __builtin_amdgcn_ballot_w64(running);
    if (lane == 0 && br) atomicAdd(&a.flags[1], (u32)__builtin_popcountll(br));
  }
  return done_frame;
}

template <typename F, bool FMA, int T, bool PAN>
__device__ __forceinline__ void pipe_fold_tile(const F* tile, const VoiceKernelArgs<F>& a, int lane, u32 wave_global, u32 n_waves_total,
                                               int blk, u32 n0, u32 len, u32 v0, u32 nv, u32 res_tile, u32 res_epoch) {
  constexpr int ST = EdgeLayout<F, T>::stride;
  if ((u32)lane < len) {
    const F* col = tile + lane;
    if constexpr (!PAN) {
      F* const row = a.partials + ((long)blk * n_waves_total + wave_global) * a.block_size + n0 + lane;
      const F sum = fold_group<F, 64>(col, ST, nv);
      if (a.res.bell) res_put_sample(a.res.rows + (((long)res_tile * n_waves_total + wave_global) * 64 + lane) * ResWords<F>::value, sum, res_tag(res_epoch, res_tile));
      else *row = sum;
      if (a.voices_out) {
        for (u32 v = 0; v < nv; ++v) a.voices_out[(long)(v0 + v) * a.block_size + n0 + lane] = col[v * ST];
      }
    } else {
      const F* gain = tile + T;
      F accl, accr;
      fold_group_pan<F, 64>(col, ST, gain, gain + 1, ST, nv, accl, accr);
      F* const rl = a.partials + (((long)blk * 2 + 0) * n_waves_total + wave_global) * a.block_size + n0 + lane;
      F* const rr = a.partials + (((long)blk * 2 + 1) * n_waves_total + wave_global) * a.block_size + n0 + lane;
      if (a.res.bell) {
        res_put_sample(a.res.rows + ((((long)res_tile * 2 + 0) * n_waves_total + wave_global) * 64 + lane) * ResWords<F>::value, accl, res_tag(res_epoch, res_tile));
        res_put_sample(a.res.rows + ((((long)res_tile * 2 + 1) * n_waves_total + wave_global) * 64 + lane) * ResWords<F>::value, accr, res_tag(res_epoch, res_tile));
      } else { *rl = accl; *rr = accr; }
      if (a.voices_out) {
        for (u32 v = 0; v < nv; ++v) {
          const F t = col[v * ST];
          a.voices_out[(long)(v0 + v) * a.block_size + n0 + lane] = t * gain[v * ST];
          a.voices_out[((long)a.n_voices + v0 + v) * a.block_size + n0 + lane] = t * gain[v * ST + 1];
        }
      }
    }
  }
}

template <typename F, bool FMA, int T, int MODE, int NG, bool PAN, int CHAINW, bool HAS_ENV>
__device__ __forceinline__ void pipe_run_mixer(const PipeShared<F>& sh, const VoiceKernelArgs<F>& a, int lane, u32 wave_global,
                                               u32 v0, u32 nv, int wave_all) {
  u32 fbeg = a.frame_begin, fend = a.frame_end;
  const bool resident = a.res.bell != nullptr;
  u32 res_expect = a.res.first_epoch;
  const u32 n_waves_total = (a.n_voices + 63u) / 64u;
  for (;;) {
  ResCall call;
  call.epoch = 0u;
  if (resident) {
    call = res_wait(a.res, res_expect, sh.res_slot, wave_all, lane);
    if (call.leave) break;
    res_expect = (res_expect + 1u) & (u32)RES_EPOCH_MASK;
    fbeg = call.frame_begin;
    fend = call.frame_end;
    (void)res_stage_events(a.res, call, sh.ev_stage, sh.ev_cap, v0, nv, (u32)(wave_all * 64 + lane), sh.n_threads);
  }
  const u32 n_frames = fend - fbeg;
  const int tpb = (int)((n_frames + T - 1) / T);
  const int n_tiles = tpb * (int)a.n_blocks;
  const int n_steps = n_tiles + NG;
  int blk = 0, ti = 0;
#ifdef KNH_DAG_STAMPS
  u64 busy = 0;
#endif
  for (int s = 0; s < n_steps; ++s) {
    const int g = s - NG;
    if (g >= 0 && g < n_tiles) {
#ifdef KNH_DAG_STAMPS
      const u64 t0 = __builtin_amdgcn_s_memtime();
#endif
      const u32 rel = (u32)ti * T;
      const u32 len = n_frames - rel < (u32)T ? n_frames - rel : (u32)T;
      const F* tile = sh.edge + (long)EdgeMap<MODE, NG>::mixer_tile(g) * EdgeLayout<F, T>::tile;
      pipe_fold_tile<F, FMA, T, PAN>(tile, a, lane, wave_global, n_waves_total, blk, fbeg + rel, len, v0, nv, (u32)g, call.epoch);
      if (resident && g == n_tiles - 1) {
        u32 n_done = 0u, n_run = 0u;
        if (HAS_ENV) {
          u32 d = 0xFFFFFFFFu;
#pragma unroll
          for (int w = 0; w < CHAINW; ++w) d = sh.res_marks[w * 64 + lane] != 0xFFFFFFFFu ? sh.res_marks[w * 64 + lane] : d;
          const bool live = (u32)lane < nv;
          if (live) a.done_frames[v0 + lane] = d;
          n_done = (u32)__builtin_popcountll(__builtin_amdgcn_ballot_w64(live && d != 0xFFFFFFFFu));
          n_run = (u32)__builtin_popcountll(__builtin_amdgcn_ballot_w64(live && sh.res_marks[15 * 64 + lane] != 0u));
        }
        if (lane == 0) res_put(a.res.wg_flags + wave_global, n_done | (n_run << 8), res_tag(call.epoch, 255u));
      }
      if (++ti == tpb) { ti = 0; ++blk; }
#ifdef KNH_DAG_STAMPS
      asm volatile("s_waitcnt vmcnt(0) lgkmcnt(0)" ::: "memory");
      busy += __builtin_amdgcn_s_memtime() - t0;
#endif
    }
    if (resident) asm volatile("s_waitcnt lgkmcnt(0)\n\ts_barrier" ::: "memory");
    else pipe_barrier();
  }
#ifdef KNH_DAG_STAMPS
  if (wave_global == 0u && lane == 0) a.flags[4 + NG] = (u32)(busy / (u64)(n_tiles > 0 ? n_tiles : 1));
#endif
  if (!resident) break;
  }
}

template <typename F, bool FMA, int T, int MODE, int NG, int I, int BASE, int W0, int LAST_ENV, typename G, typename... Rest>
__device__ __forceinline__ u32 pipe_dispatch(int wave, const PipeShared<F>& sh, const VoiceKernelArgs<F>& a, int lane, u32 wave_global, u32 v0, u32 nv, int wave_all) {
  constexpr int KF = GroupInfo<G>::fan_for(T);
  if (wave >= W0 && wave < W0 + KF) return pipe_run_group<F, FMA, T, MODE, NG, I, BASE, LAST_ENV, G>(sh, a, lane, wave_global, v0, nv, wave - W0, wave_all);
  if constexpr (sizeof...(Rest) > 0)
    return pipe_dispatch<F, FMA, T, MODE, NG, I + 1, BASE + GroupInfo<G>::slots, W0 + KF, LAST_ENV, Rest...>(wave, sh, a, lane, wave_global, v0, nv, wave_all);
  return 0xFFFFFFFFu;
}
template <int T, int MODE, typename... Gs> struct PipeWaves {
  static constexpr int chain = (0 + ... + GroupInfo<Gs>::fan_for(T));
  static constexpr int value = chain + (MODE == PIPE_FOLD ? 0 : 1);
};

template <int I, typename... Gs> struct LastEnv;
template <int I> struct LastEnv<I> { static constexpr int value = -1; };
template <int I, typename G, typename... Rest> struct LastEnv<I, G, Rest...> {
  static constexpr int later = LastEnv<I + 1, Rest...>::value;
  static constexpr int value = later >= 0 ? later : (GroupInfo<G>::has_env ? I : -1);
};

template <typename F, bool FMA, int T, int MODE, int GPW, typename... Gs>
__global__ void __launch_bounds__((GPW * PipeWaves<T, MODE, Gs...>::value * 64)) voice_pipe_kernel(VoiceKernelArgs<F> a) {
  constexpr int NG = (int)sizeof...(Gs);
  constexpr int CHAINW = PipeWaves<T, MODE, Gs...>::chain;
  constexpr int WAVES = PipeWaves<T, MODE, Gs...>::value;
  static_assert(GPW == 1 || GPW == 2, "one or two voice groups per workgroup");
  static_assert(T <= 64 && T % 8 == 0, "a tile column per lane of the folding wavefront");
  constexpr bool kSine = (false || ... || GroupInfo<Gs>::uses_sine);
  constexpr long kEdgeElems = (long)EdgeMap<MODE, NG>::tiles * EdgeLayout<F, T>::tile;
  constexpr int kRingTiles = T * (int)sizeof(F) >= RingLines<F>::kLine ? (0 + ... + (GroupInfo<Gs>::uses_ring ? 1 : 0)) : 0;
  constexpr long kLdsFree = 160 * 1024 - 1024 - 4096 - 64 - (long)sizeof(float) * (kSine ? 16384 : 4) - (long)sizeof(F) * GPW * kEdgeElems
                            - (long)GPW * kRingTiles * RingLines<F>::kTileBytes;
#ifndef KNH_EVCAP_MAX
#define KNH_EVCAP_MAX 2048
#endif
  constexpr int kEvCap = kLdsFree < 16 ? 0 : (kLdsFree / 16 > KNH_EVCAP_MAX ? KNH_EVCAP_MAX : (int)(kLdsFree / 16));
  struct Lds {
    float sine[kSine ? 16384 : 4];
    __attribute__((aligned(16))) F edge[GPW * kEdgeElems];
    __attribute__((aligned(16))) Event ev_stage[kEvCap > 0 ? kEvCap : 1];
    __attribute__((aligned(16))) char ring_tiles[GPW * kRingTiles > 0 ? GPW * kRingTiles * RingLines<F>::kTileBytes : 16];
    u32 res_marks[16 * 64];
    u32 res_slot[16];
  };
  __shared__ Lds lds;
  float* const sine = lds.sine;
  F* const edge = lds.edge;
  Event* const ev_stage = lds.ev_stage;

  const int lane = threadIdx.x & 63;
  const int wave_all = threadIdx.x >> 6;
  const int grp = GPW > 1 ? wave_all / WAVES : 0;
  const int wave = GPW > 1 ? (wave_all + (grp ? WAVES / 2 : 0)) % WAVES : wave_all;
  u32 ev_first = 0, ev_count = 0;
  if (kEvCap > 0 && a.ev_start && !a.res.bell) {
    const u32 gv0 = blockIdx.x * (u32)(GPW * 64);
    const u32 gnv = a.n_voices - gv0 < (u32)(GPW * 64) ? a.n_voices - gv0 : (u32)(GPW * 64);
    ev_first = a.ev_start[gv0];
    ev_count = a.ev_start[gv0 + gnv] - ev_first;
    if (ev_count > (u32)kEvCap) ev_count = 0u;
    for (u32 i = threadIdx.x; i < ev_count; i += GPW * WAVES * 64) ev_stage[i] = a.events[ev_first + i];
  }
  if (kSine) {
    typedef __attribute__((address_space(1))) const void* gptr_t;
    typedef __attribute__((address_space(3))) void* lptr_t;
#pragma unroll 4
    for (int k = wave_all; k < 64; k += GPW * WAVES) {
      const float* g = a.sine_table + (k * 64 + lane) * 4;
      __builtin_amdgcn_global_load_lds((gptr_t)g, (lptr_t)(sine + k * 256), 16, 0, 0);
    }
    asm volatile("s_waitcnt vmcnt(0)" ::: "memory");
  }
  __syncthreads();
  if (a.res.bell) __builtin_amdgcn_s_setprio(3);
  PipeShared<F> sh;
  sh.sine = sine;
  sh.edge = edge + (long)grp * kEdgeElems;
  sh.ev_lds = ev_stage;
  sh.ev_lds_first = ev_first;
  sh.ev_lds_n = ev_count;
  sh.res_slot = lds.res_slot;
  sh.res_marks = lds.res_marks;
  sh.ev_stage = ev_stage;
  sh.ev_cap = (u32)(kEvCap > 0 ? kEvCap : 0);
  sh.n_threads = (u32)(GPW * WAVES * 64);
  {
    constexpr bool ring_groups[] = {GroupInfo<Gs>::uses_ring...};
    int k = 0;
#pragma unroll
    for (int i = 0; i < 4; ++i) {
      const bool u = i < NG && kRingTiles > 0 && ring_groups[i < NG ? i : 0];
      sh.ring_tile_of[i] = u ? (__attribute__((address_space(3))) char*)(lds.ring_tiles + ((long)grp * kRingTiles + k) * RingLines<F>::kTileBytes) : nullptr;
      k += u ? 1 : 0;
    }
  }
  const u32 wave_global = blockIdx.x * (u32)GPW + (u32)grp;
  const u32 v0 = wave_global * 64u;
  const bool dead = GPW > 1 && v0 >= a.n_voices;
  const u32 nv = dead ? 0u : (a.n_voices - v0 < 64u ? a.n_voices - v0 : 64u);
  u32 done_frame = 0xFFFFFFFFu;
  constexpr bool kPan = (false || ... || GroupInfo<Gs>::pan);
  if (dead) {
    const u32 n_frames = a.frame_end - a.frame_begin;
    const int n_steps = (int)((n_frames + T - 1) / T) * (int)a.n_blocks + NG - (MODE == PIPE_FOLD ? 1 : 0);
    for (int s = 0; s < n_steps; ++s) pipe_barrier();
  } else if (wave == CHAINW) {
    constexpr bool kAnyEnvM = (false || ... || GroupInfo<Gs>::has_env);
    pipe_run_mixer<F, FMA, T, MODE, NG, kPan, CHAINW, kAnyEnvM>(sh, a, lane, wave_global, v0, nv, wave_all);
  } else {
    done_frame = pipe_dispatch<F, FMA, T, MODE, NG, 0, 0, 0, LastEnv<0, Gs...>::value, Gs...>(wave, sh, a, lane, wave_global, v0, nv, wave_all);
  }
  if (a.res.bell) return;
  constexpr bool kAnyEnv = (false || ... || GroupInfo<Gs>::has_env);
  if constexpr (kAnyEnv) {
    u32* marks = reinterpret_cast<u32*>(edge) + (long)grp * (CHAINW * 64);
    pipe_barrier();
    if (wave < CHAINW) marks[wave * 64 + lane] = done_frame;
    pipe_barrier();
    if (wave == 0 && !dead) {
      u32 d = 0xFFFFFFFFu;
#pragma unroll
      for (int g = 0; g < CHAINW; ++g) d = marks[g * 64 + lane] != 0xFFFFFFFFu ? marks[g * 64 + lane] : d;
      const bool live = (u32)lane < nv;
      if (live) a.done_frames[v0 + lane] = d;
      const u64 bd = __builtin_amdgcn_ballot_w64(live && d != 0xFFFFFFFFu);
      if (lane == 0 && bd) atomicOr(&a.flags[0], 1u);
    }
  }
}

}
```

Before: 2911 billion.

## Fold per-wave partials inside pipe kernel via cluster tree with atomic counters

Adds an in-kernel fold path. The mixer wave of each workgroup reduces partial rows hierarchically: clusters of 16 rows first, then a root fold driven by atomic arrival counters. This removes the separate fold kernel launch for eligible pipe configurations (tree mix, gpw 1, no jit or interp). The cost is extra atomics, relaxed agent-scope stores, a changed barrier in the mixer loop, extra device buffers, and more mixer-wave work that may lengthen the critical path.

Result: slower. 1948 billion (-33.1%).

```diff
diff --git a/bindings/rust/knaster_hip/src/ffi.rs b/bindings/rust/knaster_hip/src/ffi.rs
--- a/bindings/rust/knaster_hip/src/ffi.rs
+++ b/bindings/rust/knaster_hip/src/ffi.rs
@@ -144,6 +144,7 @@
     pub fn knh_bank_process_block(bank: *mut knh_bank, frames_to_process: usize, block_start_offset: usize, frame_clock: u64, out: *mut c_void, out_flags: *mut u32) -> i32;
     pub fn knh_jit_stats(memory_hits: *mut u64, disk_hits: *mut u64, helper_compiles: *mut u64, in_process_compiles: *mut u64);
     pub fn knh_bank_resident_stats(bank: *mut knh_bank, calls: *mut u64, launches: *mut u64) -> i32;
+    pub fn knh_bank_fold_in_kernel_launches(bank: *mut knh_bank, launches: *mut u64) -> i32;
     pub fn knh_bank_resident_trace(bank: *mut knh_bank, ticks5: *mut u64) -> i32;
     pub fn knh_bank_process_block_channels(bank: *mut knh_bank, frames_to_process: usize, block_start_offset: usize, frame_clock: u64, out_channels: *const *mut c_void, out_flags: *mut u32) -> i32;
     pub fn knh_bank_process_block_device(bank: *mut knh_bank, frames_to_process: usize, block_start_offset: usize, frame_clock: u64, out_device: *mut c_void, hip_stream: *mut c_void) -> i32;
diff --git a/include/knaster_hip.h b/include/knaster_hip.h
--- a/include/knaster_hip.h
+++ b/include/knaster_hip.h
@@ -157,6 +157,7 @@
 int32_t knh_bank_process_block_channels(knh_bank* bank, size_t frames_to_process, size_t block_start_offset,
                                         uint64_t frame_clock, void* const* out_channels, uint32_t* out_flags);
 int32_t knh_bank_resident_stats(knh_bank* bank, uint64_t* calls, uint64_t* launches);
+int32_t knh_bank_fold_in_kernel_launches(knh_bank* bank, uint64_t* launches);
 int32_t knh_bank_resident_trace(knh_bank* bank, uint64_t* ticks5);
 int32_t knh_bank_process_block_device(knh_bank* bank, size_t frames_to_process,
                                       size_t block_start_offset, uint64_t frame_clock,
diff --git a/knaster_amd/_lib.py b/knaster_amd/_lib.py
--- a/knaster_amd/_lib.py
+++ b/knaster_amd/_lib.py
@@ -70,6 +70,7 @@
     "knh_bank_process_block": (C.c_int32, [C.c_void_p, C.c_size_t, C.c_size_t, C.c_uint64, C.c_void_p, C.POINTER(C.c_uint32)]),
     "knh_jit_stats": (None, [C.POINTER(C.c_uint64), C.POINTER(C.c_uint64), C.POINTER(C.c_uint64), C.POINTER(C.c_uint64)]),
     "knh_bank_resident_stats": (C.c_int32, [C.c_void_p, C.POINTER(C.c_uint64), C.POINTER(C.c_uint64)]),
+    "knh_bank_fold_in_kernel_launches": (C.c_int32, [C.c_void_p, C.POINTER(C.c_uint64)]),
     "knh_bank_resident_trace": (C.c_int32, [C.c_void_p, C.POINTER(C.c_uint64)]),
     "knh_bank_process_block_channels": (C.c_int32, [C.c_void_p, C.c_size_t, C.c_size_t, C.c_uint64, C.POINTER(C.c_void_p), C.POINTER(C.c_uint32)]),
     "knh_bank_process_block_device": (C.c_int32, [C.c_void_p, C.c_size_t, C.c_size_t, C.c_uint64, C.c_void_p, C.c_void_p]),
diff --git a/knaster_amd/bank.py b/knaster_amd/bank.py
--- a/knaster_amd/bank.py
+++ b/knaster_amd/bank.py
@@ -260,6 +260,11 @@
         self._check(self._lib.knh_bank_resident_stats(self._h, C.byref(c), C.byref(n)))
         return int(c.value), int(n.value)
 
+    def fold_in_kernel_launches(self) -> int:
+        n = C.c_uint64(0)
+        self._check(self._lib.knh_bank_fold_in_kernel_launches(self._h, C.byref(n)))
+        return int(n.value)
+
     def debug_words(self) -> np.ndarray:
         d = np.zeros(16, dtype=np.uint32)
         self._check(self._lib.knh_bank_debug_words(self._h, d.ctypes.data_as(C.c_void_p)))
diff --git a/knaster_amd/build.py b/knaster_amd/build.py
--- a/knaster_amd/build.py
+++ b/knaster_amd/build.py
@@ -12,7 +12,7 @@
 UNITS = [("kernels_pipe.hip", "kernels_pipe_mixer.o", ["-DKNH_PIPE_PART=0"]), ("kernels_pipe.hip", "kernels_pipe_fold.o", ["-DKNH_PIPE_PART=1"]),
          ("kernels_pipe.hip", "kernels_pipe_inplace.o", ["-DKNH_PIPE_PART=2"])] + [(s, s.replace(".hip", ".o"), []) for s in SOURCES[1:]]
 HELPER = os.path.join(CSRC, "knh_jit_helper")
-HEADERS = ["jit_cache.hpp", "stage_table.hpp", "bank_base.hpp", "voice_bank.hpp", "resident_call.hpp", "event_resolver.hpp", "chain_signature.hpp", "voice_stages.hpp", "voice_chain.hpp", "voice_pipe.hpp", "voice_frame.hpp", "kernel_registry.hpp", "jit.hpp", "host_shards.hpp", "shard_workers.hpp", "rank_bank.hpp", "galactic_bank.hpp", "voice_galactic.hpp", os.path.join("..", "..", "include", "knaster_hip.h"),
+HEADERS = ["jit_cache.hpp", "stage_table.hpp", "bank_base.hpp", "voice_bank.hpp", "fold_in_path.hpp", "resident_call.hpp", "event_resolver.hpp", "chain_signature.hpp", "voice_stages.hpp", "voice_chain.hpp", "voice_pipe.hpp", "voice_frame.hpp", "kernel_registry.hpp", "jit.hpp", "host_shards.hpp", "shard_workers.hpp", "rank_bank.hpp", "galactic_bank.hpp", "voice_galactic.hpp", os.path.join("..", "..", "include", "knaster_hip.h"),
            os.path.join("..", "build.py")]
 FLAGS = [
     "--offload-arch=gfx950",
diff --git a/knaster_amd/csrc/bank.hip b/knaster_amd/csrc/bank.hip
--- a/knaster_amd/csrc/bank.hip
+++ b/knaster_amd/csrc/bank.hip
@@ -29,6 +29,7 @@
 #include "chain_signature.hpp"
 #include "event_resolver.hpp"
 #include "resident_call.hpp"
+#include "fold_in_path.hpp"
 #include "voice_bank.hpp"
 
 namespace {
@@ -476,6 +477,13 @@
     return KNH_OK;
   });
 }
+int32_t knh_bank_fold_in_kernel_launches(knh_bank* bank, uint64_t* launches) {
+  return guarded(bank, [&]() -> int32_t {
+    if (!bank || !launches) return KNH_ERR_INVALID_ARGUMENT;
+    *launches = bank->fold_in_kernel_launches();
+    return KNH_OK;
+  });
+}
 int32_t knh_bank_resident_trace(knh_bank* bank, uint64_t* ticks5) {
   return guarded(bank, [&]() -> int32_t {
     if (!bank || !ticks5) return KNH_ERR_INVALID_ARGUMENT;
diff --git a/knaster_amd/csrc/bank_base.hpp b/knaster_amd/csrc/bank_base.hpp
--- a/knaster_amd/csrc/bank_base.hpp
+++ b/knaster_amd/csrc/bank_base.hpp
@@ -79,6 +79,7 @@
   }
   virtual uint32_t ranks() const { return 1; }
   virtual void resident_stats(uint64_t* calls, uint64_t* launches) { if (calls) *calls = 0; if (launches) *launches = 0; }
+  virtual uint64_t fold_in_kernel_launches() { return 0; }
   virtual void resident_trace(uint64_t* five) { for (int k = 0; k < 5; ++k) five[k] = 0; }
 
   int fail(int code, const std::string& msg) {
diff --git a/knaster_amd/csrc/fold_in_path.hpp b/knaster_amd/csrc/fold_in_path.hpp
--- /dev/null
+++ b/knaster_amd/csrc/fold_in_path.hpp
@@ -0,0 +1,34 @@
+#pragma once
+#include <cstddef>
+#include <cstdint>
+
+namespace knh {
+
+struct FoldInForm {
+  bool mix_tree;
+  bool interp, jit;
+  int wide_waves;
+  bool pipe;
+  bool pipe_pair;
+  int pipe_form;
+  int pipe_gpw;
+  bool pipe_fan;
+  unsigned n_groups;
+};
+enum : unsigned { kFoldInCluster = 16u, kFoldInMaxGroups = kFoldInCluster * kFoldInCluster, kFoldInCounterWords = kFoldInCluster + 1u };
+
+inline bool fold_in_form_ok(const FoldInForm& f, const char* env) {
+  if (env && env[0] == '0') return false;
+  if (!f.mix_tree || f.interp || f.jit || f.wide_waves != 0 || !f.pipe || f.pipe_pair) return false;
+  if (f.pipe_gpw != 1 || f.pipe_form == 1 || f.pipe_fan) return false;
+  return f.n_groups >= 1u && f.n_groups <= kFoldInMaxGroups;
+}
+inline bool fold_in_launch_ok(bool form_ok, bool hand_over, bool want_voices, uint32_t frame_begin, uint32_t frame_end) {
+  return form_ok && !hand_over && !want_voices && frame_end > frame_begin;
+}
+inline size_t fold_in_counter_words(uint32_t n_blocks) { return static_cast<size_t>(n_blocks) * kFoldInCounterWords; }
+inline size_t fold_in_cluster_elems(uint32_t n_blocks, unsigned planes, size_t block_size) {
+  return static_cast<size_t>(n_blocks) * planes * kFoldInCluster * block_size;
+}
+
+}
diff --git a/knaster_amd/csrc/voice_bank.hpp b/knaster_amd/csrc/voice_bank.hpp
--- a/knaster_amd/csrc/voice_bank.hpp
+++ b/knaster_amd/csrc/voice_bank.hpp
@@ -183,6 +183,24 @@
     a.done_frames = d_done;
     a.flags = d_flags;
     a.res = knh_dev::Resident{};
+    a.fold = knh_dev::FoldIn<F>{};
+  }
+  bool fold_in_form = false;
+  uint32_t* d_fold_in_counters = nullptr;
+  F* d_cluster_rows = nullptr;
+  uint64_t fold_in_launches = 0;
+  uint64_t fold_in_kernel_launches() override { return fold_in_launches; }
+  bool fold_in_kernel(bool hand_over, bool want_voices, uint32_t fb, uint32_t fe) const { return knh::fold_in_launch_ok(fold_in_form, hand_over, want_voices, fb, fe); }
+  hipError_t fold_in_alloc(uint32_t n_blocks, hipStream_t s) {
+    if (d_fold_in_counters) (void)hipFree(d_fold_in_counters);
+    if (d_cluster_rows) (void)hipFree(d_cluster_rows);
+    d_fold_in_counters = nullptr;
+    d_cluster_rows = nullptr;
+    hipError_t e = hipMalloc(&d_fold_in_counters, knh::fold_in_counter_words(n_blocks) * sizeof(uint32_t));
+    if (e != hipSuccess) return e;
+    e = hipMemsetAsync(d_fold_in_counters, 0, knh::fold_in_counter_words(n_blocks) * sizeof(uint32_t), s);
+    if (e != hipSuccess) return e;
+    return hipMalloc(&d_cluster_rows, knh::fold_in_cluster_elems(n_blocks, fold_planes, block_size) * sizeof(F));
   }
   bool timing = false;
   std::vector<std::pair<hipEvent_t, hipEvent_t>> timing_pool;
@@ -196,7 +214,7 @@
     if (own_stream) (void)hipStreamSynchronize(own_stream);
     resolver.quiesce();
     if (flags_stream_set && flags_stream != own_stream) (void)hipStreamSynchronize(flags_stream);
-    void* dev_ptrs[] = {d_state, d_sine, d_seg_table, d_delay, d_buffer, d_partials, d_out, d_voices, d_done, d_flags, d_input, d_prog, d_sin_slots, d_fold_count};
+    void* dev_ptrs[] = {d_state, d_sine, d_seg_table, d_delay, d_buffer, d_partials, d_out, d_voices, d_done, d_flags, d_input, d_prog, d_sin_slots, d_fold_count, d_fold_in_counters, d_cluster_rows};
     for (void* p : dev_ptrs)
       if (p) (void)hipFree(p);
     void* host_ptrs[] = {h_ev_start2[0], h_ev_start2[1], h_events2[0], h_events2[1], h_out, h_input, h_done};
@@ -606,6 +624,12 @@
     pan = !signature.empty() && stages.back().kind == KNH_STAGE_PAN2;
     fold_planes = pan ? 2u : 1u;
     KNH_HIP(hipMalloc(&d_partials, fold_planes * n_waves * bs * sizeof(F)));
+    fold_in_form = knh::fold_in_form_ok(knh::FoldInForm{desc.mix_mode == KNH_MIX_TREE, interp, jit != nullptr, wide_waves, pipe != nullptr, pipe_pair,
+                                                        pipe ? pipe->form : -1, pipe ? pipe->gpw : 0, pipe && pipe->form == 0 && pipe->long_tiles != 0, n_groups}, std::getenv("KNH_FOLD_IN_KERNEL"));
+    if (fold_in_form) {
+      KNH_HIP(fold_in_alloc(1, nullptr));
+      KNH_HIP(hipDeviceSynchronize());
+    }
     KNH_HIP(hipMalloc(&d_out, desc.out_channels * bs * sizeof(F)));
     KNH_HIP(hipMemset(d_out, 0, desc.out_channels * bs * sizeof(F)));
     KNH_HIP(hipMalloc(&d_done, static_cast<size_t>(nv) * sizeof(uint32_t)));
@@ -1484,6 +1508,7 @@
       KNH_HIP(hipFree(d_partials));
       d_partials = nullptr;
       KNH_HIP(hipMalloc(&d_partials, static_cast<size_t>(n_blocks) * fold_planes * n_waves * block_size * sizeof(F)));
+      if (fold_in_form) KNH_HIP(fold_in_alloc(n_blocks, s));
       partials_blocks = n_blocks;
     }
     if (!out_device && n_blocks > out_blocks) {
@@ -1535,6 +1560,14 @@
     }
     a.voices_out = want_voices ? (stage_out ? stage_out : d_voices) : nullptr;
     a.flags = flags_now;
+    const bool hand_over = sync && out_host && !out_device && !voices_host && fe > fb;
+    F* dst = out_device ? static_cast<F*>(out_device) : (hand_over ? h_out : d_out);
+    const unsigned fold_channels = pan ? 1u : desc.out_channels;
+    const bool fold_in = fold_in_kernel(hand_over, want_voices, fb, fe);
+    if (fold_in) {
+      a.fold = knh_dev::FoldIn<F>{d_fold_in_counters, d_cluster_rows, dst, flags_next, fold_channels, accumulate ? 1u : 0u};
+      fold_in_launches += 1;
+    }
     std::pair<hipEvent_t, hipEvent_t>* tp = nullptr;
     if (timing) {
       if (timing_used == timing_pool.size()) {
@@ -1563,16 +1596,14 @@
       list_in_use = -1;
     }
 
-    const bool hand_over = sync && out_host && !out_device && !voices_host && fe > fb;
-    F* dst = out_device ? static_cast<F*>(out_device) : (hand_over ? h_out : d_out);
     knh_dev::HostDone hd{nullptr, nullptr, nullptr, 0u};
     if (hand_over) {
       done_epoch += 1;
       if (done_epoch == 0) done_epoch = 1;
       hd = knh_dev::HostDone{h_done, d_fold_count, flags_now, done_epoch};
     }
-    const unsigned fold_channels = pan ? 1u : desc.out_channels;
-    if (desc.mix_mode == KNH_MIX_LEFT_FOLD)
+    if (fold_in) {
+    } else if (desc.mix_mode == KNH_MIX_LEFT_FOLD)
       KNH_HIP(launch_fold(false, interp ? d_partials : d_voices, nv, static_cast<unsigned>(block_size), fb, fe, dst, fold_channels, static_cast<unsigned>(block_size), fold_planes, accumulate, flags_next, s, hand_over ? &hd : nullptr));
     else
       KNH_HIP(launch_fold(true, d_partials, n_waves, static_cast<unsigned>(block_size), fb, fe, dst, fold_channels, static_cast<unsigned>(block_size), n_blocks * fold_planes, accumulate, flags_next, s, hand_over ? &hd : nullptr));
diff --git a/knaster_amd/csrc/voice_chain.hpp b/knaster_amd/csrc/voice_chain.hpp
--- a/knaster_amd/csrc/voice_chain.hpp
+++ b/knaster_amd/csrc/voice_chain.hpp
@@ -380,6 +380,14 @@
   const u64 c = (u64)slot[0] | ((u64)slot[1] << 32);
   return res_unpack(c);
 }
+template <typename F>
+struct FoldIn {
+  u32* counters;
+  F* cluster_rows;
+  F* out;
+  u32* zero_flags;
+  u32 channels, accumulate;
+};
 template <typename F>
 struct VoiceKernelArgs {
   typename WordOf<F>::type* state;
@@ -407,6 +415,7 @@
   u32* done_frames;
   u32* flags;
   Resident res;
+  FoldIn<F> fold;
 };
 
 constexpr int kWave = 64;
@@ -467,6 +476,98 @@
   if (nv == 64u) tree_cols_pan<F, 64, true, B>(col, st, gl, gr, gst, nv, l, r);
   else tree_cols_pan<F, 64, false, B>(col, st, gl, gr, gst, nv, l, r);
 }
+
+template <typename F, int PLANES>
+struct FoldInJob {
+  static constexpr int FPL = sizeof(F) == 8 ? 2 : 4;
+  static constexpr u32 CH = 64u * FPL;
+  enum : u32 { IDLE = 0, ARRIVED = 1, FOLDING = 2, STORED = 3 };
+  u32 st = IDLE, level = 0;
+  u32 blk = 0, next_blk = 0;
+  u32 chunk = 0;
+  u32 ticket = 0;
+  F ld[16 * FPL];
+
+  __device__ __forceinline__ bool busy(u32 n_blocks) const { return st != IDLE || next_blk < n_blocks; }
+
+  __device__ __forceinline__ void turn(const VoiceKernelArgs<F>& a, int lane, u32 wave_global, u32 n_rows, u32 fbeg, u32 fend, u32 ready) {
+    const u32 n_clusters = (n_rows + 15u) / 16u, cluster = wave_global >> 4;
+    const u32 csize = n_rows - cluster * 16u < 16u ? n_rows - cluster * 16u : 16u;
+    const u32 bs = a.block_size;
+    const u32 cpp = (fend - fbeg + CH - 1u) / CH;
+    u32* const cnt_blk = a.fold.counters + (long)blk * 17;
+    const bool root = level != 0u;
+    const u32 cnt = root ? n_clusters : csize;
+    const F* const src = root ? a.fold.cluster_rows + (long)blk * PLANES * 16 * bs : a.partials + ((long)blk * PLANES * n_rows + cluster * 16u) * bs;
+    const long pstride = (long)(root ? 16u : n_rows) * bs;
+    auto issue = [&](u32 c) {
+      const u32 plane = PLANES > 1 ? c / cpp : 0u;
+      const u32 f0 = fbeg + (c - plane * cpp) * CH + (u32)lane;
+#pragma unroll
+      for (int r = 0; r < 16; ++r) {
+        if ((u32)r < cnt) {
+#pragma unroll
+          for (int k = 0; k < FPL; ++k) {
+            const u32 f = f0 + 64u * k < fend ? f0 + 64u * k : fend - 1u;
+            ld[k * 16 + r] = __hip_atomic_load(src + plane * pstride + (long)r * bs + f, __ATOMIC_RELAXED, __HIP_MEMORY_SCOPE_AGENT);
+          }
+        } else {
+#pragma unroll
+          for (int k = 0; k < FPL; ++k) ld[k * 16 + r] = (F)0;
+        }
+      }
+    };
+    if (st == ARRIVED) {
+      const u32 t = __builtin_amdgcn_readfirstlane(ticket);
+      if (t + 1u != cnt) {
+        st = IDLE;
+      } else {
+        if (lane == 0) __hip_atomic_store(cnt_blk + (root ? 16u : cluster), 0u, __ATOMIC_RELAXED, __HIP_MEMORY_SCOPE_AGENT);
+        issue(0u);
+        chunk = 1u;
+        st = FOLDING;
+        return;
+      }
+    } else if (st == FOLDING) {
+      const u32 c = chunk - 1u;
+      const u32 plane = PLANES > 1 ? c / cpp : 0u;
+      const u32 f0 = fbeg + (c - plane * cpp) * CH + (u32)lane;
+      const bool last_level = root || n_clusters == 1u;
+#pragma unroll
+      for (int k = 0; k < FPL; ++k) {
+        F v[16];
+#pragma unroll
+        for (int r = 0; r < 16; ++r) v[r] = ld[k * 16 + r];
+        const F node = cnt == 16u ? tree_reduce<F, 16, true>(v, 1u, 16u) : tree_reduce<F, 16, false>(v, 1u, cnt);
+        const u32 f = f0 + 64u * k;
+        if (f < fend) {
+          if (last_level) {
+            F* o = a.fold.out + ((long)blk * PLANES + plane) * a.fold.channels * bs + f;
+            for (u32 ch = 0; ch < a.fold.channels; ++ch, o += bs) *o = a.fold.accumulate ? *o + node : node;
+          } else {
+            __hip_atomic_store(a.fold.cluster_rows + (((long)blk * PLANES + plane) * 16 + cluster) * bs + f, node, __ATOMIC_RELAXED, __HIP_MEMORY_SCOPE_AGENT);
+          }
+        }
+      }
+      if (chunk < cpp * (u32)PLANES) { issue(chunk); ++chunk; return; }
+      if (last_level) { st = IDLE; level = 0u; }
+      else { st = STORED; return; }
+    } else if (st == STORED) {
+      asm volatile("s_waitcnt vmcnt(0)" ::: "memory");
+      if (lane == 0) ticket = __hip_atomic_fetch_add(cnt_blk + 16, 1u, __ATOMIC_RELAXED, __HIP_MEMORY_SCOPE_AGENT);
+      level = 1u;
+      st = ARRIVED;
+      return;
+    }
+    if (st == IDLE && next_blk < ready) {
+      blk = next_blk++;
+      level = 0u;
+      asm volatile("s_waitcnt vmcnt(0)" ::: "memory");
+      if (lane == 0) ticket = __hip_atomic_fetch_add(a.fold.counters + (long)blk * 17 + cluster, 1u, __ATOMIC_RELAXED, __HIP_MEMORY_SCOPE_AGENT);
+      st = ARRIVED;
+    }
+  }
+};
 
 template <typename F>
 struct ResServerArgs {
diff --git a/knaster_amd/csrc/voice_pipe.hpp b/knaster_amd/csrc/voice_pipe.hpp
--- a/knaster_amd/csrc/voice_pipe.hpp
+++ b/knaster_amd/csrc/voice_pipe.hpp
@@ -424,6 +424,7 @@
       F* const row = a.partials + ((long)blk * n_waves_total + wave_global) * a.block_size + n0 + lane;
       const F sum = fold_group<F, 64>(col, ST, nv);
       if (a.res.bell) res_put_sample(a.res.rows + (((long)res_tile * n_waves_total + wave_global) * 64 + lane) * ResWords<F>::value, sum, res_tag(res_epoch, res_tile));
+      else if (a.fold.counters) __hip_atomic_store(row, sum, __ATOMIC_RELAXED, __HIP_MEMORY_SCOPE_AGENT);
       else *row = sum;
       if (a.voices_out) {
         for (u32 v = 0; v < nv; ++v) a.voices_out[(long)(v0 + v) * a.block_size + n0 + lane] = col[v * ST];
@@ -437,6 +438,9 @@
       if (a.res.bell) {
         res_put_sample(a.res.rows + ((((long)res_tile * 2 + 0) * n_waves_total + wave_global) * 64 + lane) * ResWords<F>::value, accl, res_tag(res_epoch, res_tile));
         res_put_sample(a.res.rows + ((((long)res_tile * 2 + 1) * n_waves_total + wave_global) * 64 + lane) * ResWords<F>::value, accr, res_tag(res_epoch, res_tile));
+      } else if (a.fold.counters) {
+        __hip_atomic_store(rl, accl, __ATOMIC_RELAXED, __HIP_MEMORY_SCOPE_AGENT);
+        __hip_atomic_store(rr, accr, __ATOMIC_RELAXED, __HIP_MEMORY_SCOPE_AGENT);
       } else { *rl = accl; *rr = accr; }
       if (a.voices_out) {
         for (u32 v = 0; v < nv; ++v) {
@@ -449,13 +453,16 @@
   }
 }
 
-template <typename F, bool FMA, int T, int MODE, int NG, bool PAN, int CHAINW, bool HAS_ENV>
+template <typename F, bool FMA, int T, int MODE, int NG, bool PAN, int CHAINW, bool HAS_ENV, bool FOLD_IN>
 __device__ __forceinline__ void pipe_run_mixer(const PipeShared<F>& sh, const VoiceKernelArgs<F>& a, int lane, u32 wave_global,
                                                u32 v0, u32 nv, int wave_all) {
   u32 fbeg = a.frame_begin, fend = a.frame_end;
   const bool resident = a.res.bell != nullptr;
   u32 res_expect = a.res.first_epoch;
   const u32 n_waves_total = (a.n_voices + 63u) / 64u;
+  const bool fold_in = FOLD_IN && !resident && a.fold.counters != nullptr;
+  FoldInJob<F, PAN ? 2 : 1> job;
+  if (fold_in && wave_global == 0u && lane == 0) { a.fold.zero_flags[0] = 0u; a.fold.zero_flags[1] = 0u; }
   for (;;) {
   ResCall call;
   call.epoch = 0u;
@@ -475,7 +482,10 @@
 #ifdef KNH_DAG_STAMPS
   u64 busy = 0;
 #endif
-  for (int s = 0; s < n_steps; ++s) {
+  u32 blocks_done = 0u, done_1 = 0u, done_2 = 0u;
+  for (int s = 0; s < n_steps || (fold_in && job.busy(a.n_blocks)); ++s) {
+    if (fold_in) job.turn(a, lane, wave_global, n_waves_total, fbeg, fend, s < n_steps ? done_2 : blocks_done);
+    if (s >= n_steps) continue;
     const int g = s - NG;
     if (g >= 0 && g < n_tiles) {
 #ifdef KNH_DAG_STAMPS
@@ -498,13 +508,15 @@
         }
         if (lane == 0) res_put(a.res.wg_flags + wave_global, n_done | (n_run << 8), res_tag(call.epoch, 255u));
       }
-      if (++ti == tpb) { ti = 0; ++blk; }
+      if (++ti == tpb) { ti = 0; ++blk; ++blocks_done; }
 #ifdef KNH_DAG_STAMPS
       asm volatile("s_waitcnt vmcnt(0) lgkmcnt(0)" ::: "memory");
       busy += __builtin_amdgcn_s_memtime() - t0;
 #endif
     }
-    if (resident) asm volatile("s_waitcnt lgkmcnt(0)\n\ts_barrier" ::: "memory");
+    done_2 = done_1;
+    done_1 = blocks_done;
+    if (resident || fold_in) asm volatile("s_waitcnt lgkmcnt(0)\n\ts_barrier" ::: "memory");
     else pipe_barrier();
   }
 #ifdef KNH_DAG_STAMPS
@@ -621,7 +633,7 @@
     for (int s = 0; s < n_steps; ++s) pipe_barrier();
   } else if (wave == CHAINW) {
     constexpr bool kAnyEnvM = (false || ... || GroupInfo<Gs>::has_env);
-    pipe_run_mixer<F, FMA, T, MODE, NG, kPan, CHAINW, kAnyEnvM>(sh, a, lane, wave_global, v0, nv, wave_all);
+    pipe_run_mixer<F, FMA, T, MODE, NG, kPan, CHAINW, kAnyEnvM, (GPW == 1 && WAVES <= 4)>(sh, a, lane, wave_global, v0, nv, wave_all);
   } else {
     done_frame = pipe_dispatch<F, FMA, T, MODE, NG, 0, 0, 0, LastEnv<0, Gs...>::value, Gs...>(wave, sh, a, lane, wave_global, v0, nv, wave_all);
   }
```
